# e4s2022/e4s

Measured on AMD Instinct MI355X. Metric: 1024^2 face-swap images/sec, higher is better.
Workload: dtype f32 operands as hi+lo bf16, 3 bf16 MFMAs per product, f32 accumulate (bf16x3) on the 3x3 convs whose launch fills the chip; exact f32 elsewhere; 1 GPU; E4S-core face swap at 1024^2 (2x Net3 encoder @256^2, style swap, 12 LocalMLPs, mask-guided StyleGAN2 generator K=13), BASELINE.json configs[3] shard: 8 swaps per GPU per step; per_gpu_batch=8, global_batch=8, out_size=1024, hip_graph=True, precision=as bf16x3 where the launch fills the chip (this batch), else exact fp32, parallelism=image-parallel x1

## Files before the change

### e4s_amd/csrc/encoder.hip

```cpp
#include "common.h"

namespace {

__global__ void resize_bilinear_kernel(const float* __restrict__ x, float* __restrict__ y, int B, int C, int Hi,
                                       int Wi, int Ho, int Wo) {
    const int64_t n = (int64_t)B * Ho * Wo * C;
    const int64_t i = (int64_t)blockIdx.x * blockDim.x + threadIdx.x;
    if (i >= n) return;
    const int c = (int)(i % C);
    int64_t r = i / C;
    const int ox = (int)(r % Wo); r /= Wo;
    const int oy = (int)(r % Ho);
    const int b = (int)(r / Ho);
    const float sy = (float)Hi / Ho, sx = (float)Wi / Wo;
    float fy = ((float)oy + 0.5f) * sy - 0.5f, fx = ((float)ox + 0.5f) * sx - 0.5f;
    fy = fy < 0.f ? 0.f : fy;
    fx = fx < 0.f ? 0.f : fx;
    const int y0 = (int)fy, x0 = (int)fx;
    const int y1 = y0 + (y0 < Hi - 1 ? 1 : 0), x1 = x0 + (x0 < Wi - 1 ? 1 : 0);
    const float ly = fy - y0, lx = fx - x0, hy = 1.f - ly, hx = 1.f - lx;
    const float* p = x + ((int64_t)b * C + c) * Hi * Wi;
    y[i] = hy * (hx * p[(int64_t)y0 * Wi + x0] + lx * p[(int64_t)y0 * Wi + x1]) +
           ly * (hx * p[(int64_t)y1 * Wi + x0] + lx * p[(int64_t)y1 * Wi + x1]);
}

__global__ void conv3x3_small_kernel(const float* __restrict__ x, const float* __restrict__ w, float* __restrict__ y,
                                     int B, int H, int W, int Cin, int Cout) {
    extern __shared__ float sw[];
    const int nw = Cout * Cin * 9;
    for (int t = threadIdx.x; t < nw; t += blockDim.x) {
        const int k = t % 9, ci = (t / 9) % Cin, co = t / (9 * Cin);
        sw[(k * Cin + ci) * Cout + co] = w[t];
    }
    __syncthreads();
    const int cg = Cout / 4;
    const int64_t n = (int64_t)B * H * W * cg;
    for (int64_t i = (int64_t)blockIdx.x * blockDim.x + threadIdx.x; i < n; i += (int64_t)gridDim.x * blockDim.x) {
        const int c4 = (int)(i % cg) * 4;
        int64_t r = i / cg;
        const int ox = (int)(r % W); r /= W;
        const int oy = (int)(r % H);
        const int b = (int)(r / H);
        f32x4 acc = {0.f, 0.f, 0.f, 0.f};
        for (int ky = 0; ky < 3; ++ky) {
            const int iy = oy + ky - 1;
            if (iy < 0 || iy >= H) continue;
            for (int kx = 0; kx < 3; ++kx) {
                const int ix = ox + kx - 1;
                if (ix < 0 || ix >= W) continue;
                const float* xp = x + (((int64_t)b * H + iy) * W + ix) * Cin;
                const float* wp = sw + ((ky * 3 + kx) * Cin) * Cout + c4;
                for (int ci = 0; ci < Cin; ++ci) acc += xp[ci] * *reinterpret_cast<const f32x4*>(wp + ci * Cout);
            }
        }
        *reinterpret_cast<f32x4*>(y + i * 4) = acc;
    }
}

__global__ __launch_bounds__(256) void conv3x3_stem_kernel(const float* __restrict__ x, const float* __restrict__ w, float* __restrict__ y,
                                                           double* __restrict__ stats_ws, int H, int W, int tx_n, int per_img) {
    __shared__ f32x4 sx[18 * 18];
    __shared__ double sred[2][16][64];
    const int tid = threadIdx.x;
    const int b = blockIdx.x / per_img, rem = blockIdx.x - b * per_img;
    const int tyb = rem / tx_n, txb = rem - tyb * tx_n;
    const int y0 = tyb * 16, x0 = txb * 16;
    for (int h = tid; h < 324; h += 256) {
        const int hy = h / 18, hx = h - hy * 18;
        const int iy = y0 + hy - 1, ix = x0 + hx - 1;
        f32x4 v = {0.f, 0.f, 0.f, 0.f};
        if ((unsigned)iy < (unsigned)H && (unsigned)ix < (unsigned)W) {
            const float* xp = x + (((int64_t)b * H + iy) * W + ix) * 3;
            v = f32x4{xp[0], xp[1], xp[2], 0.f};
        }
        sx[h] = v;
    }
    const int g = tid & 15, py = tid >> 4;
    f32x4 wr[27];
#pragma unroll
    for (int k = 0; k < 9; ++k)
#pragma unroll
        for (int ci = 0; ci < 3; ++ci)
#pragma unroll
            for (int j = 0; j < 4; ++j) wr[k * 3 + ci][j] = w[((4 * g + j) * 3 + ci) * 9 + k];
    __syncthreads();
    double s[4] = {0.0, 0.0, 0.0, 0.0}, q[4] = {0.0, 0.0, 0.0, 0.0};
    float* yrow = y + (((int64_t)b * H + y0 + py) * W + x0) * 64 + 4 * g;
#pragma unroll 4
    for (int px = 0; px < 16; ++px) {
        f32x4 acc = {0.f, 0.f, 0.f, 0.f};
#pragma unroll
        for (int ky = 0; ky < 3; ++ky)
#pragma unroll
            for (int kx = 0; kx < 3; ++kx) {
                const f32x4 v = sx[(py + ky) * 18 + px + kx];
                const int k = (ky * 3 + kx) * 3;
                acc += v[0] * wr[k] + v[1] * wr[k + 1] + v[2] * wr[k + 2];
            }
        *reinterpret_cast<f32x4*>(yrow + (int64_t)px * 64) = acc;
        if (stats_ws) {
#pragma unroll
            for (int j = 0; j < 4; ++j) {
                s[j] += (double)acc[j];
                q[j] += (double)acc[j] * (double)acc[j];
            }
        }
    }
    if (stats_ws) {
#pragma unroll
        for (int j = 0; j < 4; ++j) {
            sred[0][py][4 * g + j] = s[j];
            sred[1][py][4 * g + j] = q[j];
        }
        __syncthreads();
        if (tid < 64) {
            double a = 0.0, c = 0.0;
#pragma unroll
            for (int r = 0; r < 16; ++r) {
                a += sred[0][r][tid];
                c += sred[1][r][tid];
            }
            double* slot = stats_ws + (((int64_t)b * 64 + tid) * per_img + rem) * 2;
            slot[0] = a;
            slot[1] = c;
        }
    }
}

__global__ void instnorm_partial_kernel(const float* __restrict__ x, double* __restrict__ ws, int HW, int C, int nsplit) {
    const int slabs = C / 64;
    const int split = blockIdx.x % nsplit;
    const int slab = (blockIdx.x / nsplit) % slabs;
    const int b = blockIdx.x / (nsplit * slabs);
    const int cl = threadIdx.x & 63, pg = threadIdx.x >> 6;
    const int c = slab * 64 + cl;
    const int per = (HW + nsplit - 1) / nsplit;
    const int p0 = split * per, p1 = (p0 + per < HW) ? p0 + per : HW;
    const float* xb = x + (int64_t)b * HW * C + c;
    double s = 0.0, q = 0.0;
    for (int p = p0 + pg; p < p1; p += 4) {
        const double v = (double)xb[(int64_t)p * C];
        s += v;
        q += v * v;
    }
    __shared__ double red[2][4][64];
    red[0][pg][cl] = s;
    red[1][pg][cl] = q;
    __syncthreads();
    if (pg == 0) {
        s = red[0][0][cl] + red[0][1][cl] + red[0][2][cl] + red[0][3][cl];
        q = red[1][0][cl] + red[1][1][cl] + red[1][2][cl] + red[1][3][cl];
        double* slot = ws + (((int64_t)b * C + c) * nsplit + split) * 2;
        slot[0] = s;
        slot[1] = q;
    }
}

__global__ __launch_bounds__(1024) void instnorm_small_kernel(const float* __restrict__ x, float* __restrict__ stats,
                                                              float* __restrict__ pooled, int HW, int C, float eps) {
    const int slabs = C / 64;
    const int slab = blockIdx.x % slabs, b = blockIdx.x / slabs;
    const int cl = threadIdx.x & 63, pg = threadIdx.x >> 6;
    const int c = slab * 64 + cl;
    const float* xb = x + (int64_t)b * HW * C + c;
    double s = 0.0, q = 0.0;
    int p = pg;
    for (; p + 7 * 16 < HW; p += 8 * 16) {
        float v[8];
#pragma unroll
        for (int u = 0; u < 8; ++u) v[u] = xb[(int64_t)(p + 16 * u) * C];
#pragma unroll
        for (int u = 0; u < 8; ++u) {
            s += (double)v[u];
            q += (double)v[u] * (double)v[u];
        }
    }
    for (; p < HW; p += 16) {
        const double v = (double)xb[(int64_t)p * C];
        s += v;
        q += v * v;
    }
    __shared__ double red[2][16][64];
    red[0][pg][cl] = s;
    red[1][pg][cl] = q;
    __syncthreads();
    if (pg == 0) {
        s = 0.0;
        q = 0.0;
#pragma unroll
        for (int k = 0; k < 16; ++k) { s += red[0][k][cl]; q += red[1][k][cl]; }
        const double mean = s / HW;
        double var = q / HW - mean * mean;
        if (var < 0.0) var = 0.0;
        const float mf = (float)mean;
        const float rstd = rsqrtf((float)var + eps);
        const int64_t i = (int64_t)b * C + c;
        stats[i * 2] = mf;
        stats[i * 2 + 1] = rstd;
        if (pooled) pooled[i] = (float)((mean - (double)mf) * (double)rstd);
    }
}

__global__ void instnorm_finalize_kernel(const double* __restrict__ ws, float* __restrict__ stats,
                                         float* __restrict__ pooled, int n, int HW, float eps, int nsplit) {
    const int i = blockIdx.x * blockDim.x + threadIdx.x;
    if (i >= n) return;
    double s = 0.0, q = 0.0;
#pragma unroll 8
    for (int k = 0; k < nsplit; ++k) {
        s += ws[((int64_t)i * nsplit + k) * 2];
        q += ws[((int64_t)i * nsplit + k) * 2 + 1];
    }
    const double mean = s / HW;
    double var = q / HW - mean * mean;
    if (var < 0.0) var = 0.0;
    const float mf = (float)mean;
    const float rstd = rsqrtf((float)var + eps);
    stats[i * 2] = mf;
    stats[i * 2 + 1] = rstd;
    if (pooled) pooled[i] = (float)((mean - (double)mf) * (double)rstd);
}

__global__ void instnorm_apply_kernel(const float* __restrict__ x, const float* __restrict__ stats,
                                      const float* __restrict__ gate, const float* __restrict__ res,
                                      const float* __restrict__ res_stats, const float* __restrict__ slope,
                                      float* __restrict__ y, int B, int H, int W, int C, int rs) {
    const int C4 = C / 4;
    const int64_t n = (int64_t)B * H * W * C4;
    const int64_t i = (int64_t)blockIdx.x * blockDim.x + threadIdx.x;
    if (i >= n) return;
    const int c = (int)(i % C4) * 4;
    int64_t r = i / C4;
    const int xx = (int)(r % W); r /= W;
    const int yy = (int)(r % H);
    const int b = (int)(r / H);
    f32x4 v = *reinterpret_cast<const f32x4*>(x + i * 4);
    f32x4 o;
#pragma unroll
    for (int e = 0; e < 4; ++e) {
        const float* st = stats + ((int64_t)b * C + c + e) * 2;
        o[e] = (v[e] - st[0]) * st[1];
        if (gate) o[e] *= gate[(int64_t)b * C + c + e];
    }
    if (res) {
        const int Hr = H * rs, Wr = W * rs;
        const f32x4 rv = *reinterpret_cast<const f32x4*>(res + (((int64_t)b * Hr + (int64_t)yy * rs) * Wr + (int64_t)xx * rs) * C + c);
#pragma unroll
        for (int e = 0; e < 4; ++e) {
            float t = rv[e];
            if (res_stats) {
                const float* st = res_stats + ((int64_t)b * C + c + e) * 2;
                t = (t - st[0]) * st[1];
            }
            o[e] += t;
        }
    }
    if (slope) {
#pragma unroll
        for (int e = 0; e < 4; ++e) o[e] = o[e] > 0.f ? o[e] : o[e] * slope[c + e];
    }
    *reinterpret_cast<f32x4*>(y + i * 4) = o;
}

__global__ void instnorm_apply_stats_kernel(const float* __restrict__ x, const float* __restrict__ stats,
                                            const float* __restrict__ gate, const float* __restrict__ res,
                                            const float* __restrict__ res_stats, const float* __restrict__ slope,
                                            float* __restrict__ y, double* __restrict__ ws, int H, int W, int C, int rs,
                                            int nsplit) {
    const int slabs = C / 64, HW = H * W;
    const int split = blockIdx.x % nsplit;
    const int slab = (blockIdx.x / nsplit) % slabs;
    const int b = blockIdx.x / (nsplit * slabs);
    const int cl = (threadIdx.x & 15) * 4, pg = threadIdx.x >> 4;
    const int c = slab * 64 + cl;
    const int per = (HW + nsplit - 1) / nsplit;
    const int p0 = split * per, p1 = (p0 + per < HW) ? p0 + per : HW;
    const int64_t bc = (int64_t)b * C + c;
    f32x4 mean, rstd, g, rmean, rrstd, sl;
#pragma unroll
    for (int e = 0; e < 4; ++e) {
        mean[e] = stats[(bc + e) * 2];
        rstd[e] = stats[(bc + e) * 2 + 1];
        g[e] = gate ? gate[bc + e] : 1.f;
        rmean[e] = res_stats ? res_stats[(bc + e) * 2] : 0.f;
        rrstd[e] = res_stats ? res_stats[(bc + e) * 2 + 1] : 1.f;
        sl[e] = slope ? slope[c + e] : 0.f;
    }
    const int Wr = W * rs;
    double s[4] = {0.0, 0.0, 0.0, 0.0}, q[4] = {0.0, 0.0, 0.0, 0.0};
    for (int p = p0 + pg; p < p1; p += 16) {
        const int64_t idx = ((int64_t)b * HW + p) * C + c;
        f32x4 o = (*reinterpret_cast<const f32x4*>(x + idx) - mean) * rstd;
        if (gate) o *= g;
        if (res) {
            const int yy = p / W, xx = p - yy * W;
            f32x4 t = *reinterpret_cast<const f32x4*>(res + (((int64_t)b * H * rs + (int64_t)yy * rs) * Wr + (int64_t)xx * rs) * C + c);
            if (res_stats) t = (t - rmean) * rrstd;
            o += t;
        }
        if (slope) {
#pragma unroll
            for (int e = 0; e < 4; ++e) o[e] = o[e] > 0.f ? o[e] : o[e] * sl[e];
        }
        *reinterpret_cast<f32x4*>(y + idx) = o;
#pragma unroll
        for (int e = 0; e < 4; ++e) {
            s[e] += (double)o[e];
            q[e] += (double)o[e] * (double)o[e];
        }
    }
    __shared__ double red[2][16][64];
#pragma unroll
    for (int e = 0; e < 4; ++e) {
        red[0][pg][cl + e] = s[e];
        red[1][pg][cl + e] = q[e];
    }
    __syncthreads();
    if (threadIdx.x < 64) {
        double a = 0.0, d = 0.0;
#pragma unroll
        for (int k = 0; k < 16; ++k) {
            a += red[0][k][threadIdx.x];
            d += red[1][k][threadIdx.x];
        }
        double* slot = ws + (((int64_t)b * C + slab * 64 + threadIdx.x) * nsplit + split) * 2;
        slot[0] = a;
        slot[1] = d;
    }
}

__device__ __forceinline__ void se_body(const float* pooled, float* hidden, const float* __restrict__ fc1,
                                        const float* __restrict__ fc2, float* __restrict__ gate, int C, int Cr) {
    int tpr = 64;
    while (tpr * Cr > (int)blockDim.x && tpr > 1) tpr >>= 1;
    for (int j0 = 0; j0 < Cr; j0 += blockDim.x / tpr) {
        const int j = j0 + threadIdx.x / tpr, l = threadIdx.x % tpr;
        float a = 0.f;
        if (j < Cr) {
            const float* row = fc1 + (int64_t)j * C;
            int c = l;
            for (; c + 7 * tpr < C; c += 8 * tpr) {
                float w[8];
#pragma unroll
                for (int u = 0; u < 8; ++u) w[u] = row[c + u * tpr];
#pragma unroll
                for (int u = 0; u < 8; ++u) a += w[u] * pooled[c + u * tpr];
            }
            for (; c < C; c += tpr) a += row[c] * pooled[c];
        }
        for (int o = tpr >> 1; o > 0; o >>= 1) a += __shfl_xor(a, o, 64);
        if (j < Cr && l == 0) hidden[j] = a > 0.f ? a : 0.f;
    }
    __syncthreads();
    for (int c = threadIdx.x; c < C; c += blockDim.x) {
        float a = 0.f;
        if ((Cr & 3) == 0) {
            const f32x4* w4 = reinterpret_cast<const f32x4*>(fc2 + (int64_t)c * Cr);
#pragma unroll 8
            for (int j = 0; j < Cr; j += 4) {
                const f32x4 w = w4[j >> 2];
                a += w[0] * hidden[j];
                a += w[1] * hidden[j + 1];
                a += w[2] * hidden[j + 2];
                a += w[3] * hidden[j + 3];
            }
        } else {
            for (int j = 0; j < Cr; ++j) a += fc2[(int64_t)c * Cr + j] * hidden[j];
        }
        gate[c] = 1.f / (1.f + __expf(-a));
    }
}

__global__ __launch_bounds__(512) void se_gate_kernel(const float* __restrict__ pooled_in, const float* __restrict__ fc1,
                                                      const float* __restrict__ fc2, float* __restrict__ gate, int C, int Cr) {
    extern __shared__ float sm[];
    float* pooled = sm;
    float* hidden = sm + C;
    const int b = blockIdx.x;
    for (int c = threadIdx.x; c < C; c += blockDim.x) pooled[c] = pooled_in[(int64_t)b * C + c];
    __syncthreads();
    se_body(pooled, hidden, fc1, fc2, gate + (int64_t)b * C, C, Cr);
}

__global__ __launch_bounds__(512) void finalize_se_kernel(const double* __restrict__ ws, float* __restrict__ stats,
                                                          const float* __restrict__ fc1, const float* __restrict__ fc2,
                                                          float* __restrict__ gate, int C, int Cr, int HW, float eps, int nsplit) {
    extern __shared__ float sm[];
    float* pooled = sm;
    float* hidden = sm + C;
    const int b = blockIdx.x;
    for (int c = threadIdx.x; c < C; c += blockDim.x) {
        const int64_t i = (int64_t)b * C + c;
        double s = 0.0, q = 0.0;
#pragma unroll 8
        for (int k = 0; k < nsplit; ++k) {
            s += ws[(i * nsplit + k) * 2];
            q += ws[(i * nsplit + k) * 2 + 1];
        }
        const double mean = s / HW;
        double var = q / HW - mean * mean;
        if (var < 0.0) var = 0.0;
        const float mf = (float)mean;
        const float rstd = rsqrtf((float)var + eps);
        stats[i * 2] = mf;
        stats[i * 2 + 1] = rstd;
        pooled[c] = (float)((mean - (double)mf) * (double)rstd);
    }
    __syncthreads();
    se_body(pooled, hidden, fc1, fc2, gate + (int64_t)b * C, C, Cr);
}

__device__ __forceinline__ int nearest_src(int dst, int in, int out) {
    const float scale = (float)in / (float)out;
    const int s = (int)floorf((float)dst * scale);
    return s < in - 1 ? s : in - 1;
}

constexpr int RM_PIX = 256;
constexpr int RM_NPG = 16;
__global__ __launch_bounds__(256) void region_mean_kernel(const float* __restrict__ feats, const uint8_t* __restrict__ labels, int Hm,
                                                          int Wm, float* __restrict__ out, float* __restrict__ ws, int H, int W, int C,
                                                          int R, int out_stride, int out_off, int nsplit) {
    extern __shared__ float sm[];
    const int slabs = C / 64;
    const int split = blockIdx.x % nsplit;
    const int slab = (blockIdx.x / nsplit) % slabs;
    const int b = blockIdx.x / (nsplit * slabs);
    const int cl = (threadIdx.x & 15) * 4, pg = threadIdx.x >> 4;
    float* sums = sm;
    int* cnt = reinterpret_cast<int*>(sm + RM_NPG * R * 64);
    for (int t = threadIdx.x; t < RM_NPG * R * 64; t += blockDim.x) sums[t] = 0.f;
    for (int t = threadIdx.x; t < R; t += blockDim.x) cnt[t] = 0;
    __syncthreads();
    const int HW = H * W;
    const int pbeg = split * RM_PIX, pend = pbeg + RM_PIX < HW ? pbeg + RM_PIX : HW;
    const float* fb = feats + (int64_t)b * HW * C + slab * 64 + cl;
    float* mine = sums + (pg * R) * 64 + cl;
    constexpr int U = 8;
    for (int p0 = pbeg + pg; p0 < pend; p0 += RM_NPG * U) {
        f32x4 v[U];
        int lab[U];
#pragma unroll
        for (int u = 0; u < U; ++u) {
            const int p = p0 + u * RM_NPG;
            const bool ok = p < pend;
            const int pp = ok ? p : pbeg;
            const int yy = pp / W, xx = pp - yy * W;
            lab[u] = ok ? labels[((int64_t)b * Hm + nearest_src(yy, Hm, H)) * Wm + nearest_src(xx, Wm, W)] : -1;
            v[u] = *reinterpret_cast<const f32x4*>(fb + (int64_t)pp * C);
        }
#pragma unroll
        for (int u = 0; u < U; ++u) {
            if (lab[u] >= 0 && lab[u] < R) {
                f32x4* acc = reinterpret_cast<f32x4*>(mine + lab[u] * 64);
                *acc += v[u];
                if (cl == 0) atomicAdd(&cnt[lab[u]], 1);
            }
        }
    }
    __syncthreads();
    for (int t = threadIdx.x; t < R * 64; t += blockDim.x) {
        const int r = t / 64, c = t % 64;
        float s = 0.f;
        for (int j = 0; j < RM_NPG; ++j) s += sums[(j * R + r) * 64 + c];
        if (ws) {
            ws[((int64_t)blockIdx.x * R + r) * 65 + c] = s;
            if (c == 0) ws[((int64_t)blockIdx.x * R + r) * 65 + 64] = __int_as_float(cnt[r]);
        } else {
            const int n = cnt[r];
            out[((int64_t)b * R + r) * out_stride + out_off + slab * 64 + c] = n > 0 ? s / (float)n : 0.f;
        }
    }
}

__global__ void region_mean_finish_kernel(const float* __restrict__ ws, float* __restrict__ out, int B, int C, int R, int out_stride,
                                          int out_off, int nsplit) {
    const int i = blockIdx.x * blockDim.x + threadIdx.x;
    if (i >= B * R * C) return;
    const int c = i % C, r = (i / C) % R, b = i / (C * R);
    const int slab = c >> 6, cc = c & 63;
// ... 36 lines not shown
                acc += w[j][0] * v[0] + w[j][1] * v[1] + w[j][2] * v[2] + w[j][3] * v[3];
            }
        }
        float a = wave_sum(acc);
        if (lane == 0) {
            a = a * scale + bs;
            if (act == 1) a = a > 0.f ? a : a * alpha;
            y[((int64_t)b * R + r) * O + o] = a + ad;
        }
    }
}

constexpr int GL_TB = 8;
template <int KV, int NR>
__global__ __launch_bounds__(256) __attribute__((amdgpu_waves_per_eu(2))) void grouped_linear_rows_kernel(const float* __restrict__ x, const float* __restrict__ Wt,
                                                                  const float* __restrict__ bias, const float* __restrict__ add,
                                                                  float* __restrict__ y, int B, int R, int K, int O, float scale,
                                                                  int act, float alpha) {
    constexpr int N = NR * GL_TB;
    const int lane = threadIdx.x & 63;
    const int opr = O / NR;
    const int64_t wid = (int64_t)blockIdx.x * (blockDim.x >> 6) + (threadIdx.x >> 6);
    if (wid >= (int64_t)R * opr) return;
    const int r = (int)(wid / opr), o0 = (int)(wid % opr) * NR;
    const float* wrow = Wt + ((int64_t)r * O + o0) * K;
    f32x4 w[NR][KV];
#pragma unroll
    for (int n = 0; n < NR; ++n)
#pragma unroll
        for (int j = 0; j < KV; ++j) {
            const int i = (j * 64 + lane) * 4;
            w[n][j] = i < K ? *reinterpret_cast<const f32x4*>(wrow + (int64_t)n * K + i) : f32x4{0.f, 0.f, 0.f, 0.f};
        }
    static_assert(N == 64 || N == 32, "lane -> value mapping below");
    constexpr int SH = N == 64 ? 0 : 1;
    const int mine = lane >> SH, tbm = mine / NR, nm = mine % NR;
    const float bs = bias ? bias[(int64_t)r * O + o0 + nm] : 0.f;
    const float ad = add ? add[o0 + nm] : 0.f;
    for (int b0 = 0; b0 < B; b0 += GL_TB) {
        float v[N];
#pragma unroll
        for (int tb = 0; tb < GL_TB; ++tb) {
            if (b0 + tb < B) {
                const float* xr = x + ((int64_t)(b0 + tb) * R + r) * K;
                f32x4 xv[KV];
#pragma unroll
                for (int j = 0; j < KV; ++j) {
                    const int i = (j * 64 + lane) * 4;
                    xv[j] = i < K ? *reinterpret_cast<const f32x4*>(xr + i) : f32x4{0.f, 0.f, 0.f, 0.f};
                }
#pragma unroll
                for (int n = 0; n < NR; ++n) {
                    float acc = 0.f;
#pragma unroll
                    for (int j = 0; j < KV; ++j)
#pragma unroll
                        for (int e = 0; e < 4; ++e) acc = fmaf(w[n][j][e], xv[j][e], acc);
                    v[tb * NR + n] = acc;
                }
            } else {
#pragma unroll
                for (int n = 0; n < NR; ++n) v[tb * NR + n] = 0.f;
            }
        }
        packed_wave_sum<N>(v, lane);
        if ((lane & ((1 << SH) - 1)) == 0 && b0 + tbm < B) {
            float a = v[0] * scale + bs;
            if (act == 1) a = a > 0.f ? a : a * alpha;
            y[((int64_t)(b0 + tbm) * R + r) * O + o0 + nm] = a + ad;
        }
    }
}

__global__ void grouped_linear_longk_kernel(const float* __restrict__ x, const float* __restrict__ Wt,
                                            const float* __restrict__ bias, const float* __restrict__ add,
                                            float* __restrict__ y, int B, int R, int K, int O, float scale, int act,
                                            float alpha) {
    const int lane = threadIdx.x & 63;
    const int64_t wid = (int64_t)blockIdx.x * (blockDim.x >> 6) + (threadIdx.x >> 6);
    if (wid >= (int64_t)R * O) return;
    const int r = (int)(wid / O), o = (int)(wid % O);
    const float* wrow = Wt + ((int64_t)r * O + o) * K;
    for (int b = 0; b < B; ++b) {
        const float* xr = x + ((int64_t)b * R + r) * K;
        float acc = 0.f;
        for (int i = lane * 4; i < K; i += 256) {
            const f32x4 w = *reinterpret_cast<const f32x4*>(wrow + i);
            const f32x4 v = *reinterpret_cast<const f32x4*>(xr + i);
            acc += w[0] * v[0] + w[1] * v[1] + w[2] * v[2] + w[3] * v[3];
        }
        float a = wave_sum(acc);
        if (lane == 0) {
            a = a * scale + (bias ? bias[(int64_t)r * O + o] : 0.f);
            if (act == 1) a = a > 0.f ? a : a * alpha;
            y[((int64_t)b * R + r) * O + o] = a + (add ? add[o] : 0.f);
        }
    }
}


__global__ __launch_bounds__(256) void swap_styles_kernel(const float* __restrict__ tgt, const float* __restrict__ src,
                                                          float* __restrict__ out, int R, int C, unsigned sel, int ear, int teeth,
                                                          int below) {
    __shared__ float part[256];
    const int b = blockIdx.x / R, r = blockIdx.x - b * R;
    const float* a = tgt + ((int64_t)b * R + r) * C;
    const float* c = src + ((int64_t)b * R + r) * C;
    float* o = out + ((int64_t)b * R + r) * C;
    int mode = (sel >> r) & 1u;
    if (r == ear || r == teeth) {
        float s = 0.f;
        for (int i = threadIdx.x; i < C; i += 256) s += c[i];
        part[threadIdx.x] = s;
        __syncthreads();
        for (int st = 128; st > 0; st >>= 1) {
            if ((int)threadIdx.x < st) part[threadIdx.x] += part[threadIdx.x + st];
            __syncthreads();
        }
        if (part[0] == 0.f) mode = (r == ear) ? 2 : 0;
    }
    if (r == below) mode = 2;
    for (int i = threadIdx.x; i < C; i += 256) o[i] = mode == 2 ? (a[i] + c[i]) / 2.f : (mode == 1 ? c[i] : a[i]);
}

}

extern "C" int e4s_resize_bilinear_f32(const float* x, float* y, int B, int C, int Hi, int Wi, int Ho, int Wo, void* stream) {
    const int64_t n = (int64_t)B * Ho * Wo * C;
    if (n <= 0) return 0;
    hipLaunchKernelGGL(resize_bilinear_kernel, dim3((unsigned)((n + 255) / 256)), dim3(256), 0, as_stream(stream), x, y, B, C, Hi, Wi, Ho, Wo);
    E4S_CHECK_LAUNCH();
    return 0;
}

extern "C" int e4s_conv3x3_small_f32(const float* x, const float* w, float* y, int B, int H, int W, int Cin, int Cout, void* stream) {
    if (Cout % 4) return (int)hipErrorInvalidValue;
    const int64_t n = (int64_t)B * H * W * (Cout / 4);
    if (n <= 0) return 0;
    const size_t smem = (size_t)Cout * Cin * 9 * sizeof(float);
    if (smem > 48 * 1024) return (int)hipErrorInvalidValue;
    int64_t nblk = (n + 255) / 256;
    if (nblk > 4096) nblk = 4096;
    hipLaunchKernelGGL(conv3x3_small_kernel, dim3((unsigned)nblk), dim3(256), smem, as_stream(stream), x, w, y, B, H, W, Cin, Cout);
    E4S_CHECK_LAUNCH();
    return 0;
}

extern "C" int e4s_conv3x3_stem_f32(const float* x, const float* w, float* y, double* stats_ws, int B, int H, int W, int Cin, int Cout,
                                    void* stream) {
    if (!x || !w || !y || Cin != 3 || Cout != 64 || H % 16 || W % 16 || B <= 0 || H <= 0 || W <= 0) return (int)hipErrorInvalidValue;
    const int tx_n = W / 16, per_img = (H / 16) * tx_n;
    const int64_t blocks = (int64_t)B * per_img;
    if (blocks >= (1ll << 31)) return (int)hipErrorInvalidValue;
    hipLaunchKernelGGL(conv3x3_stem_kernel, dim3((unsigned)blocks), dim3(256), 0, as_stream(stream), x, w, y, stats_ws, H, W, tx_n, per_img);
    E4S_CHECK_LAUNCH();
    return 0;
}

static int instnorm_nsplit(int B, int HW, int C) {
    int nsplit = 2048 / (B * (C / 64) > 0 ? B * (C / 64) : 1);
    if (nsplit < 1) nsplit = 1;
    if (nsplit > HW / 64) nsplit = HW / 64 > 0 ? HW / 64 : 1;
    if (nsplit > 64) nsplit = 64;
    return nsplit;
}

extern "C" int e4s_instnorm_stats_f32(const float* x, float* stats, float* pooled, double* ws, int B, int HW, int C,
                                      float eps, void* stream) {
    if (C % 64) return (int)hipErrorInvalidValue;
    hipStream_t st = as_stream(stream);
    if (HW <= 1024 && HW >= 16) {
        hipLaunchKernelGGL(instnorm_small_kernel, dim3(B * (C / 64)), dim3(1024), 0, st, x, stats, pooled, HW, C, eps);
        E4S_CHECK_LAUNCH();
        return 0;
    }
    const int nsplit = instnorm_nsplit(B, HW, C);
    hipLaunchKernelGGL(instnorm_partial_kernel, dim3(B * (C / 64) * nsplit), dim3(256), 0, st, x, ws, HW, C, nsplit);
    E4S_CHECK_LAUNCH();
    const int n = B * C;
    hipLaunchKernelGGL(instnorm_finalize_kernel, dim3((n + 255) / 256), dim3(256), 0, st, ws, stats, pooled, n, HW, eps, nsplit);
    E4S_CHECK_LAUNCH();
    return 0;
}

extern "C" int e4s_instnorm_finalize_f32(const double* ws, float* stats, float* pooled, int B, int HW, int C, int nslots,
                                         float eps, void* stream) {
    const int n = B * C;
    if (n <= 0 || nslots < 1) return (int)hipErrorInvalidValue;
    hipLaunchKernelGGL(instnorm_finalize_kernel, dim3((n + 255) / 256), dim3(256), 0, as_stream(stream), ws, stats, pooled, n,
                       HW, eps, nslots);
    E4S_CHECK_LAUNCH();
    return 0;
}

extern "C" int e4s_instnorm_apply_stats_f32(const float* x, const float* stats, const float* gate, const float* res,
                                            const float* res_stats, const float* slope, float* y, double* ws, int* nslots,
                                            int B, int H, int W, int C, int rs, void* stream) {
    if (C % 64 || rs < 1 || !nslots) return (int)hipErrorInvalidValue;
    const int ns = instnorm_nsplit(B, H * W, C);
    *nslots = ns;
    hipLaunchKernelGGL(instnorm_apply_stats_kernel, dim3(B * (C / 64) * ns), dim3(256), 0, as_stream(stream), x, stats, gate,
                       res, res_stats, slope, y, ws, H, W, C, rs, ns);
    E4S_CHECK_LAUNCH();
    return 0;
}

extern "C" int64_t e4s_instnorm_ws_doubles(int B, int HW, int C) {
    return (int64_t)2 * B * C * instnorm_nsplit(B, HW, C);
}

extern "C" int e4s_instnorm_apply_f32(const float* x, const float* stats, const float* gate, const float* res,
                                      const float* res_stats, const float* slope, float* y, int B, int H, int W, int C,
                                      int rs, void* stream) {
    if (C % 4 || rs < 1) return (int)hipErrorInvalidValue;
    const int64_t n = (int64_t)B * H * W * (C / 4);
    if (n <= 0) return 0;
    hipLaunchKernelGGL(instnorm_apply_kernel, dim3((unsigned)((n + 255) / 256)), dim3(256), 0, as_stream(stream), x, stats, gate, res, res_stats, slope, y, B, H, W, C, rs);
    E4S_CHECK_LAUNCH();
    return 0;
}

extern "C" int e4s_se_gate_f32(const float* pooled, const float* fc1, const float* fc2, float* gate, int B, int C,
                               int Cr, void* stream) {
    if (B <= 0 || C <= 0 || Cr <= 0 || (size_t)(C + Cr) * sizeof(float) > 48 * 1024) return (int)hipErrorInvalidValue;
    hipLaunchKernelGGL(se_gate_kernel, dim3(B), dim3(512), (size_t)(C + Cr) * sizeof(float), as_stream(stream), pooled, fc1, fc2, gate, C, Cr);
    E4S_CHECK_LAUNCH();
    return 0;
}

extern "C" int e4s_instnorm_finalize_se_f32(const double* ws, float* stats, const float* fc1, const float* fc2, float* gate, int B,
                                            int HW, int C, int Cr, int nslots, float eps, void* stream) {
    if (B <= 0 || C <= 0 || Cr <= 0 || nslots <= 0 || HW <= 0 || (size_t)(C + Cr) * sizeof(float) > 48 * 1024)
        return (int)hipErrorInvalidValue;
    hipLaunchKernelGGL(finalize_se_kernel, dim3(B), dim3(512), (size_t)(C + Cr) * sizeof(float), as_stream(stream), ws, stats, fc1, fc2,
                       gate, C, Cr, HW, eps, nslots);
    E4S_CHECK_LAUNCH();
    return 0;
}

static int region_mean_nsplit(int HW) { return (HW + RM_PIX - 1) / RM_PIX; }

extern "C" int64_t e4s_region_mean_ws_floats(int B, int HW, int C, int R) {
    const int ns = region_mean_nsplit(HW);
    return ns > 1 ? (int64_t)B * (C / 64) * ns * R * 65 : 0;
}

extern "C" int e4s_region_mean_f32(const float* feats, const uint8_t* labels, int Hm, int Wm, float* out, float* ws, int B, int H,
                                   int W, int C, int R, int out_stride, int out_off, void* stream) {
    if (C % 64 || R > 64 || R < 1 || B <= 0 || H <= 0 || W <= 0) return (int)hipErrorInvalidValue;
    if (reinterpret_cast<uintptr_t>(feats) & 15) return (int)hipErrorInvalidValue;
    const int ns = region_mean_nsplit(H * W);
    if (ns > 1 && !ws) return (int)hipErrorInvalidValue;
    const int64_t blocks = (int64_t)B * (C / 64) * ns;
    if (blocks >= (1ll << 31) || (int64_t)B * R * C >= (1ll << 31)) return (int)hipErrorInvalidValue;
    const size_t smem = (size_t)(RM_NPG * R * 64) * sizeof(float) + (size_t)R * sizeof(int);
    if (smem > 64 * 1024) return (int)hipErrorInvalidValue;
    hipStream_t st = as_stream(stream);
    hipLaunchKernelGGL(region_mean_kernel, dim3((unsigned)blocks), dim3(256), smem, st, feats, labels, Hm, Wm, out, ns > 1 ? ws : nullptr,
                       H, W, C, R, out_stride, out_off, ns);
    E4S_CHECK_LAUNCH();
    if (ns > 1) {
        const int n = B * R * C;
        hipLaunchKernelGGL(region_mean_finish_kernel, dim3((n + 255) / 256), dim3(256), 0, st, ws, out, B, C, R, out_stride, out_off, ns);
        E4S_CHECK_LAUNCH();
    }
    return 0;
}

extern "C" int e4s_grouped_linear_f32(const float* x, const float* W, const float* bias, const float* add, float* y,
                                      int B, int R, int K, int O, float scale, int act, float alpha, void* stream) {
    if (K % 4) return (int)hipErrorInvalidValue;
    const int64_t nw = (int64_t)R * O;
    if (nw <= 0 || B <= 0) return 0;
    hipStream_t st = as_stream(stream);
    if (K > 64 * 4 * MAXKV) {
        hipLaunchKernelGGL(grouped_linear_longk_kernel, dim3((unsigned)((nw + 3) / 4)), dim3(256), 0, st, x, W, bias, add, y, B, R, K, O, scale, act, alpha);
        E4S_CHECK_LAUNCH();
        return 0;
    }
    if (K <= 1536 && O % 8 == 0 && nw >= 4096) {
        if (K <= 512)
            hipLaunchKernelGGL((grouped_linear_rows_kernel<2, 8>), dim3((unsigned)((nw / 8 + 3) / 4)), dim3(256), 0, st, x, W, bias, add, y, B, R, K, O, scale, act, alpha);
        else if (K <= 1024)
            hipLaunchKernelGGL((grouped_linear_rows_kernel<4, 4>), dim3((unsigned)((nw / 4 + 3) / 4)), dim3(256), 0, st, x, W, bias, add, y, B, R, K, O, scale, act, alpha);
        else
            hipLaunchKernelGGL((grouped_linear_rows_kernel<6, 4>), dim3((unsigned)((nw / 4 + 3) / 4)), dim3(256), 0, st, x, W, bias, add, y, B, R, K, O, scale, act, alpha);
        E4S_CHECK_LAUNCH();
        return 0;
    }
    hipLaunchKernelGGL(grouped_linear_kernel, dim3((unsigned)((nw + 3) / 4)), dim3(256), 0, st, x, W, bias, add, y, B, R, K, O, scale, act, alpha);
    E4S_CHECK_LAUNCH();
    return 0;
}

extern "C" int e4s_swap_styles_f32(const float* tgt, const float* src, float* out, int B, int R, int C, unsigned sel, int ear, int teeth,
                                   int below, void* stream) {
    if (!tgt || !src || !out || B < 1 || R < 1 || R > 32 || C < 1) return (int)hipErrorInvalidValue;
    hipLaunchKernelGGL(swap_styles_kernel, dim3((unsigned)(B * R)), dim3(256), 0, as_stream(stream), tgt, src, out, R, C, sel, ear, teeth,
                       below);
    E4S_CHECK_LAUNCH();
    return 0;
}
```

### e4s_amd/csrc/ops.hip

```cpp
#include "common.h"

namespace {

__device__ __forceinline__ float bias_act_one(float x, float ref, int code, float alpha, float scale) {
    float y;
    switch (code) {
        case 12: case 32: y = 0.f; break;
        case 30: y = (x > 0.f) ? x : x * alpha; break;
        case 31: y = (ref > 0.f) ? x : x * alpha; break;
        default: y = x; break;
    }
    return y * scale;
}

__global__ void fused_bias_act_v4(const f32x4* __restrict__ x, const float* __restrict__ b,
                                  const f32x4* __restrict__ ref, f32x4* __restrict__ y, int64_t n4,
                                  int step_b, int size_b, int code, float alpha, float scale) {
    const int64_t stride = (int64_t)gridDim.x * blockDim.x;
    for (int64_t i = (int64_t)blockIdx.x * blockDim.x + threadIdx.x; i < n4; i += stride) {
        f32x4 v = x[i];
        if (b) {
            const float bv = b[((i * 4) / step_b) % size_b];
            v += bv;
        }
        f32x4 r = {0.f, 0.f, 0.f, 0.f};
        if (ref) r = ref[i];
        f32x4 o;
#pragma unroll
        for (int e = 0; e < 4; ++e) o[e] = bias_act_one(v[e], r[e], code, alpha, scale);
        y[i] = o;
    }
}

__global__ void fused_bias_act_scalar(const float* __restrict__ x, const float* __restrict__ b,
                                      const float* __restrict__ ref, float* __restrict__ y, int64_t n,
                                      int step_b, int size_b, int code, float alpha, float scale) {
    const int64_t stride = (int64_t)gridDim.x * blockDim.x;
    for (int64_t i = (int64_t)blockIdx.x * blockDim.x + threadIdx.x; i < n; i += stride) {
        float v = x[i];
        if (b) v += b[(i / step_b) % size_b];
        y[i] = bias_act_one(v, ref ? ref[i] : 0.f, code, alpha, scale);
    }
}

__global__ void channel_sum_kernel(const float* __restrict__ g, float* __restrict__ out, int64_t n,
                                   int step_b, int size_b) {
    const int c = blockIdx.x;
    const int64_t outer = n / ((int64_t)step_b * size_b);
    float acc = 0.f;
    for (int64_t o = 0; o < outer; ++o) {
        const float* base = g + (o * size_b + c) * (int64_t)step_b;
        for (int i = threadIdx.x; i < step_b; i += blockDim.x) acc += base[i];
    }
    __shared__ float red[4];
    acc = wave_sum(acc);
    if ((threadIdx.x & 63) == 0) red[threadIdx.x >> 6] = acc;
    __syncthreads();
    if (threadIdx.x == 0) out[c] = red[0] + red[1] + red[2] + red[3];
}

constexpr int TOH = 16, TOW = 64;

__device__ __forceinline__ int floordiv(int a, int b) {
    int c = a / b;
    if (c * b > a) --c;
    return c;
}

__global__ void upfirdn2d_kernel(const float* __restrict__ x, const float* __restrict__ k, float* __restrict__ y,
                                 int major, int in_h, int in_w, int minor, int kh, int kw, int up_x, int up_y,
                                 int down_x, int down_y, int pad_x0, int pad_y0, int out_h, int out_w,
                                 int tin_h, int tin_w, int tiles_x, int tiles_y) {
    extern __shared__ float sm[];
    float* sk = sm;
    float* sx = sm + kh * kw;
    int bid = blockIdx.x;
    const int tx = bid % tiles_x; bid /= tiles_x;
    const int ty = bid % tiles_y; bid /= tiles_y;
    const int mi = bid % minor;
    const int mj = bid / minor;
    const int oy0 = ty * TOH, ox0 = tx * TOW;
    for (int t = threadIdx.x; t < kh * kw; t += blockDim.x) {
        const int ky = t / kw, kx = t - ky * kw;
        sk[t] = k[(kh - 1 - ky) * kw + (kw - 1 - kx)];
    }
    const int mid_y0 = oy0 * down_y - pad_y0, mid_x0 = ox0 * down_x - pad_x0;
    const int in_y0 = floordiv(mid_y0 + up_y - 1, up_y), in_x0 = floordiv(mid_x0 + up_x - 1, up_x);
    for (int t = threadIdx.x; t < tin_h * tin_w; t += blockDim.x) {
        const int ry = t / tin_w, rx = t - ry * tin_w;
        const int iy = in_y0 + ry, ix = in_x0 + rx;
        float v = 0.f;
        if (iy >= 0 && ix >= 0 && iy < in_h && ix < in_w)
            v = x[(((int64_t)mj * in_h + iy) * in_w + ix) * minor + mi];
        sx[t] = v;
    }
    __syncthreads();
    for (int t = threadIdx.x; t < TOH * TOW; t += blockDim.x) {
        const int ry = t / TOW, rx = t - ry * TOW;
        const int oy = oy0 + ry, ox = ox0 + rx;
        if (oy >= out_h || ox >= out_w) continue;
        const int my = oy * down_y - pad_y0, mx = ox * down_x - pad_x0;
        const int iy_first = floordiv(my + up_y - 1, up_y), ix_first = floordiv(mx + up_x - 1, up_x);
        float acc = 0.f;
        for (int iy = iy_first, jy = iy_first * up_y - my; jy < kh; ++iy, jy += up_y) {
            const float* row = sx + (iy - in_y0) * tin_w;
            for (int ix = ix_first, jx = ix_first * up_x - mx; jx < kw; ++ix, jx += up_x)
                acc += row[ix - in_x0] * sk[jy * kw + jx];
        }
        y[(((int64_t)mj * out_h + oy) * out_w + ox) * minor + mi] = acc;
    }
}

}

extern "C" int e4s_abi_version(void) { return 18; }
extern "C" const char* e4s_build_arch(void) { return "gfx950"; }

extern "C" int e4s_fused_bias_act_f32(const float* x, const float* b, const float* ref, float* y, int64_t n,
                                      int step_b, int size_b, int act, int grad, float alpha, float scale,
                                      void* stream) {
    if (n <= 0) return 0;
    const int code = act * 10 + grad;
    if (code == 31 && !ref) return (int)hipErrorInvalidValue;
    if (b && (step_b <= 0 || size_b <= 0)) return (int)hipErrorInvalidValue;
    const bool vec = (n % 4 == 0) && (!b || step_b % 4 == 0) &&
                     ((reinterpret_cast<uintptr_t>(x) | reinterpret_cast<uintptr_t>(y) |
                       reinterpret_cast<uintptr_t>(ref)) % 16 == 0);
    const int block = 256;
    if (vec) {
        const int64_t n4 = n / 4;
        const int grid = (int)((n4 + block - 1) / block < 8192 ? (n4 + block - 1) / block : 8192);
        hipLaunchKernelGGL(fused_bias_act_v4, dim3(grid), dim3(block), 0, as_stream(stream),
                           reinterpret_cast<const f32x4*>(x), b, reinterpret_cast<const f32x4*>(ref),
                           reinterpret_cast<f32x4*>(y), n4, step_b, size_b, code, alpha, scale);
    } else {
        const int grid = (int)((n + block - 1) / block < 8192 ? (n + block - 1) / block : 8192);
        hipLaunchKernelGGL(fused_bias_act_scalar, dim3(grid), dim3(block), 0, as_stream(stream), x, b, ref, y, n,
                           step_b, size_b, code, alpha, scale);
    }
    E4S_CHECK_LAUNCH();
    return 0;
}

extern "C" int e4s_channel_sum_f32(const float* g, float* out, int64_t n, int step_b, int size_b, void* stream) {
    if (size_b <= 0 || step_b <= 0 || n % ((int64_t)step_b * size_b)) return (int)hipErrorInvalidValue;
    hipLaunchKernelGGL(channel_sum_kernel, dim3(size_b), dim3(256), 0, as_stream(stream), g, out, n, step_b, size_b);
    E4S_CHECK_LAUNCH();
    return 0;
}

__global__ __launch_bounds__(256) void fir_nhwc_kernel(const float* __restrict__ x, const float* __restrict__ k, float* __restrict__ y,
                                                       int in_h, int in_w, int C, int kh, int kw, int pad_x0, int pad_y0,
                                                       int out_h, int out_w) {
    __shared__ float sk[64];
    if (threadIdx.x < kh * kw) {
        const int ky = threadIdx.x / kw, kx = threadIdx.x - ky * kw;
        sk[threadIdx.x] = k[(kh - 1 - ky) * kw + (kw - 1 - kx)];
    }
    __syncthreads();
    const int c4n = C >> 2, ppb = 256 / c4n;
    const int c4 = threadIdx.x % c4n, pxl = threadIdx.x / c4n;
    const int ox = blockIdx.x * ppb + pxl, oy0 = blockIdx.y * 4;
    if (pxl >= ppb || ox >= out_w) return;
    const float* xb = x + (size_t)blockIdx.z * in_h * in_w * C + c4 * 4;
    f32x4 acc[4];
#pragma unroll
    for (int r = 0; r < 4; ++r) acc[r] = f32x4{0.f, 0.f, 0.f, 0.f};
    for (int ry = 0; ry < kh + 3; ++ry) {
        const int iy = oy0 + ry - pad_y0;
        if ((unsigned)iy >= (unsigned)in_h) continue;
        for (int jx = 0; jx < kw; ++jx) {
            const int ix = ox + jx - pad_x0;
            if ((unsigned)ix >= (unsigned)in_w) continue;
            const f32x4 v = *reinterpret_cast<const f32x4*>(xb + ((size_t)iy * in_w + ix) * C);
#pragma unroll
            for (int r = 0; r < 4; ++r) {
                const int jy = ry - r;
                if (jy >= 0 && jy < kh) acc[r] += v * sk[jy * kw + jx];
            }
        }
    }
#pragma unroll
    for (int r = 0; r < 4; ++r)
        if (oy0 + r < out_h)
            *reinterpret_cast<f32x4*>(y + (((size_t)blockIdx.z * out_h + oy0 + r) * out_w + ox) * C + c4 * 4) = acc[r];
}

template <int KH, int KW>
__global__ __launch_bounds__(256) void fir_nhwc_fixed_kernel(const float* __restrict__ x, const float* __restrict__ k, float* __restrict__ y,
                                                             int in_h, int in_w, int C, int pad_x0, int pad_y0, int out_h, int out_w) {
    __shared__ float sk[KH * KW];
    if (threadIdx.x < KH * KW) {
        const int ky = threadIdx.x / KW, kx = threadIdx.x - ky * KW;
        sk[threadIdx.x] = k[(KH - 1 - ky) * KW + (KW - 1 - kx)];
    }
    __syncthreads();
    const int c4n = C >> 2, ppb = 256 / c4n;
    const int c4 = threadIdx.x % c4n, pxl = threadIdx.x / c4n;
    const int ox = blockIdx.x * ppb + pxl, oy0 = blockIdx.y * 4;
    if (pxl >= ppb || ox >= out_w) return;
    const float* xb = x + (size_t)blockIdx.z * in_h * in_w * C + c4 * 4;
    f32x4 v[KH + 3][KW];
#pragma unroll
    for (int ry = 0; ry < KH + 3; ++ry) {
        const int iy = oy0 + ry - pad_y0;
#pragma unroll
        for (int jx = 0; jx < KW; ++jx) {
            const int ix = ox + jx - pad_x0;
            v[ry][jx] = ((unsigned)iy < (unsigned)in_h && (unsigned)ix < (unsigned)in_w)
                            ? *reinterpret_cast<const f32x4*>(xb + ((size_t)iy * in_w + ix) * C) : f32x4{0.f, 0.f, 0.f, 0.f};
        }
    }
#pragma unroll
    for (int r = 0; r < 4; ++r) {
        if (oy0 + r >= out_h) continue;
        f32x4 acc = {0.f, 0.f, 0.f, 0.f};
#pragma unroll
        for (int ry = r; ry < r + KH; ++ry) {
            const int iy = oy0 + ry - pad_y0;
            if ((unsigned)iy >= (unsigned)in_h) continue;
#pragma unroll
            for (int jx = 0; jx < KW; ++jx) {
                const int ix = ox + jx - pad_x0;
                if ((unsigned)ix < (unsigned)in_w) acc += v[ry][jx] * sk[(ry - r) * KW + jx];
            }
        }
        *reinterpret_cast<f32x4*>(y + (((size_t)blockIdx.z * out_h + oy0 + r) * out_w + ox) * C + c4 * 4) = acc;
    }
}

extern "C" int e4s_upfirdn2d_f32(const float* x, const float* k, float* y, int major, int in_h, int in_w, int minor,
                                 int kh, int kw, int up_x, int up_y, int down_x, int down_y, int pad_x0, int pad_x1,
                                 int pad_y0, int pad_y1, void* stream) {
    if (up_x < 1 || up_y < 1 || down_x < 1 || down_y < 1 || kh < 1 || kw < 1 || kh > 16 || kw > 16)
        return (int)hipErrorInvalidValue;
    const int out_h = (in_h * up_y + pad_y0 + pad_y1 - kh) / down_y + 1;
    const int out_w = (in_w * up_x + pad_x0 + pad_x1 - kw) / down_x + 1;
    if (out_h <= 0 || out_w <= 0 || major <= 0 || minor <= 0) return 0;
    if (up_x == 1 && up_y == 1 && down_x == 1 && down_y == 1 && minor % 4 == 0 && minor >= 8 && minor <= 1024 && kh * kw <= 64 &&
        major <= 65535) {
        const int ppb = 256 / (minor / 4);
        if (kh == 4 && kw == 4) {
            hipLaunchKernelGGL((fir_nhwc_fixed_kernel<4, 4>), dim3((unsigned)((out_w + ppb - 1) / ppb), (unsigned)((out_h + 3) / 4), (unsigned)major),
                               dim3(256), 0, as_stream(stream), x, k, y, in_h, in_w, minor, pad_x0, pad_y0, out_h, out_w);
            E4S_CHECK_LAUNCH();
            return 0;
        }
        hipLaunchKernelGGL(fir_nhwc_kernel, dim3((unsigned)((out_w + ppb - 1) / ppb), (unsigned)((out_h + 3) / 4), (unsigned)major),
                           dim3(256), 0, as_stream(stream), x, k, y, in_h, in_w, minor, kh, kw, pad_x0, pad_y0, out_h, out_w);
        E4S_CHECK_LAUNCH();
        return 0;
    }
    const int tin_h = ((TOH - 1) * down_y + kh - 1) / up_y + 2;
    const int tin_w = ((TOW - 1) * down_x + kw - 1) / up_x + 2;
    const int tiles_x = (out_w + TOW - 1) / TOW, tiles_y = (out_h + TOH - 1) / TOH;
    const int64_t blocks = (int64_t)tiles_x * tiles_y * major * minor;
    if (blocks > 0x7fffffff) return (int)hipErrorInvalidValue;
    const size_t smem = (size_t)(kh * kw + tin_h * tin_w) * sizeof(float);
    hipLaunchKernelGGL(upfirdn2d_kernel, dim3((unsigned)blocks), dim3(256), smem, as_stream(stream), x, k, y, major,
                       in_h, in_w, minor, kh, kw, up_x, up_y, down_x, down_y, pad_x0, pad_y0, out_h, out_w, tin_h,
                       tin_w, tiles_x, tiles_y);
    E4S_CHECK_LAUNCH();
    return 0;
}
```

### e4s_amd/csrc/style.hip

```cpp
#include "common.h"

namespace {

constexpr int GCHUNK = 8;
constexpr int RD_OW = 4;
template <int MODE>
__global__ void rowdot_kernel(const float* __restrict__ in, int64_t in_stride, const float* __restrict__ M,
                              const float* __restrict__ bias, float* __restrict__ out, int G, int O, int K,
                              float scale) {
    const int lane = threadIdx.x & 63;
    const int o = blockIdx.x * (blockDim.x >> 6) + (threadIdx.x >> 6);
    if (o >= O) return;
    const int g0 = blockIdx.y * GCHUNK;
    const float* mrow = M + (size_t)o * K;
    float acc[GCHUNK];
#pragma unroll
    for (int j = 0; j < GCHUNK; ++j) acc[j] = 0.f;
    for (int i = lane * 4; i < K; i += 256) {
        const f32x4 m = *reinterpret_cast<const f32x4*>(mrow + i);
#pragma unroll
        for (int j = 0; j < GCHUNK; ++j) {
            if (g0 + j < G) {
                f32x4 x = *reinterpret_cast<const f32x4*>(in + (size_t)(g0 + j) * in_stride + i);
                if (MODE == 1) x *= x;
                acc[j] += m[0] * x[0] + m[1] * x[1] + m[2] * x[2] + m[3] * x[3];
            }
        }
    }
#pragma unroll
    for (int j = 0; j < GCHUNK; ++j) {
        if (g0 + j < G) {
            const float a = wave_sum(acc[j]);
            if (lane == 0) {
                float r;
                if (MODE == 0) r = a * scale + (bias ? bias[o] : 0.f);
                else r = scale * rsqrtf(scale * scale * a + 1e-8f);
                out[(size_t)(g0 + j) * O + o] = r;
            }
        }
    }
}

template <int MODE>
__global__ void rowdot_multi_kernel(const e4s_rowdot_job* __restrict__ jobs, const float* __restrict__ in_base,
                                    float* __restrict__ out_base) {
    const e4s_rowdot_job jb = jobs[blockIdx.z];
    const int lane = threadIdx.x & 63;
    const int o0 = (blockIdx.x * (blockDim.x >> 6) + (threadIdx.x >> 6)) * RD_OW;
    const int g0 = blockIdx.y * GCHUNK;
    if (o0 >= jb.O || g0 >= jb.G) return;
    const float* in = in_base + jb.in_off;
    float* out = out_base + jb.out_off;
    const int G = jb.G, O = jb.O, K = jb.K;
    const float scale = jb.scale;
    float acc[RD_OW * GCHUNK];
#pragma unroll
    for (int t = 0; t < RD_OW * GCHUNK; ++t) acc[t] = 0.f;
    for (int i = lane * 4; i < K; i += 256) {
        f32x4 m[RD_OW];
#pragma unroll
        for (int w = 0; w < RD_OW; ++w)
            m[w] = o0 + w < O ? *reinterpret_cast<const f32x4*>(jb.M + (size_t)(o0 + w) * K + i) : f32x4{0.f, 0.f, 0.f, 0.f};
#pragma unroll
        for (int j = 0; j < GCHUNK; ++j) {
            if (g0 + j < G) {
                f32x4 x = *reinterpret_cast<const f32x4*>(in + (size_t)(g0 + j) * jb.in_stride + i);
                if (MODE == 1) x *= x;
#pragma unroll
                for (int w = 0; w < RD_OW; ++w) acc[w * GCHUNK + j] += m[w][0] * x[0] + m[w][1] * x[1] + m[w][2] * x[2] + m[w][3] * x[3];
            }
        }
    }
    static_assert(RD_OW * GCHUNK == 32, "lane -> (w, j) below");
    packed_wave_sum<RD_OW * GCHUNK>(acc, lane);
    const int o = o0 + (lane >> 1) / GCHUNK, g = g0 + (lane >> 1) % GCHUNK;
    if ((lane & 1) == 0 && o < O && g < G) {
        const float a = acc[0];
        float r;
        if (MODE == 0) r = a * scale + (jb.bias ? jb.bias[o] : 0.f);
        else r = scale * rsqrtf(scale * scale * a + 1e-8f);
        out[(size_t)g * O + o] = r;
    }
}

__global__ void weight_sqsum_kernel(const float* __restrict__ w, float* __restrict__ wsq, int64_t n, int taps) {
    const int64_t i = (int64_t)blockIdx.x * blockDim.x + threadIdx.x;
    if (i >= n) return;
    float acc = 0.f;
    for (int t = 0; t < taps; ++t) {
        const float v = w[i * taps + t];
        acc += v * v;
    }
    wsq[i] = acc;
}

__global__ void rgb_weights_kernel(const float* __restrict__ w, const float* __restrict__ s, float* __restrict__ ws,
                                   int G, int cin, float scale) {
    const int64_t i = (int64_t)blockIdx.x * blockDim.x + threadIdx.x;
    const int64_t n = (int64_t)G * 3 * cin;
    if (i >= n) return;
    const int ci = (int)(i % cin);
    const int c = (int)((i / cin) % 3);
    const int g = (int)(i / (3 * (int64_t)cin));
    ws[i] = scale * w[c * cin + ci] * s[(size_t)g * cin + ci];
}

__global__ void polyphase_weights_kernel(const float* __restrict__ w, const float* __restrict__ k4,
                                         float* __restrict__ out, int cout, int cin) {
    const int64_t n = (int64_t)cout * cin;
    const int64_t i = (int64_t)blockIdx.x * blockDim.x + threadIdx.x;
    if (i >= n) return;
    float wv[9], kf[16];
#pragma unroll
    for (int t = 0; t < 9; ++t) wv[t] = w[i * 9 + t];
#pragma unroll
    for (int t = 0; t < 16; ++t) kf[t] = k4[15 - t];
#pragma unroll
    for (int ph = 0; ph < 4; ++ph) {
        const int py = ph >> 1, px = ph & 1;
#pragma unroll
        for (int ey = 0; ey < 3; ++ey) {
#pragma unroll
            for (int ex = 0; ex < 3; ++ex) {
                const int ty = py - 2 * (ey - 1), tx = px - 2 * (ex - 1);
                float acc = 0.f;
#pragma unroll
                for (int jy = 0; jy < 4; ++jy) {
                    const int ky = ty + jy - 1;
                    if (ky < 0 || ky > 2) continue;
#pragma unroll
                    for (int jx = 0; jx < 4; ++jx) {
                        const int kx = tx + jx - 1;
                        if (kx < 0 || kx > 2) continue;
                        acc += kf[jy * 4 + jx] * wv[ky * 3 + kx];
                    }
                }
                out[((int64_t)(ph * 9 + ey * 3 + ex)) * n + i] = acc;
            }
        }
    }
}

__global__ void polyphase_fold_kernel(const float* __restrict__ deff, const float* __restrict__ k4, float* __restrict__ dw, int cout,
                                      int cin) {
    const int64_t n = (int64_t)cout * cin;
    const int64_t i = (int64_t)blockIdx.x * blockDim.x + threadIdx.x;
    if (i >= n) return;
    float kf[16], acc[9];
#pragma unroll
    for (int t = 0; t < 16; ++t) kf[t] = k4[15 - t];
#pragma unroll
    for (int t = 0; t < 9; ++t) acc[t] = 0.f;
#pragma unroll
    for (int ph = 0; ph < 4; ++ph) {
        const int py = ph >> 1, px = ph & 1;
#pragma unroll
        for (int ey = 0; ey < 3; ++ey) {
#pragma unroll
            for (int ex = 0; ex < 3; ++ex) {
                const int ty = py - 2 * (ey - 1), tx = px - 2 * (ex - 1);
                const float g = deff[((int64_t)(ph * 9 + ey * 3 + ex)) * n + i];
#pragma unroll
                for (int jy = 0; jy < 4; ++jy) {
                    const int ky = ty + jy - 1;
                    if (ky < 0 || ky > 2) continue;
#pragma unroll
                    for (int jx = 0; jx < 4; ++jx) {
                        const int kx = tx + jx - 1;
                        if (kx < 0 || kx > 2) continue;
                        acc[ky * 3 + kx] += kf[jy * 4 + jx] * g;
                    }
                }
            }
        }
    }
#pragma unroll
    for (int t = 0; t < 9; ++t) dw[i * 9 + t] = acc[t];
}

__global__ void pack_taps_kernel(const float* __restrict__ w, float* __restrict__ out, int64_t n, int taps) {
    const int64_t i = (int64_t)blockIdx.x * blockDim.x + threadIdx.x;
    if (i >= n) return;
    for (int t = 0; t < taps; ++t) out[(int64_t)t * n + i] = w[i * taps + t];
}

}

extern "C" int e4s_polyphase_weights_f32(const float* w, const float* k4, float* out, int cout, int cin, void* stream) {
    const int64_t n = (int64_t)cout * cin;
    hipLaunchKernelGGL(polyphase_weights_kernel, dim3((unsigned)((n + 255) / 256)), dim3(256), 0, as_stream(stream), w, k4, out, cout, cin);
    E4S_CHECK_LAUNCH();
    return 0;
}

extern "C" int e4s_polyphase_fold_f32(const float* deff, const float* k4, float* dw, int cout, int cin, void* stream) {
    if (!deff || !k4 || !dw || cout <= 0 || cin <= 0) return (int)hipErrorInvalidValue;
    const int64_t n = (int64_t)cout * cin;
    hipLaunchKernelGGL(polyphase_fold_kernel, dim3((unsigned)((n + 255) / 256)), dim3(256), 0, as_stream(stream), deff, k4, dw, cout, cin);
    E4S_CHECK_LAUNCH();
    return 0;
}

extern "C" int e4s_pack_taps_f32(const float* w, float* out, int cout, int cin, int taps, void* stream) {
    const int64_t n = (int64_t)cout * cin;
    hipLaunchKernelGGL(pack_taps_kernel, dim3((unsigned)((n + 255) / 256)), dim3(256), 0, as_stream(stream), w, out, n, taps);
    E4S_CHECK_LAUNCH();
    return 0;
}

extern "C" int e4s_rowdot_f32(const float* in, int64_t in_stride, const float* M, const float* bias, float* out,
                              int G, int O, int K, int mode, float scale, void* stream) {
    if (K % 4 || (mode != 0 && mode != 1)) return (int)hipErrorInvalidValue;
    if (G <= 0 || O <= 0) return 0;
    const int waves = 4;
    dim3 grid((O + waves - 1) / waves, (G + GCHUNK - 1) / GCHUNK), block(64 * waves);
    if (mode == 0)
        hipLaunchKernelGGL(rowdot_kernel<0>, grid, block, 0, as_stream(stream), in, in_stride, M, bias, out, G, O, K, scale);
    else
        hipLaunchKernelGGL(rowdot_kernel<1>, grid, block, 0, as_stream(stream), in, in_stride, M, bias, out, G, O, K, scale);
    E4S_CHECK_LAUNCH();
    return 0;
}

extern "C" int e4s_rowdot_multi_f32(const e4s_rowdot_job* jobs, int njobs, const float* in_base, float* out_base, int max_O,
                                    int max_G, int mode, void* stream) {
    if (!jobs || njobs <= 0 || (mode != 0 && mode != 1) || max_O <= 0 || max_G <= 0 || njobs > 65535) return (int)hipErrorInvalidValue;
    const int waves = 4;
    dim3 grid((max_O + waves * RD_OW - 1) / (waves * RD_OW), (max_G + GCHUNK - 1) / GCHUNK, njobs), block(64 * waves);
    if (mode == 0) hipLaunchKernelGGL(rowdot_multi_kernel<0>, grid, block, 0, as_stream(stream), jobs, in_base, out_base);
    else hipLaunchKernelGGL(rowdot_multi_kernel<1>, grid, block, 0, as_stream(stream), jobs, in_base, out_base);
    E4S_CHECK_LAUNCH();
    return 0;
}

extern "C" int e4s_weight_sqsum_f32(const float* w, float* wsq, int cout, int cin, int taps, void* stream) {
    const int64_t n = (int64_t)cout * cin;
    hipLaunchKernelGGL(weight_sqsum_kernel, dim3((unsigned)((n + 255) / 256)), dim3(256), 0, as_stream(stream), w, wsq, n, taps);
    E4S_CHECK_LAUNCH();
    return 0;
}

extern "C" int e4s_rgb_weights_f32(const float* w, const float* s, float* ws, int G, int cin, float scale, void* stream) {
    const int64_t n = (int64_t)G * 3 * cin;
    hipLaunchKernelGGL(rgb_weights_kernel, dim3((unsigned)((n + 255) / 256)), dim3(256), 0, as_stream(stream), w, s, ws, G, cin, scale);
    E4S_CHECK_LAUNCH();
    return 0;
}
```

### e4s_amd/kernels.py

```python
import contextlib
import ctypes
import math
import os
import threading

import torch

from . import lib
from .lib import ConvBwdParams, ConvParams, ConvWgradParams, c_p, call, fptr, ptr, stream

BM = 128
PRECISION = os.environ.get("E4S_PRECISION", "auto")
if PRECISION not in ("f32", "bf16x3", "auto"):
    raise RuntimeError(f"E4S_PRECISION must be f32, bf16x3 or auto, got {PRECISION!r}")
BF16X3_MIN_BLOCKS = int(os.environ.get("E4S_BF16X3_MIN_BLOCKS", "128"))
LRELU_GAIN = math.sqrt(2.0)


def _f32(t):
    if t.dtype != torch.float32:
        raise RuntimeError(f"expected float32 tensor, got {t.dtype}")
    return t.contiguous()


# ... 9 lines not shown
         fptr(_f32(ref)) if has_r else None, fptr(y), x.numel(), step_b, bias.numel() if has_b else 1,
         int(act), int(grad), float(alpha), float(scale), stream())
    return y


def channel_sum(g):
    g = _f32(g)
    c = g.shape[1]
    step_b = 1
    for d in g.shape[2:]:
        step_b *= d
    out = torch.empty(c, device=g.device, dtype=torch.float32)
    call("e4s_channel_sum_f32", fptr(g), fptr(out), g.numel(), step_b, c, stream())
    return out


def upfirdn2d_raw(x, kernel, up_x, up_y, down_x, down_y, pad_x0, pad_x1, pad_y0, pad_y1):
    x = _f32(x)
    kernel = _f32(kernel)
    major, in_h, in_w, minor = x.shape
    kh, kw = kernel.shape
    out_h = (in_h * up_y + pad_y0 + pad_y1 - kh) // down_y + 1
    out_w = (in_w * up_x + pad_x0 + pad_x1 - kw) // down_x + 1
    y = torch.empty(major, out_h, out_w, minor, device=x.device, dtype=torch.float32)
    call("e4s_upfirdn2d_f32", fptr(x), fptr(kernel), fptr(y), major, in_h, in_w, minor, kh, kw, up_x, up_y,
         down_x, down_y, pad_x0, pad_x1, pad_y0, pad_y1, stream())
    return y


def nchw_to_nhwc(x):
    x = _f32(x)
    b, c, h, w = x.shape
    y = torch.empty(b, h, w, c, device=x.device, dtype=torch.float32)
    call("e4s_nchw_to_nhwc_f32", fptr(x), fptr(y), b, c, h, w, stream())
    return y


def nhwc_to_nchw(x):
    x = _f32(x)
    b, h, w, c = x.shape
    y = torch.empty(b, c, h, w, device=x.device, dtype=torch.float32)
    call("e4s_nhwc_to_nchw_f32", fptr(x), fptr(y), b, c, h, w, stream())
    return y


def const_input(inp, batch):
    inp = _f32(inp)
    _, c, h, w = inp.shape
    y = torch.empty(batch, h, w, c, device=inp.device, dtype=torch.float32)
    call("e4s_const_input_f32", fptr(inp), fptr(y), batch, c, h, w, stream())
    return y


def modulate(latent, layer_idx, masked, mod_weight, mod_bias):
    b, r, nl, d = latent.shape
    cin = mod_weight.shape[0]
    g = b * r if masked else b
    stride = nl * d if masked else r * nl * d
    out = torch.empty(g, cin, device=latent.device, dtype=torch.float32)
    base = c_p(latent.data_ptr() + layer_idx * d * 4)
    call("e4s_rowdot_f32", base, stride, fptr(mod_weight), fptr(mod_bias), fptr(out), g, cin, d, 0,
         1.0 / math.sqrt(d), stream())
    return out


def modulate_vec(style, mod_weight, mod_bias):
    style = _f32(style)
    g, d = style.shape
    cin = mod_weight.shape[0]
    out = torch.empty(g, cin, device=style.device, dtype=torch.float32)
    call("e4s_rowdot_f32", fptr(style), d, fptr(mod_weight), fptr(mod_bias), fptr(out), g, cin, d, 0,
         1.0 / math.sqrt(d), stream())
    return out


_JOB_FMT = "qqqQQiiif"


def rowdot_jobs(jobs, device):
    import struct
    buf = b"".join(struct.pack(_JOB_FMT, int(j["in_off"]), int(j["in_stride"]), int(j["out_off"]), j["M"].data_ptr(),
                               j["bias"].data_ptr() if j["bias"] is not None else 0, int(j["G"]), int(j["O"]), int(j["K"]),
                               float(j["scale"])) for j in jobs)
    assert struct.calcsize(_JOB_FMT) == 56
    for j in jobs:
        if j["M"].dtype != torch.float32 or not j["M"].is_contiguous() or j["K"] % 4:
            raise RuntimeError("rowdot_jobs: contiguous fp32 matrices with K % 4 == 0")
    table = torch.frombuffer(bytearray(buf), dtype=torch.uint8).to(device)
    return table, len(jobs), max(j["O"] for j in jobs), max(j["G"] for j in jobs)


def rowdot_multi(table, njobs, max_o, max_g, in_base, out_base, mode):
    call("e4s_rowdot_multi_f32", ptr(table), njobs, fptr(in_base), fptr(out_base), max_o, max_g, mode, stream())


def demod_coefs(s, wsq, conv_scale):
    g, cin = s.shape
    cout = wsq.shape[0]
    out = torch.empty(g, cout, device=s.device, dtype=torch.float32)
    call("e4s_rowdot_f32", fptr(s), cin, fptr(wsq), None, fptr(out), g, cout, cin, 1, float(conv_scale), stream())
    return out


def weight_sqsum(w, out=None):
    w = _f32(w)
    cout, cin = w.shape[:2]
    taps = w.shape[2] * w.shape[3]
    if out is None:
        out = torch.empty(cout, cin, device=w.device, dtype=torch.float32)
    elif out.shape != (cout, cin) or out.dtype != torch.float32 or out.device != w.device or not out.is_contiguous():
        raise RuntimeError("weight_sqsum: out must be a contiguous fp32 [Cout,Cin] tensor on the weight's device")
    call("e4s_weight_sqsum_f32", fptr(w), fptr(out), cout, cin, taps, stream())
    return out


def _into(out, shape, device):
    if out is None:
        return torch.empty(shape, device=device, dtype=torch.float32)
    if tuple(out.shape) != tuple(shape) or out.dtype != torch.float32 or out.device != device or not out.is_contiguous():
        raise RuntimeError(f"pack buffer mismatch: need contiguous fp32 {tuple(shape)} on {device}, got {tuple(out.shape)} {out.dtype} {out.device}")
    return out


def pack_taps(w, out=None):
    w = _f32(w)
    cout, cin = w.shape[:2]
    taps = w.shape[2] * w.shape[3]
    out = _into(out, (1, taps, cout, cin), w.device)
    call("e4s_pack_taps_f32", fptr(w), fptr(out), cout, cin, taps, stream())
    return out


def polyphase_weights(w, blur_kernel, out=None):
    w = _f32(w)
    cout, cin = w.shape[:2]
    out = _into(out, (4, 9, cout, cin), w.device)
    call("e4s_polyphase_weights_f32", fptr(w), fptr(_f32(blur_kernel)), fptr(out), cout, cin, stream())
    return out


def polyphase_fold(deff, blur_kernel, cout, cin):
    deff = _f32(deff)
    if deff.numel() != 36 * cout * cin:
        raise RuntimeError("polyphase_fold: deff must hold 4 * 9 * Cout * Cin values")
    dw = torch.empty(cout, cin, 3, 3, device=deff.device, dtype=torch.float32)
    call("e4s_polyphase_fold_f32", fptr(deff), fptr(_f32(blur_kernel)), fptr(dw), cout, cin, stream())
    return dw


def rgb_weights(w, s, scale):
    g, cin = s.shape
    out = torch.empty(g, 3, cin, device=s.device, dtype=torch.float32)
    call("e4s_rgb_weights_f32", fptr(w), fptr(s), fptr(out), g, cin, float(scale), stream())
    return out


_tls = threading.local()


@contextlib.contextmanager
def flag_sink(flags):
    prev = getattr(_tls, "sink", None)
    _tls.sink = flags
    try:
        yield flags
    finally:
        _tls.sink = prev


def mask_labels(mask):
    mask = _f32(mask)
    b, r, hm, wm = mask.shape
    labels = torch.empty(b, hm, wm, device=mask.device, dtype=torch.uint8)
    sink = getattr(_tls, "sink", None)
    flags = sink if sink is not None else torch.zeros(1, device=mask.device, dtype=torch.int32)
    call("e4s_mask_labels", fptr(mask), ptr(labels), ptr(flags), b, r, hm, wm, stream())
    return labels, flags


def swap_styles(tgt, src, comp_indices, below_face=False):
    tgt, src = _f32(tgt), _f32(src)
    b, r, c = tgt.shape
    out = torch.empty_like(tgt)
    sel = 0
    for i in comp_indices:
        sel |= 1 << int(i)
    call("e4s_swap_styles_f32", fptr(tgt), fptr(src), fptr(out), b, r, c, sel, 7, 9, 8 if below_face else -1, stream())
    return out


class RowPlan:
    __slots__ = ("rows", "tiles", "meta", "tiles_cap", "Ha", "Wa", "nphase", "R")


def region_plan(labels, num_regions, ha, wa, nphase):
    b, hm, wm = labels.shape
    nkeys = b * num_regions * nphase
    rows_cap = b * ha * wa * nphase + nkeys * BM
    tiles_cap = (rows_cap + BM - 1) // BM
    dev = labels.device
    pl = RowPlan()
    pl.rows = torch.empty(rows_cap, device=dev, dtype=torch.int32)
    pl.tiles = torch.empty(tiles_cap * 4, device=dev, dtype=torch.int32)
    pl.meta = torch.empty(4, device=dev, dtype=torch.int32)
    work = torch.empty(3 * nkeys, device=dev, dtype=torch.int32)
    call("e4s_region_plan", ptr(labels), b, num_regions, hm, wm, ha, wa, nphase, BM, ptr(pl.rows), ptr(pl.tiles),
         ptr(pl.meta), ptr(work), rows_cap, tiles_cap, stream())
    pl.tiles_cap, pl.Ha, pl.Wa, pl.nphase, pl.R = tiles_cap, ha, wa, nphase, num_regions
    return pl


_split_tl = threading.local()


@contextlib.contextmanager
def f32_plain_split(on=True):
    prev = getattr(_split_tl, "on", False)
    _split_tl.on = bool(on)
    try:
        yield
    finally:
        _split_tl.on = prev


def conv_mfma(x, w, cout, *, plan=None, istride=1, ostride=1, ntaps=9, ncls=1, in_scale=None, out_scale=None,
              noise=None, noise_w=None, noise_per_channel=False, bias=None, slope=None, act=0, alpha=0.2,
              gain=LRELU_GAIN, spatial=None, anchors=None, labels=None, num_regions=1, w_split=None, in_stats=None,
              out=None, tap_shift=0, want_stats=False, w_split16=None, se=None):
    b, hi, wi, cin = x.shape
    if anchors is None:
        anchors = (hi // istride, wi // istride)
    ha, wa = anchors
    ho, wo = ha * ostride, wa * ostride
    if spatial is None:
        spatial = plan is None and istride == 1 and ntaps == 9
    if labels is not None and not spatial:
        raise RuntimeError("per-pixel region labels need the spatial (halo-tiled) mode")
    if plan is None and not spatial and (ha * wa) % BM != 0 and w_split is None and (in_scale is not None or out_scale is not None):
        plan = region_plan(torch.zeros(b, 1, 1, device=x.device, dtype=torch.uint8), 1, ha, wa, ncls)
    if out is None:
        y = torch.empty(b, ho, wo, cout, device=x.device, dtype=torch.float32)
    else:
        y = out
        if tuple(y.shape[:3]) != (b, ho, wo) or y.shape[3] < cout or labels is not None or plan is not None:
            raise RuntimeError("conv_mfma(out=...): need an unlabelled conv and an NHWC buffer [B,Ho,Wo,>=Cout]")
    p = ConvParams()
    p.x, p.w, p.y = fptr(x), fptr(w), fptr(y)
    p.y_cstride = y.shape[3] if out is not None else 0
    p.tap_shift = int(tap_shift)
    if plan is not None:
        p.rows, p.tiles, p.meta, p.tiles_cap = ptr(plan.rows), ptr(plan.tiles), ptr(plan.meta), plan.tiles_cap
        p.groups_per_batch = plan.R
    else:
        p.rows = p.tiles = p.meta = None
        p.tiles_cap = 0
        p.groups_per_batch = num_regions if labels is not None else 1
    if labels is not None:
        p.labels, p.Hm, p.Wm = ptr(labels), labels.shape[1], labels.shape[2]
    else:
        p.labels, p.Hm, p.Wm = None, 0, 0
    p.B, p.Ha, p.Wa = b, ha, wa
    p.Hi, p.Wi, p.Ho, p.Wo, p.Cin, p.Cout = hi, wi, ho, wo, cin, cout
    p.istride, p.ostride, p.ntaps, p.ncls = istride, ostride, ntaps, ncls
    p.in_scale, p.out_scale = fptr(in_scale), fptr(out_scale)
    if noise is not None:
        p.noise, p.noise_w = fptr(noise), fptr(noise_w)
        p.noise_bstride = ho * wo if noise.shape[0] > 1 else 0
        p.noise_per_channel = 1 if noise_per_channel else 0
    else:
        p.noise = p.noise_w = None
        p.noise_bstride = 0
        p.noise_per_channel = 0
    p.bias, p.slope = fptr(bias), fptr(slope)
    p.act, p.alpha, p.gain = act, alpha, gain
    p.in_stats = fptr(in_stats)
    p.split_hint = 1 if getattr(_split_tl, "on", False) else 0
    if w_split is not None:
        gather_ok = (istride == 2 or ntaps == 1) and cin % 32 == 0 and (cout % 128 == 0 or cout == 64) and ncls == 1 and ostride == 1 \
            and plan is None and labels is None and in_scale is None and out_scale is None and noise is None \
            and in_stats is None
        if not gather_ok and (
                not bf16x3_eligible(cin, cout, istride=istride, ostride=ostride, ntaps=ntaps, ncls=ncls,
                                    masked=labels is not None)
                or not spatial or noise_per_channel or (labels is not None and in_scale is None)
                or (in_stats is not None and (in_scale is not None or labels is not None))):
            raise RuntimeError("e4s_conv_bf16x3_f32 does not cover this contraction")
        p.w = fptr(w_split)
        if w_split16 is not None:
            if labels is None or out is not None:
                raise RuntimeError("e4s_conv_region_bf16x3_f32 is the masked-layer kernel")
            nws = lib.load().e4s_conv_region_ws_floats(ctypes.byref(p))
            if nws <= 0:
                raise RuntimeError("e4s_conv_region_bf16x3_f32 does not cover this contraction")
            skws = torch.empty(nws, device=x.device, dtype=torch.float32)
            p.splitk_ws = fptr(skws)
            global LAST_REGION_PATH
            LAST_REGION_PATH = lib.load().e4s_conv_region_path(ctypes.byref(p))
            call("e4s_conv_region_bf16x3_f32", ctypes.byref(p), ptr(w_split16), stream())
            return y
        nws = lib.load().e4s_conv_bf16x3_ws_floats(ctypes.byref(p))
        skws = torch.empty(nws, device=x.device, dtype=torch.float32) if nws else None
        p.splitk_ws = fptr(skws)
        fused = None
        if want_stats and nws == 0 and act == 0 and noise is None and out_scale is None and labels is None and ncls == 1 \
                and cout % 64 == 0 and out is None:
            if gather_ok:
# ... 151 lines not shown
    p.x, p.w, p.y = fptr(x), fptr(w3), fptr(y)
    p.y_cstride = y.shape[3] if out is not None else 0
    p.rows = p.tiles = p.meta = None
    p.tiles_cap = 0
    p.B, p.Ha, p.Wa = b, hi, wi
    p.Hi, p.Wi, p.Ho, p.Wo, p.Cin, p.Cout = hi, wi, ho, wo, cin, cout
    p.istride, p.ostride, p.ntaps, p.ncls = 1, 2, 9, 1
    p.in_scale, p.out_scale = fptr(in_scale), fptr(out_scale)
    p.groups_per_batch = num_regions if labels is not None else 1
    if labels is not None:
        p.labels, p.Hm, p.Wm = ptr(labels), labels.shape[1], labels.shape[2]
    else:
        p.labels, p.Hm, p.Wm = None, 0, 0
    if noise is not None:
        p.noise, p.noise_w = fptr(noise), fptr(noise_w)
        p.noise_bstride = ho * wo if noise.shape[0] > 1 else 0
        p.noise_per_channel = 1 if noise_per_channel else 0
    else:
        p.noise = p.noise_w = None
        p.noise_bstride = 0
        p.noise_per_channel = 0
    p.bias, p.slope = fptr(bias), None
    p.act, p.alpha, p.gain = act, alpha, gain
    call("e4s_upconv_mfma_f32", ctypes.byref(p), fptr(_f32(k4)), stream())
    return y


def subpixel_weights(w, out=None):
    w = _f32(w)
    cout, cin = w.shape[:2]
    out = _into(out, (cin // 32, cout // 32, 9, 32, 32), w.device)
    call("e4s_subpixel_weights_f32", fptr(w), ptr(out), cout, cin, stream())
    return out


def upconv_bf16x3_eligible(cin, cout):
    return cin % 64 == 0 and cin <= 512 and cout % 32 == 0


def upconv_bf16x3(x, w_sub, cout, k4, *, in_scale=None, out_scale=None, noise=None, noise_w=None, bias=None, act=0,
                  alpha=0.2, gain=LRELU_GAIN, out=None):
    b, hi, wi, cin = x.shape
    ho, wo = 2 * hi, 2 * wi
    y = torch.empty(b, ho, wo, cout, device=x.device, dtype=torch.float32) if out is None else out
    p = ConvParams()
    p.x, p.w, p.y = fptr(x), fptr(w_sub), fptr(y)
    p.y_cstride = y.shape[3] if out is not None else 0
    p.rows = p.tiles = p.meta = None
    p.tiles_cap = 0
    p.B, p.Ha, p.Wa = b, hi, wi
    p.Hi, p.Wi, p.Ho, p.Wo, p.Cin, p.Cout = hi, wi, ho, wo, cin, cout
    p.istride, p.ostride, p.ntaps, p.ncls = 1, 2, 9, 1
    p.in_scale, p.out_scale = fptr(in_scale), fptr(out_scale)
    p.groups_per_batch = 1
    p.labels, p.Hm, p.Wm = None, 0, 0
    if noise is not None:
        p.noise, p.noise_w = fptr(noise), fptr(noise_w)
        p.noise_bstride = ho * wo if noise.shape[0] > 1 else 0
    else:
        p.noise = p.noise_w = None
        p.noise_bstride = 0
    p.noise_per_channel = 0
    p.bias, p.slope = fptr(bias), None
    p.act, p.alpha, p.gain = act, alpha, gain
    call("e4s_upconv_bf16x3_f32", ctypes.byref(p), fptr(_f32(k4)), stream())
    return y


def conv_c32(x, w_split, cout, *, in_scale=None, out_scale=None, noise=None, noise_w=None, bias=None, act=0, alpha=0.2,
             gain=LRELU_GAIN, rgb_ws=None):
    b, h, w, cin = x.shape
    if cin != 32 or cout % 32:
        raise RuntimeError("conv_c32: Cin == 32 and Cout % 32 == 0")
    y = torch.empty(b, h, w, cout, device=x.device, dtype=torch.float32)
    p = ConvParams()
    p.x, p.w, p.y = fptr(x), fptr(w_split), fptr(y)
    p.y_cstride = 0
    p.rows = p.tiles = p.meta = None
    p.tiles_cap = 0
    p.B, p.Ha, p.Wa = b, h, w
    p.Hi, p.Wi, p.Ho, p.Wo, p.Cin, p.Cout = h, w, h, w, cin, cout
    p.istride, p.ostride, p.ntaps, p.ncls = 1, 1, 9, 1
    p.in_scale, p.out_scale = fptr(in_scale), fptr(out_scale)
    p.groups_per_batch = 1
    p.labels, p.Hm, p.Wm = None, 0, 0
    if noise is not None:
        p.noise, p.noise_w = fptr(noise), fptr(noise_w)
        p.noise_bstride = h * w if noise.shape[0] > 1 else 0
    else:
        p.noise = p.noise_w = None
        p.noise_bstride = 0
    p.noise_per_channel = 0
    p.bias, p.slope = fptr(bias), None
    p.act, p.alpha, p.gain = act, alpha, gain
    partial = None
    if rgb_ws is not None:
        if cout != 32 or tuple(rgb_ws.shape) != (b, 3, 32):
            raise RuntimeError("conv_c32: the fused ToRGB partial needs Cout == 32 and rgb_ws [B,3,32]")
        partial = torch.empty(b, 3, h, w, device=x.device, dtype=torch.float32)
    call("e4s_conv_c32_bf16x3_f32", ctypes.byref(p), fptr(rgb_ws), fptr(partial), stream())
    return y if partial is None else (y, partial)


def torgb_finish(partial, bias, skip, k4):
    b, _, h, w = partial.shape
    out = torch.empty_like(partial)
    call("e4s_torgb_finish_f32", fptr(partial), fptr(_f32(bias)), fptr(skip), fptr(_f32(k4)) if skip is not None else None,
         fptr(out), b, h, w, stream())
    return out


def torgb(x, ws, bias, skip, k4, labels, num_regions):
    b, h, w, cin = x.shape
    out = torch.empty(b, 3, h, w, device=x.device, dtype=torch.float32)
    hm = wm = 0
    if labels is not None:
        hm, wm = labels.shape[1:]
    call("e4s_torgb_f32", fptr(x), fptr(ws), fptr(bias), fptr(skip), fptr(k4), ptr(labels), hm, wm, num_regions,
         fptr(out), b, h, w, cin, stream())
    return out


def mask_mul_add(y, mask, r, out, channels_last):
    if channels_last:
        b, h, w, c = y.shape
    else:
        b, c, h, w = y.shape
    acc = 1 if out is not None else 0
    if out is None:
        out = torch.empty_like(y)
    mask = _f32(mask)
    call("e4s_mask_mul_add_f32", fptr(y), fptr(mask), fptr(out), r, b, h, w, c, mask.shape[1], mask.shape[2],
         mask.shape[3], 1 if channels_last else 0, acc, stream())
    return out


def noise_bias_act_nhwc(x, noise, noise_w, bias, alpha, gain):
    b, h, w, c = x.shape
    y = torch.empty_like(x)
    nb = 0 if noise is None or noise.shape[0] == 1 else h * w
    call("e4s_noise_bias_act_nhwc_f32", fptr(x), fptr(noise), fptr(noise_w) if noise is not None else None, nb,
         fptr(bias), fptr(y), b, h * w, c, float(alpha), float(gain), stream())
    return y


def resize_bilinear_to_nhwc(x, ho, wo):
    x = _f32(x)
    b, c, hi, wi = x.shape
    y = torch.empty(b, ho, wo, c, device=x.device, dtype=torch.float32)
    call("e4s_resize_bilinear_f32", fptr(x), fptr(y), b, c, hi, wi, ho, wo, stream())
    return y


def conv3x3_small(x, w, want_stats=False):
    b, h, wd, cin = x.shape
    cout = w.shape[0]
    y = torch.empty(b, h, wd, cout, device=x.device, dtype=torch.float32)
    if cin == 3 and cout == 64 and h % 16 == 0 and wd % 16 == 0:
        slots = (h // 16) * (wd // 16)
        fused = torch.empty(b * cout * slots * 2, device=x.device, dtype=torch.float64) if want_stats else None
        call("e4s_conv3x3_stem_f32", fptr(x), fptr(_f32(w)), fptr(y), ptr(fused), b, h, wd, cin, cout, stream())
        if not want_stats:
            return y
        stats = torch.empty(b, cout, 2, device=x.device, dtype=torch.float32)
        call("e4s_instnorm_finalize_f32", ptr(fused), fptr(stats), None, b, h * wd, cout, slots, 1e-5, stream())
        return y, stats
    call("e4s_conv3x3_small_f32", fptr(x), fptr(w), fptr(y), b, h, wd, cin, cout, stream())
    if want_stats:
        return y, instnorm_stats(y)[0]
    return y


def instnorm_stats(x, want_pooled=False, eps=1e-5):
    b, h, w, c = x.shape
    stats = torch.empty(b, c, 2, device=x.device, dtype=torch.float32)
    pooled = torch.empty(b, c, device=x.device, dtype=torch.float32) if want_pooled else None
    ws = torch.empty(lib.load().e4s_instnorm_ws_doubles(b, h * w, c), device=x.device, dtype=torch.float64)
    call("e4s_instnorm_stats_f32", fptr(x), fptr(stats), fptr(pooled), ptr(ws), b, h * w, c, float(eps), stream())
    return stats, pooled


def instnorm_apply(x, stats, gate=None, res=None, res_stats=None, slope=None, rs=1, want_stats=False):
    b, h, w, c = x.shape
    y = torch.empty_like(x)
    if want_stats and c % 64 == 0:
        ws = torch.empty(lib.load().e4s_instnorm_ws_doubles(b, h * w, c), device=x.device, dtype=torch.float64)
        nslots = ctypes.c_int(0)
        call("e4s_instnorm_apply_stats_f32", fptr(x), fptr(stats), fptr(gate), fptr(res), fptr(res_stats), fptr(slope),
             fptr(y), ptr(ws), ctypes.byref(nslots), b, h, w, c, rs, stream())
        out_stats = torch.empty(b, c, 2, device=x.device, dtype=torch.float32)
        call("e4s_instnorm_finalize_f32", ptr(ws), fptr(out_stats), None, b, h * w, c, nslots.value, 1e-5, stream())
        return y, out_stats
    call("e4s_instnorm_apply_f32", fptr(x), fptr(stats), fptr(gate), fptr(res), fptr(res_stats), fptr(slope), fptr(y),
         b, h, w, c, rs, stream())
    if want_stats:
        return y, instnorm_stats(y)[0]
    return y


def se_gate(pooled, fc1, fc2):
    b, c = pooled.shape
    cr = fc1.shape[0]
    gate = torch.empty(b, c, device=pooled.device, dtype=torch.float32)
    call("e4s_se_gate_f32", fptr(pooled), fptr(fc1), fptr(fc2), fptr(gate), b, c, cr, stream())
    return gate


def region_mean_into(feats, labels, out, num_regions, out_off):
    b, h, w, c = feats.shape
    hm, wm = labels.shape[1:]
    nws = lib.load().e4s_region_mean_ws_floats(b, h * w, c, num_regions)
    ws = torch.empty(nws, device=feats.device, dtype=torch.float32) if nws else None
    call("e4s_region_mean_f32", fptr(feats), ptr(labels), hm, wm, fptr(out), fptr(ws), b, h, w, c, num_regions,
         out.shape[2], out_off, stream())


def grouped_linear(x, w, bias, add, scale, act=0, alpha=0.01):
    b, r, k = x.shape
    o = w.shape[1]
    y = torch.empty(b, r, o, device=x.device, dtype=torch.float32)
    call("e4s_grouped_linear_f32", fptr(x), fptr(w), fptr(bias), fptr(add), fptr(y), b, r, k, o, float(scale), act,
         float(alpha), stream())
    return y


def grouped_linear_t(g, w, scale, base=None, mul=None, ref=None, alpha=1.0):
    b, r, o = g.shape
    k = w.shape[2]
    out = torch.empty(b, r, k, device=g.device, dtype=torch.float32)
    for lo in range(0, b, 16):
        n = min(16, b - lo)
        ws = torch.empty(lib.load().e4s_grouped_linear_t_ws_floats(n, r, o, k), device=g.device, dtype=torch.float32)
        sl = slice(lo, lo + n)
        call("e4s_grouped_linear_t_f32", fptr(g[sl]), fptr(w), fptr(out[sl]), fptr(ws), n, r, o, k, float(scale),
             fptr(base[sl]) if base is not None else None, fptr(mul[sl]) if mul is not None else None,
             fptr(ref[sl]) if ref is not None else None, float(alpha), stream())
    return out


STYLE_GRAD_MULTI = os.environ.get("E4S_STYLE_GRAD_MULTI", "1") != "0"


def style_grad_multi(jobs, b, r, nl, sdim, device):
    if len(jobs) > lib.STYLE_GRAD_MAX_JOBS:
        raise RuntimeError(f"{len(jobs)} style-gradient jobs: the ABI carries at most {lib.STYLE_GRAD_MAX_JOBS}")
    arr = (lib.StyleGradJob * max(len(jobs), 1))()
    ws = torch.empty(sum(j["G"] * j["Cin"] for j in jobs), device=device, dtype=torch.float32)
    outs, keep, off = [], [], 0
    for q, j in zip(arr, jobs):
        n = j["G"] * j["Cin"]
        out = ws[off:off + n].view(j["G"], j["Cin"])
        off += n
        outs.append(out)
        rgb = "dws" in j
        for name in (("dws", "w3") if rgb else ("ds_raw", "dd_d", "d", "s", "wsq")) + ("wmod",):
            t = _f32(j[name])
            keep.append(t)
            setattr(q, name, fptr(t).value)
        q.ds_total = fptr(out).value
        q.conv_scale = float(j.get("conv_scale", 0.0))
        q.mod_scale = float(j["mod_scale"])
        q.G, q.Cin, q.Cout, q.slot, q.masked = j["G"], j["Cin"], j.get("Cout", 0), j["slot"], int(j["masked"])
    dlat = torch.empty(b, r, nl, sdim, device=device, dtype=torch.float32)
    call("e4s_style_grad_multi_f32", ctypes.cast(arr, ctypes.c_void_p), len(jobs), fptr(dlat), b, r, nl, sdim, stream())
    return dlat, outs


def grouped_outer(g, h, scale):
    b, r, o = g.shape
    k = h.shape[2]
    dw = torch.empty(r, o, k, device=g.device, dtype=torch.float32)
    call("e4s_grouped_outer_f32", fptr(g), fptr(h), fptr(dw), b, r, o, k, float(scale), stream())
    return dw


def batch_sum(x):
    x = _f32(x)
    out = torch.empty(x.shape[1:], device=x.device, dtype=torch.float32)
    call("e4s_batch_sum_f32", fptr(x), fptr(out), x.shape[0], out.numel(), stream())
    return out


def colsum(x):
    x = _f32(x)
    c = x.shape[-1]
    rows = x.numel() // c
    if rows <= 64 or c % 4 or c > 1024:
        return batch_sum(x.view(rows, c))
    out = torch.empty(c, device=x.device, dtype=torch.float32)
    ws = torch.empty(lib.load().e4s_colsum_ws_floats(rows, c), device=x.device, dtype=torch.float32)
    call("e4s_colsum_f32", fptr(x), fptr(out), fptr(ws), rows, c, stream())
    return out


def sum_all(x):
    x = _f32(x)
    n = x.numel()
    if n % 4 == 0 and n // 4 > 64:
        return colsum(x.view(-1, 4)).sum()
    return x.sum()


def adam_step(p, grad, m, v, lr, beta1, beta2, eps, weight_decay, step):
    call("e4s_adam_step_f32", fptr(p), fptr(_f32(grad)), fptr(m), fptr(v), p.numel(), float(lr), float(beta1), float(beta2),
         float(eps), float(weight_decay), int(step), stream())


def _ptr_array(tensors, dtype=torch.float32):
    arr = (ctypes.c_void_p * len(tensors))()
    for i, t in enumerate(tensors):
        if t.dtype != dtype or not t.is_cuda or not t.is_contiguous():
            raise RuntimeError(f"multi-tensor call: contiguous {dtype} ROCm tensors expected")
        arr[i] = t.data_ptr()
    return arr


def advance_steps(steps):
    if steps.dtype != torch.int64 or not steps.is_cuda:
        raise RuntimeError("advance_steps: device int64 tensor")
    call("e4s_advance_i64", ptr(steps), steps.numel(), stream())


def adam_step_dev(p, grad, m, v, lr, beta1, beta2, eps, weight_decay, step, lr_dev=None):
    if step.dtype != torch.int64 or not step.is_cuda:
        raise RuntimeError("adam_step_dev: step must be a device int64 tensor")
    if lr_dev is not None and (lr_dev.dtype != torch.float64 or not lr_dev.is_cuda):
        raise RuntimeError("adam_step_dev: lr_dev must be a device float64 tensor")
    call("e4s_adam_step_dev_f32", fptr(p), fptr(_f32(grad)), fptr(m), fptr(v), p.numel(), float(lr), ptr(lr_dev), float(beta1),
         float(beta2), float(eps), float(weight_decay), ptr(step), stream())


def adam_multi_dev(ps, grads, ms, vs, steps, lr, beta1, beta2, eps, weight_decay, lr_dev=None):
    n = len(ps)
    if not (n == len(grads) == len(ms) == len(vs) == len(steps)):
        raise RuntimeError("adam_multi_dev: list lengths differ")
    if lr_dev is not None and (lr_dev.dtype != torch.float64 or not lr_dev.is_cuda):
        raise RuntimeError("adam_multi_dev: lr_dev must be a device float64 tensor")
    for p, g in zip(ps, grads):
        if g.shape != p.shape:
# ... 633 lines not shown
```

### e4s_amd/lib.py

```python
import ctypes
import os

import torch

_HERE = os.path.dirname(os.path.abspath(__file__))
LIB_PATH = os.environ.get("E4S_LIB_PATH") or os.path.join(_HERE, "libe4s_hip.so")
ABI_VERSION = 18

c_p = ctypes.c_void_p
c_i = ctypes.c_int
c_l = ctypes.c_int64
c_f = ctypes.c_float
c_d = ctypes.c_double


STYLE_GRAD_MAX_JOBS = 32


class StyleGradJob(ctypes.Structure):
    _fields_ = [
        ("ds_raw", c_p), ("dd_d", c_p), ("d", c_p), ("s", c_p), ("wsq", c_p), ("dws", c_p), ("w3", c_p), ("wmod", c_p), ("ds_total", c_p),
        ("conv_scale", c_f), ("mod_scale", c_f), ("G", c_i), ("Cin", c_i), ("Cout", c_i), ("slot", c_i), ("masked", c_i),
    ]


class ConvParams(ctypes.Structure):
    _fields_ = [
        ("x", c_p), ("w", c_p), ("y", c_p), ("rows", c_p), ("tiles", c_p), ("meta", c_p), ("tiles_cap", c_i),
        ("B", c_i), ("Ha", c_i), ("Wa", c_i),
        ("Hi", c_i), ("Wi", c_i), ("Ho", c_i), ("Wo", c_i), ("Cin", c_i), ("Cout", c_i),
        ("istride", c_i), ("ostride", c_i), ("ntaps", c_i), ("ncls", c_i),
        ("in_scale", c_p), ("out_scale", c_p), ("groups_per_batch", c_i),
        ("labels", c_p), ("Hm", c_i), ("Wm", c_i),
        ("noise", c_p), ("noise_w", c_p), ("noise_bstride", c_l), ("noise_per_channel", c_i),
        ("bias", c_p), ("slope", c_p), ("act", c_i), ("alpha", c_f), ("gain", c_f),
        ("in_stats", c_p), ("y_cstride", c_i), ("splitk_ws", c_p), ("stats_ws", c_p), ("stats_slots", c_i), ("tap_shift", c_i),
        ("split_hint", c_i),
    ]


class ConvBwdParams(ctypes.Structure):
    _fields_ = [
        ("gz", c_p), ("wt", c_p), ("dx", c_p), ("x", c_p), ("ds", c_p), ("s", c_p), ("d", c_p), ("labels", c_p),
        ("Hm", c_i), ("Wm", c_i), ("R", c_i),
        ("B", c_i), ("Hx", c_i), ("Wx", c_i), ("Cx", c_i), ("Hy", c_i), ("Wy", c_i), ("Cy", c_i),
        ("ncls", c_i), ("ds_ws", c_p),
    ]


class ConvWgradParams(ctypes.Structure):
    _fields_ = [
        ("gz", c_p), ("x", c_p), ("dw", c_p), ("ws", c_p), ("s", c_p), ("d", c_p), ("labels", c_p),
        ("Hm", c_i), ("Wm", c_i), ("R", c_i),
        ("B", c_i), ("Hi", c_i), ("Wi", c_i), ("Cin", c_i), ("Ha", c_i), ("Wa", c_i), ("Ho", c_i), ("Wo", c_i), ("Cout", c_i),
        ("istride", c_i), ("ostride", c_i), ("py", c_i), ("px", c_i), ("ntaps", c_i), ("tap_shift", c_i),
    ]


class RrdbParams(ctypes.Structure):
    _fields_ = [
        ("x", c_p), ("w", c_p), ("bias", c_p), ("y", c_p), ("r0", c_p), ("r1", c_p),
        ("B", c_i), ("Hi", c_i), ("Wi", c_i), ("Cin", c_i),
        ("x_cstride", c_i), ("y_cstride", c_i), ("y_coff", c_i),
        ("r0_cstride", c_i), ("r0_coff", c_i), ("r1_cstride", c_i), ("r1_coff", c_i),
        ("epilogue", c_i), ("up2", c_i), ("precision", c_i),
        ("s0", c_f), ("s1", c_f), ("slope", c_f),
    ]


SIGNATURES = {
    "e4s_fused_bias_act_f32": [c_p, c_p, c_p, c_p, c_l, c_i, c_i, c_i, c_i, c_f, c_f, c_p],
    "e4s_upfirdn2d_f32": [c_p, c_p, c_p] + [c_i] * 14 + [c_p],
    "e4s_channel_sum_f32": [c_p, c_p, c_l, c_i, c_i, c_p],
    "e4s_rowdot_f32": [c_p, c_l, c_p, c_p, c_p, c_i, c_i, c_i, c_i, c_f, c_p],
    "e4s_weight_sqsum_f32": [c_p, c_p, c_i, c_i, c_i, c_p],
    "e4s_pack_taps_f32": [c_p, c_p, c_i, c_i, c_i, c_p],
    "e4s_polyphase_weights_f32": [c_p, c_p, c_p, c_i, c_i, c_p],
    "e4s_polyphase_fold_f32": [c_p, c_p, c_p, c_i, c_i, c_p],
    "e4s_rgb_weights_f32": [c_p, c_p, c_p, c_i, c_i, c_f, c_p],
    "e4s_mask_labels": [c_p, c_p, c_p, c_i, c_i, c_i, c_i, c_p],
    "e4s_region_plan": [c_p] + [c_i] * 8 + [c_p, c_p, c_p, c_p, c_i, c_i, c_p],
    "e4s_conv_mfma_f32": [ctypes.POINTER(ConvParams), c_i, c_p],
    "e4s_upconv_mfma_f32": [ctypes.POINTER(ConvParams), c_p, c_p],
    "e4s_conv_bf16x3_f32": [ctypes.POINTER(ConvParams), c_p],
    "e4s_conv_bf16x3_ws_floats": [ctypes.POINTER(ConvParams)],
    "e4s_conv_mfma_ws_floats": [ctypes.POINTER(ConvParams), c_i],
    "e4s_split_bf16x2_f32": [c_p, c_p, c_l, c_i, c_p],
    "e4s_conv_region_bf16x3_f32": [ctypes.POINTER(ConvParams), c_p, c_p],
    "e4s_conv_region_ws_floats": [ctypes.POINTER(ConvParams)],
    "e4s_conv_region_path": [ctypes.POINTER(ConvParams)],
    "e4s_split16_bytes": [ctypes.c_int64, c_i, c_i],
    "e4s_split16_bf16x2_f32": [c_p, c_p, c_l, c_i, c_i, c_p],
    "e4s_upconv_blocks_per_cu": [],
    "e4s_instnorm_ws_doubles": [c_i, c_i, c_i],
    "e4s_conv_bwd_mfma_f32": [ctypes.POINTER(ConvBwdParams), c_p],
    "e4s_pack_taps_bwd_f32": [c_p, c_p, c_i, c_i, c_i, c_p],
    "e4s_demod_grad_f32": [c_p, c_p, c_p, c_p, c_l, c_p, c_f, c_f, c_p, c_i, c_i, c_i, c_p, c_p, c_i, c_i, c_i, c_i, c_p],
    "e4s_torgb_bwd_w_f32": [c_p, c_p, c_p, c_i, c_i, c_i, c_p, c_p, c_i, c_i, c_i, c_i, c_p],
    "e4s_conv_bwd_ws_floats": [ctypes.POINTER(ConvBwdParams)],
    "e4s_seg_reduce_nsplit": [c_i, c_i, c_i, c_i],
    "e4s_grouped_linear_t_f32": [c_p, c_p, c_p, c_p, c_i, c_i, c_i, c_i, c_f, c_p, c_p, c_p, c_f, c_p],
    "e4s_grouped_linear_t_ws_floats": [c_i, c_i, c_i, c_i],
    "e4s_reduce_parts_f32": [c_p, c_p, c_i, c_l, c_f, c_p],
    "e4s_reduce_parts_ws_floats": [c_i, c_l],
    "e4s_grouped_outer_f32": [c_p, c_p, c_p, c_i, c_i, c_i, c_i, c_f, c_p],
    "e4s_style_grad_multi_f32": [c_p, c_i, c_p, c_i, c_i, c_i, c_i, c_p],
    "e4s_swap_styles_f32": [c_p, c_p, c_p, c_i, c_i, c_i, ctypes.c_uint, c_i, c_i, c_i, c_p],
    "e4s_batch_sum_f32": [c_p, c_p, c_i, c_l, c_p],
    "e4s_adam_step_f32": [c_p, c_p, c_p, c_p, c_l, c_d, c_d, c_d, c_d, c_d, c_i, c_p],
    "e4s_subpixel_weights_f32": [c_p, c_p, c_i, c_i, c_p],
    "e4s_upconv_bf16x3_f32": [c_p, c_p, c_p],
    "e4s_colsum_f32": [c_p, c_p, c_p, c_l, c_i, c_p],
    "e4s_colsum_ws_floats": [c_l, c_i],
    "e4s_scale_dot_f32": [c_p, c_p, c_p, c_p, c_p, c_i, c_l, c_i, c_p],
    "e4s_scale_dot_ws_floats": [c_i, c_l, c_i],
    "e4s_mask_to_u8": [c_p, c_p, c_i, c_i, c_i, c_i, c_i, c_p],
    "e4s_erode_u8": [c_p, c_p, c_i, c_i, c_i, c_i, c_i, c_p],
    "e4s_gaussian_blur_u8": [c_p, c_p, c_i, c_i, c_i, c_i, ctypes.POINTER(c_i), c_p],
    "e4s_alpha_composite_u8": [c_p, c_p, c_p, c_p, c_i, c_i, c_i, c_p],
    "e4s_pyrdown_u8": [c_p, c_p, c_i, c_i, c_i, c_i, c_p],
    "e4s_pyrdown_f32": [c_p, c_p, c_i, c_i, c_i, c_i, c_p],
    "e4s_pyrup_f32": [c_p, c_p, c_i, c_i, c_i, c_i, c_p],
    "e4s_u8_to_f32": [c_p, c_p, c_l, c_p],
    "e4s_lap_level_f32": [c_p, c_p, c_p, c_p, c_p, c_p, c_p, c_l, c_i, c_p],
    "e4s_clip_u8": [c_p, c_p, c_l, c_p],
    "e4s_conv_c32_bf16x3_f32": [c_p, c_p, c_p, c_p],
    "e4s_torgb_finish_f32": [c_p, c_p, c_p, c_p, c_p, c_i, c_i, c_i, c_p],
    "e4s_rowdot_multi_f32": [c_p, c_i, c_p, c_p, c_i, c_i, c_i, c_p],
    "e4s_ema_f32": [c_p, c_p, c_l, c_d, c_p],
    "e4s_adam_step_dev_f32": [c_p, c_p, c_p, c_p, c_l, c_d, c_p, c_d, c_d, c_d, c_d, c_p, c_p],
    "e4s_advance_i64": [c_p, c_l, c_p],
    "e4s_conv_smallcin_col2im_f32": [c_p, c_p] + [c_i] * 10 + [c_p],
    "e4s_region_scale_f32": [c_p, c_p, c_p, c_i, c_i, c_i, c_p, c_i, c_i, c_i, c_i, c_i, c_p],
    "e4s_col2im_region_nsplit": [c_i, c_i, c_i, c_i],
    "e4s_col2im_region_f32": [c_p, c_p, c_p, c_p, c_i, c_i, c_i, c_p, c_p, c_p, c_i, c_i, c_i, c_i, c_i, c_p],
    "e4s_act_bwd_demod_nsplit": [c_i, c_i, c_i, c_i],
    "e4s_act_bwd_demod_f32": [c_p, c_p, c_p, c_p, c_p, c_l, c_p, c_f, c_f, c_p, c_i, c_i, c_i, c_p, c_p, c_i, c_i, c_i, c_i, c_p],
    "e4s_pixel_unshuffle2_f32": [c_p, c_p, c_i, c_i, c_i, c_i, c_p],
    "e4s_wino_weights_bytes": [c_i, c_i],
    "e4s_wino_weights_f32": [c_p, c_p, c_i, c_i, c_p],
    "e4s_conv_wino_covers": [c_p],
    "e4s_conv_wino_ws_floats": [c_p],
    "e4s_conv_wino_bf16x3_f32": [c_p, c_p],
    "e4s_adam_multi_dev_f32": [c_i, c_p, c_p, c_p, c_p, c_p, c_p, c_d, c_p, c_d, c_d, c_d, c_d, c_p],
    "e4s_ema_multi_f32": [c_i, c_p, c_p, c_p, c_d, c_p],
    "e4s_torgb_bwd_x_f32": [c_p, c_p, c_p, c_i, c_i, c_i, c_p, c_i, c_i, c_i, c_i, c_i, c_p],
    "e4s_shift_scale_f32": [c_p, c_p, c_p, c_i, c_i, c_i, c_p] + [c_i] * 12 + [c_p],
    "e4s_torgb_f32": [c_p, c_p, c_p, c_p, c_p, c_p, c_i, c_i, c_i, c_p, c_i, c_i, c_i, c_i, c_p],
    "e4s_mask_mul_add_f32": [c_p, c_p, c_p] + [c_i] * 10 + [c_p],
    "e4s_noise_bias_act_nhwc_f32": [c_p, c_p, c_p, c_l, c_p, c_p, c_i, c_i, c_i, c_f, c_f, c_p],
    "e4s_nchw_to_nhwc_f32": [c_p, c_p, c_i, c_i, c_i, c_i, c_p],
    "e4s_nhwc_to_nchw_f32": [c_p, c_p, c_i, c_i, c_i, c_i, c_p],
    "e4s_const_input_f32": [c_p, c_p, c_i, c_i, c_i, c_i, c_p],
    "e4s_resize_bilinear_f32": [c_p, c_p] + [c_i] * 6 + [c_p],
    "e4s_conv3x3_small_f32": [c_p, c_p, c_p] + [c_i] * 5 + [c_p],
    "e4s_conv3x3_stem_f32": [c_p, c_p, c_p, c_p] + [c_i] * 5 + [c_p],
    "e4s_instnorm_stats_f32": [c_p, c_p, c_p, c_p, c_i, c_i, c_i, c_f, c_p],
    "e4s_instnorm_finalize_f32": [c_p, c_p, c_p, c_i, c_i, c_i, c_i, c_f, c_p],
    "e4s_instnorm_apply_stats_f32": [c_p] * 9 + [c_i] * 5 + [c_p],
    "e4s_instnorm_apply_f32": [c_p] * 7 + [c_i] * 5 + [c_p],
    "e4s_se_gate_f32": [c_p, c_p, c_p, c_p, c_i, c_i, c_i, c_p],
    "e4s_instnorm_finalize_se_f32": [c_p, c_p, c_p, c_p, c_p, c_i, c_i, c_i, c_i, c_i, c_f, c_p],
    "e4s_region_mean_f32": [c_p, c_p, c_i, c_i, c_p, c_p] + [c_i] * 7 + [c_p],
    "e4s_region_mean_ws_floats": [c_i, c_i, c_i, c_i],
    "e4s_conv_wgrad_f32": [ctypes.POINTER(ConvWgradParams), c_p],
    "e4s_conv_wgrad_ws_floats": [ctypes.POINTER(ConvWgradParams)],
    "e4s_conv_wgrad_path": [ctypes.POINTER(ConvWgradParams)],
    "e4s_instnorm_bwd_f32": [c_p, c_p, c_p, c_p, c_p, c_p, c_p, c_i, c_i, c_i, c_i, c_p],
    "e4s_instnorm_bwd_ws_doubles": [c_i, c_i, c_i],
    "e4s_prelu_f32": [c_p, c_p, c_p, c_l, c_i, c_p],
    "e4s_prelu_bwd_f32": [c_p, c_p, c_p, c_p, c_p, c_p, c_l, c_i, c_p],
    "e4s_prelu_bwd_ws_floats": [c_l, c_i],
    "e4s_strided_scatter_f32": [c_p, c_p, c_i, c_i, c_i, c_i, c_i, c_i, c_p],
    "e4s_strided_place_f32": [c_p, c_p] + [c_i] * 9 + [c_p],
    "e4s_region_mean_bwd_f32": [c_p, c_p, c_i, c_i, c_p, c_p, c_i, c_i, c_i, c_i, c_i, c_i, c_i, c_i, c_p],
    "e4s_conv1x1_small_f32": [c_p, c_p, c_p, c_p, c_i, c_i, c_i, c_i, c_i, c_f, c_i, c_f, c_f, c_p],
    "e4s_noise_half_f32": [c_p, c_p, c_p, c_p, c_l, c_i, c_i, c_i, c_f, c_f, c_p],
    "e4s_pixelnorm_f32": [c_p, c_p, c_i, c_i, c_p],
    "e4s_add_scale_f32": [c_p, c_p, c_p, c_f, c_l, c_p],
    "e4s_minibatch_stddev_f32": [c_p, c_p, c_i, c_i, c_i, c_i, c_i, c_p],
    "e4s_onehot_u8_f32": [c_p, c_p, c_i, c_i, c_i, c_i, c_p],
    "e4s_swap_head_mask_u8": [c_p, c_p, c_p, c_p, c_l, c_p],
    "e4s_foreground_mask_f32": [c_p, c_p, c_p, c_l, c_p],
    "e4s_morph_f32": [c_p, c_p, c_p, c_i, c_i, c_i, c_i, c_p],
    "e4s_create_masks_f32": [c_p, c_p, c_p, c_p, c_i, c_i, c_i, c_i, c_i, c_p],
    "e4s_tensor2im_u8": [c_p, c_p, c_i, c_i, c_i, c_p],
    "e4s_stream_copy_u8": [c_p, c_p, ctypes.c_int64, c_i, c_p],
    "e4s_paste_u8": [c_p, c_p, c_p, c_p, c_i, c_i, c_i, c_i, c_i, c_p],
    "e4s_grouped_linear_f32": [c_p, c_p, c_p, c_p, c_p, c_i, c_i, c_i, c_i, c_f, c_i, c_f, c_p],
    "e4s_adaptive_pool_f32": [c_p, c_p] + [c_i] * 11 + [c_p, c_p, c_p],
    "e4s_adaptive_pool_bwd_f32": [c_p, c_p] + [c_i] * 11 + [c_p, c_i, c_p],
    "e4s_conv_smallcin_f32": [c_p, c_p, c_p, c_p] + [c_i] * 11 + [c_p],
    "e4s_conv_smallcin_bwd_f32": [c_p, c_p, c_p] + [c_i] * 10 + [c_p],
    "e4s_maxpool3s2_f32": [c_p, c_p, c_p, c_i, c_i, c_i, c_i, c_p],
    "e4s_maxpool3s2_bwd_f32": [c_p, c_p, c_p, c_i, c_i, c_i, c_i, c_p],
    "e4s_maxpool2_f32": [c_p, c_p, c_p, c_i, c_i, c_i, c_i, c_p],
    "e4s_maxpool2_bwd_f32": [c_p, c_p, c_p, c_i, c_i, c_i, c_i, c_p],
    "e4s_relu_bwd_f32": [c_p, c_p, c_p, c_l, c_i, c_p],
    "e4s_lpips_layer_f32": [c_p, c_p, c_p, c_p, c_p, c_i, c_i, c_i, c_p],
    "e4s_lpips_layer_ws_doubles": [c_i, c_i],
    "e4s_lpips_layer_bwd_f32": [c_p, c_p, c_p, c_p, c_f, c_p, c_i, c_i, c_i, c_i, c_p],
    "e4s_instnorm_bwd_sums_f32": [c_p, c_p, c_p, c_p, c_p, c_i, c_i, c_i, c_p],
    "e4s_norm_bwd_frozen_f32": [c_p, c_p, c_p, c_p, c_p, c_i, c_i, c_i, c_i, c_p],
    "e4s_cosine_f32": [c_p, c_p, c_p, c_p, c_i, c_l, c_p],
    "e4s_cosine_ws_doubles": [c_i, c_l],
    "e4s_cosine_bwd_f32": [c_p, c_p, c_p, c_p, c_f, c_p, c_i, c_l, c_i, c_p],
    "e4s_parser_preprocess_f32": [c_p, c_i, c_p, c_i, c_i, c_i, ctypes.POINTER(c_f), c_p],
    "e4s_maxpool3s2p1_f32": [c_p, c_p, c_i, c_i, c_i, c_i, c_p],
    "e4s_add_relu_f32": [c_p, c_p, c_p, c_l, c_i, c_i, c_i, c_p],
    "e4s_mean_hw_f32": [c_p, c_p, c_i, c_i, c_i, c_p],
    "e4s_parser_fc_f32": [c_p, c_p, c_p, c_p, c_i, c_i, c_i, c_i, c_f, c_p],
    "e4s_gate_add_up2_f32": [c_p, c_p, c_p, c_i, c_p, c_i, c_i, c_i, c_i, c_p],
    "e4s_parser_head_f32": [c_p] + [c_i] * 8 + [c_p, c_p, c_p, c_p],
    "e4s_quad_crop_u8": [c_p, c_p, c_p, c_p, c_p, c_i, c_i, c_i, c_i, c_p],
    "e4s_perspective_paste_u8": [c_p, c_p, c_p, c_p, c_i, c_i, c_i, c_i, c_p],
    "e4s_rrdb_conv_f32": [ctypes.POINTER(RrdbParams), c_p],
    "e4s_rrdb_pack_f32": [c_p, c_p, c_i, c_i, c_p],
    "e4s_rrdb_pack_bytes": [c_i],
    "e4s_rrdb_head_f32": [c_p, c_i, c_i, c_p, c_p, c_p, c_i, c_p, c_i, c_i, c_i, c_i, c_p],
    "e4s_rrdb_tail_f32": [c_p, c_i, c_p, c_p, c_p, c_i, c_p, c_i, c_i, c_i, c_i, c_p],
}

INT64_RETURN = {"e4s_split16_bytes", "e4s_instnorm_ws_doubles", "e4s_conv_bwd_ws_floats", "e4s_grouped_linear_t_ws_floats", "e4s_reduce_parts_ws_floats", "e4s_instnorm_bwd_ws_doubles", "e4s_prelu_bwd_ws_floats", "e4s_conv_wgrad_ws_floats", "e4s_conv_bf16x3_ws_floats", "e4s_conv_region_ws_floats", "e4s_lpips_layer_ws_doubles", "e4s_conv_mfma_ws_floats",
                "e4s_cosine_ws_doubles", "e4s_region_mean_ws_floats", "e4s_colsum_ws_floats", "e4s_scale_dot_ws_floats", "e4s_wino_weights_bytes", "e4s_conv_wino_ws_floats", "e4s_rrdb_pack_bytes"}

_lib = None


def load():
    global _lib
    if _lib is not None:
        return _lib
    if not os.path.isfile(LIB_PATH):
        raise RuntimeError(f"{LIB_PATH} not found: run `python -m e4s_amd.build` (hipcc, gfx950). "
                           "e4s_amd has no CPU / eager fallback.")
    lib = ctypes.CDLL(LIB_PATH)
    lib.e4s_abi_version.restype = c_i
    lib.e4s_build_arch.restype = ctypes.c_char_p
    if lib.e4s_abi_version() != ABI_VERSION:
        raise RuntimeError("libe4s_hip.so ABI version mismatch: rebuild with `python -m e4s_amd.build --force`")
    for name, argtypes in SIGNATURES.items():
        fn = getattr(lib, name)
        fn.argtypes = argtypes
        fn.restype = c_l if name in INT64_RETURN else c_i
    _lib = lib
    return lib


def stream():
    return c_p(torch.cuda.current_stream().cuda_stream)


def ptr(t):
    if t is None:
        return None
    if not t.is_cuda:
        raise RuntimeError("e4s_amd kernels need tensors on a ROCm device (no CPU fallback)")
    if not t.is_contiguous():
        raise RuntimeError("e4s_amd kernels need contiguous tensors")
    return c_p(t.data_ptr())


def fptr(t):
    if t is not None and t.dtype != torch.float32:
        raise RuntimeError(f"expected float32, got {t.dtype}")
    return ptr(t)


def check(code, what):
    if code != 0:
        raise RuntimeError(f"{what} failed: hipError {code}")


def call(name, *args):
    check(getattr(load(), name)(*args), name)
```

### e4s_amd/networks.py

```python
import math

import torch
from torch import nn

from . import kernels as K
from .encoders import FSEncoder_PSP
from .packs import param_key
from .stylegan2 import EqualLinear, Generator


class LocalMLP(nn.Module):

    def __init__(self, dim_component=512, dim_style=512, num_w_layers=18, latent_squeeze_ratio=1):
        super().__init__()
        self.dim_component, self.dim_style, self.num_w_layers = dim_component, dim_style, num_w_layers
        self.mlp = nn.Sequential(EqualLinear(dim_component, dim_style // latent_squeeze_ratio, lr_mul=1),
                                 nn.LeakyReLU(),
                                 EqualLinear(dim_style // latent_squeeze_ratio, dim_style * num_w_layers, lr_mul=1))

    def forward(self, x):
        l0, l2 = self.mlp[0], self.mlp[2]
        h = K.grouped_linear(x.unsqueeze(1).contiguous(), l0.weight.unsqueeze(0), l0.bias.unsqueeze(0), None,
                             l0.scale, act=1, alpha=self.mlp[1].negative_slope)
        y = K.grouped_linear(h, l2.weight.unsqueeze(0), l2.bias.unsqueeze(0), None, l2.scale)
# ... 43 lines not shown
    def _encoder_needs_grad(self, img):
        if not torch.is_grad_enabled():
            return False
        if img.requires_grad:
            raise NotImplementedError("gradients w.r.t. the input image of the regional encoder are not implemented "
                                      "(parameter gradients are: e4s_amd/encoder_autograd.py)")
        return any(p.requires_grad for p in self.encoder.parameters())

    def get_style_vectors(self, img, mask):
        train = self._encoder_needs_grad(img)
        with torch.no_grad():
            labels, flags = K.mask_labels(mask)
            if self.G.strict_mask and not torch.cuda.is_current_stream_capturing() and bool(flags.item()):
                raise NotImplementedError("get_style_vectors needs a one-hot parsing mask (labelMap2OneHot); the "
                                          "regional pooling of soft masks is not implemented")
            x256 = K.resize_bilinear_to_nhwc(img, 256, 256)
            if not train:
                codes, last = self.encoder.encode_nhwc(x256, labels, mask.shape[1])
                b, h, w, c = last.shape
                return codes, torch.zeros(b, c, h, w, device=img.device, dtype=torch.float32)
        from .encoder_autograd import EncoderFn
        params = [p for p in self.encoder.parameters() if p.requires_grad]
        codes = EncoderFn.apply(self.encoder, x256, labels, mask.shape[1], *params)
        return codes, torch.zeros(img.shape[0], 512, 16, 16, device=img.device, dtype=torch.float32)

    def cal_style_codes(self, style_vectors):
        if not self.opts.start_from_latent_avg or self.opts.learn_in_w:
            raise NotImplementedError("only start_from_latent_avg=True, learn_in_w=False (the shipped configs)")
        K_ = self.remaining_layer_idx
        nw = K_ if K_ != 17 else 18
        if torch.is_grad_enabled() and any(p.requires_grad for m in self.MLPs for p in m.parameters()):
            w0 = torch.stack([m.mlp[0].weight for m in self.MLPs])
            b0 = torch.stack([m.mlp[0].bias for m in self.MLPs])
            w2 = torch.stack([m.mlp[2].weight for m in self.MLPs])
            b2 = torch.stack([m.mlp[2].bias for m in self.MLPs])
        else:
            w0, b0, w2, b2 = self._mlp_weights()
        b, r, _ = style_vectors.shape
        lat = self.latent_avg.to(device=style_vectors.device, dtype=torch.float32)
        add = lat[:nw].reshape(-1).contiguous()
        from .autograd import StyleCodesFn
        codes = StyleCodesFn.apply(style_vectors, w0, b0, w2, b2, add).view(b, r, nw, 512)
        if K_ != 17:
            rest = lat[K_:].view(1, 1, -1, 512).expand(b, r, -1, -1)
            codes = torch.cat([codes, rest], dim=2)
        return codes

    def gen_img(self, struc_codes, style_codes, mask, randomize_noise=True, noise=None, return_latents=False):
        images, result_latent, feats = self.G([style_codes], struc_codes, mask, input_is_latent=True,
                                              randomize_noise=randomize_noise, noise=noise,
                                              return_latents=return_latents, use_structure_code=False)
        if return_latents:
            return images, result_latent, feats
        return images, -1, feats

    def forward(self, img, mask, resize=False, randomize_noise=True, return_latents=False):
        sv, struct = self.get_style_vectors(img, mask)
        codes = self.cal_style_codes(sv)
        images, latent, feats = self.G([codes], struct, mask, input_is_latent=True, randomize_noise=randomize_noise,
                                       return_latents=return_latents, use_structure_code=False)
        if return_latents:
            return images, feats, latent
        return images, feats


_SWAP_SEL = {}


def swap_comp_style_vector(style_vectors1, style_vectors2, comp_indices, belowFace_interpolation=False):
    r = style_vectors1.shape[1]
    if (style_vectors1.is_cuda and style_vectors1.dtype == torch.float32 and style_vectors2.dtype == torch.float32
            and style_vectors2.device == style_vectors1.device and style_vectors2.shape == style_vectors1.shape and 9 < r <= 32):
        return K.swap_styles(style_vectors1, style_vectors2, comp_indices, belowFace_interpolation)
    key = (style_vectors1.device, r, tuple(sorted(comp_indices)))
    sel = _SWAP_SEL.get(key)
    if sel is None:
        sel = torch.zeros(1, r, 1, dtype=torch.bool)
        sel[0, list(key[2]), 0] = True
        sel = _SWAP_SEL[key] = sel.to(style_vectors1.device)
    out = torch.where(sel, style_vectors2, style_vectors1)
    no_ear = (style_vectors2[:, 7].sum(1, keepdim=True) == 0)
    out[:, 7] = torch.where(no_ear, (style_vectors1[:, 7] + style_vectors2[:, 7]) / 2, out[:, 7])
    no_teeth = (style_vectors2[:, 9].sum(1, keepdim=True) == 0)
    out[:, 9] = torch.where(no_teeth, style_vectors1[:, 9], out[:, 9])
    if belowFace_interpolation:
        out[:, 8] = (style_vectors1[:, 8] + style_vectors2[:, 8]) / 2
    return out


@torch.no_grad()
def face_swap_core(net, driven, driven_mask, target, target_mask, swapped_mask, noise=None, randomize_noise=False):
    b = driven.shape[0]

    def stacked(a, c):
        if (a.is_contiguous() and c.is_contiguous() and a.shape == c.shape and a.dtype == c.dtype
                and a.untyped_storage().data_ptr() == c.untyped_storage().data_ptr()
                and c.storage_offset() == a.storage_offset() + a.numel()):
            return a.as_strided((2 * a.shape[0],) + tuple(a.shape[1:]), a.stride(), a.storage_offset())
        return torch.cat([a, c], 0)
    sv, _ = net.get_style_vectors(stacked(driven, target), stacked(driven_mask, target_mask))
    d_sv, t_sv = sv[:b], sv[b:]
    comp = set(range(net.opts.num_seg_cls)) - {0, 4, 11, 10}
    swapped = swap_comp_style_vector(t_sv, d_sv, comp)
    codes = net.cal_style_codes(swapped)
    img, _, _ = net.gen_img(None, codes, swapped_mask, randomize_noise=randomize_noise, noise=noise)
    return img


class GraphedFaceSwap:

    def __init__(self, net, batch, img_size=1024, mask_size=512, noise_batch=None):
        dev = next(net.parameters()).device
        self.net, self.batch = net, batch
        r = net.opts.num_seg_cls
        imgs = torch.zeros(2 * batch, 3, img_size, img_size, device=dev)
        masks = torch.zeros(2 * batch, r, mask_size, mask_size, device=dev)
        self.static = [imgs[:batch], masks[:batch], imgs[batch:], masks[batch:],
                       torch.zeros(batch, r, mask_size, mask_size, device=dev)]
        for m in self.static[1::2] + [self.static[4]]:
            m[:, 0] = 1.0
        nb = batch if noise_batch is None else noise_batch
        self.noise = [torch.zeros(nb, 1, n.shape[2], n.shape[3], device=dev) for n in net.G.make_noise()]
        self.flags = torch.zeros(1, device=dev, dtype=torch.int32)
        self.graph = None
        self.out = None

    def _load(self, driven, dm, target, tm, sm, noise):
        for dst, src in zip(self.static, (driven, dm, target, tm, sm)):
            dst.copy_(src)
        for dst, src in zip(self.noise, noise):
            dst.copy_(src)

    def __call__(self, driven, dm, target, tm, sm, noise):
        self._load(driven, dm, target, tm, sm, noise)
        return self.replay()

    def load(self, driven, dm, target, tm, sm, noise):
        self._load(driven, dm, target, tm, sm, noise)

    def replay(self):
        if self.graph is None:
            side = torch.cuda.Stream()
            side.wait_stream(torch.cuda.current_stream())
            with torch.cuda.stream(side):
                for _ in range(2):
                    face_swap_core(self.net, *self.static, noise=self.noise)
            torch.cuda.current_stream().wait_stream(side)
            torch.cuda.synchronize()
            self.graph = torch.cuda.CUDAGraph()
            mode = "thread_local" if (torch.distributed.is_available() and torch.distributed.is_initialized()) else "global"
            from .shard import quiesce_before_capture
            quiesce_before_capture()
            with K.flag_sink(self.flags):
                with torch.cuda.graph(self.graph, capture_error_mode=mode):
                    self.out = face_swap_core(self.net, *self.static, noise=self.noise)
        self.graph.replay()
        return self.out

    def validate(self):
        bad = bool(self.flags.item())
        self.flags.zero_()
        if bad:
            raise RuntimeError("GraphedFaceSwap was replayed with a parsing mask that is not one-hot: its outputs used "
                               "hard argmax regions; run face_swap_core eagerly for soft masks")
```

### e4s_amd/stylegan2.py

```python
import math
import os
import random

import torch
from torch import nn
from torch.nn import functional as F

from . import kernels as K
from .op import FusedLeakyReLU, fused_leaky_relu, upfirdn2d, conv2d_gradfix


UPCONV_EXACT = os.environ.get("E4S_UPCONV", "exact") != "polyphase"
UPCONV_EXACT_MIN_RES = int(os.environ.get("E4S_UPCONV_MIN_RES", "256"))
UPCONV_BF16X3_EXACT = os.environ.get("E4S_UPCONV_BF16X3", "exact") != "polyphase"
CONV_C32 = os.environ.get("E4S_CONV_C32", "1") != "0"
REGION_ROWS = os.environ.get("E4S_REGION_ROWS", "1") != "0"


def make_kernel(k):
    k = torch.tensor(k, dtype=torch.float32)
    if k.ndim == 1:
        k = k[None, :] * k[:, None]
    return k / k.sum()


class PixelNorm(nn.Module):
    def forward(self, input):
        return input * torch.rsqrt(torch.mean(input ** 2, dim=1, keepdim=True) + 1e-8)


class Upsample(nn.Module):

    def __init__(self, kernel, factor=2):
        super().__init__()
        self.factor = factor
        self.register_buffer("kernel", make_kernel(kernel) * (factor ** 2))
        p = self.kernel.shape[0] - factor
        self.pad = ((p + 1) // 2 + factor - 1, p // 2)

    def forward(self, input):
        return upfirdn2d(input, self.kernel, up=self.factor, down=1, pad=self.pad)


class Downsample(nn.Module):

    def __init__(self, kernel, factor=2):
        super().__init__()
        self.factor = factor
        self.register_buffer("kernel", make_kernel(kernel))
        p = self.kernel.shape[0] - factor
        self.pad = ((p + 1) // 2, p // 2)

    def forward(self, input):
        return upfirdn2d(input, self.kernel, up=1, down=self.factor, pad=self.pad)


class Blur(nn.Module):

    def __init__(self, kernel, pad, upsample_factor=1):
        super().__init__()
        kernel = make_kernel(kernel)
        if upsample_factor > 1:
            kernel = kernel * (upsample_factor ** 2)
        self.register_buffer("kernel", kernel)
        self.pad = pad

    def forward(self, input):
        return upfirdn2d(input, self.kernel, pad=self.pad)


class EqualConv2d(nn.Module):

    def __init__(self, in_channel, out_channel, kernel_size, stride=1, padding=0, bias=True):
        super().__init__()
        self.weight = nn.Parameter(torch.randn(out_channel, in_channel, kernel_size, kernel_size))
        self.scale = 1 / math.sqrt(in_channel * kernel_size ** 2)
        self.stride, self.padding = stride, padding
        self.bias = nn.Parameter(torch.zeros(out_channel)) if bias else None

    def forward(self, input):
        return conv2d_gradfix.conv2d(input, self.weight * self.scale, bias=self.bias, stride=self.stride,
                                     padding=self.padding)


class EqualLinear(nn.Module):

    def __init__(self, in_dim, out_dim, bias=True, bias_init=0, lr_mul=1, activation=None):
        super().__init__()
        self.weight = nn.Parameter(torch.randn(out_dim, in_dim).div_(lr_mul))
        self.bias = nn.Parameter(torch.zeros(out_dim).fill_(bias_init)) if bias else None
        self.activation = activation
        self.scale = (1 / math.sqrt(in_dim)) * lr_mul
        self.lr_mul = lr_mul

    def forward(self, input):
        if self.activation:
            out = F.linear(input, self.weight * self.scale)
            return fused_leaky_relu(out, self.bias * self.lr_mul)
        return F.linear(input, self.weight * self.scale, bias=self.bias * self.lr_mul)


class ScaledLeakyReLU(nn.Module):
    def __init__(self, negative_slope=0.2):
        super().__init__()
        self.negative_slope = negative_slope

    def forward(self, input):
        return F.leaky_relu(input, negative_slope=self.negative_slope) * math.sqrt(2)


def polyphase_upconv_weights(w, blur_kernel):
    cout, cin = w.shape[:2]
    kf = torch.flip(blur_kernel, [0, 1])
    e = F.conv2d(F.pad(w.reshape(cout * cin, 1, 3, 3), (3, 3, 3, 3)), kf[None, None]).reshape(cout, cin, 6, 6)
    phases = []
    for py in range(2):
        for px in range(2):
            iy = [py + 4 - 2 * ey for ey in range(3)]
            ix = [px + 4 - 2 * ex for ex in range(3)]
            sub = e[:, :, iy][:, :, :, ix]
            phases.append(sub.permute(2, 3, 0, 1).reshape(9, cout, cin))
    return torch.stack(phases, 0).contiguous()


from .packs import param_key as _param_key


class ModulatedConv2d(nn.Module):

    def __init__(self, in_channel, out_channel, kernel_size, style_dim, demodulate=True, upsample=False,
                 downsample=False, blur_kernel=[1, 3, 3, 1], fused=True):
        super().__init__()
        self.eps = 1e-8
        self.kernel_size = kernel_size
        self.in_channel, self.out_channel = in_channel, out_channel
        self.upsample, self.downsample = upsample, downsample
        if downsample:
            raise NotImplementedError("downsampling ModulatedConv2d is never instantiated by E4S")
        if upsample:
            factor = 2
            p = (len(blur_kernel) - factor) - (kernel_size - 1)
            self.blur = Blur(blur_kernel, pad=((p + 1) // 2 + factor - 1, p // 2 + 1), upsample_factor=factor)
        self.scale = 1 / math.sqrt(in_channel * kernel_size ** 2)
        self.padding = kernel_size // 2
        self.weight = nn.Parameter(torch.randn(1, out_channel, in_channel, kernel_size, kernel_size))
        self.modulation = EqualLinear(style_dim, in_channel, bias_init=1)
        self.demodulate = demodulate
        self.fused = fused
        self._pack = None

    def _buf(self, name, shape, device):
        bufs = self.__dict__.setdefault("_e4s_bufs", {})
        t = bufs.get(name)
        if t is None or tuple(t.shape) != tuple(shape) or t.device != device:
            t = torch.empty(shape, device=device, dtype=torch.float32)
            bufs[name] = t
        return t

    def packed(self):
        key = _param_key(self.weight) + ((_param_key(self.blur.kernel)) if self.upsample else ())
        if self._pack is not None and self._pack["key"] == key:
            return self._pack
        with torch.no_grad():
            w = self.weight.detach()[0].float()
            cout, cin, k, _ = w.shape
            dev = w.device
            pack = {"key": key}
            if k == 1:
                pack["w"] = w.reshape(1, 1, cout, cin).contiguous()
# ... 45 lines not shown
        s = K.modulate_vec(style, self.modulation.weight, self.modulation.bias)
        if self.kernel_size == 1:
            if self.out_channel != 3 or self.demodulate:
                raise NotImplementedError("1x1 ModulatedConv2d exists only as the ToRGB conv (model.py:417)")
            ws = K.rgb_weights(pk["w"].view(3, -1), s, self.scale)
            zero = torch.zeros(3, device=x.device)
            return K.torgb(x, ws, zero, None, None, None, 1)
        else:
            d = K.demod_coefs(s, pk["wsq"], self.scale) if self.demodulate else \
                torch.full((b, self.out_channel), self.scale, device=x.device)
            if self.upsample:
                y = K.conv_mfma(x, pk["w"], self.out_channel, ncls=4, ostride=2, in_scale=s, out_scale=d)
            else:
                y = K.conv_mfma(x, pk["w"], self.out_channel, in_scale=s, out_scale=d)
        return K.nhwc_to_nchw(y)


class NoiseInjection(nn.Module):
    def __init__(self):
        super().__init__()
        self.weight = nn.Parameter(torch.zeros(1))

    def forward(self, image, noise=None):
        if noise is None:
            b, _, h, w = image.shape
            noise = image.new_empty(b, 1, h, w).normal_()
        return image + self.weight * noise


class ConstantInput(nn.Module):
    def __init__(self, channel, size=4):
        super().__init__()
        self.input = nn.Parameter(torch.randn(1, channel, size, size))

    def forward(self, input):
        return self.input.repeat(input.shape[0], 1, 1, 1)


def _prep_noise(noise, b, h, w, device):
    if noise is None:
        return torch.randn(b, 1, h, w, device=device), False
    noise = noise.to(device=device, dtype=torch.float32)
    if noise.ndim != 4 or noise.shape[2] != h or noise.shape[3] != w or noise.shape[0] not in (1, b):
        raise RuntimeError(f"noise of shape {tuple(noise.shape)} is not broadcastable to [{b},C,{h},{w}]")
    if noise.shape[1] == 1:
        return noise.contiguous(), False
    return K.nchw_to_nhwc(noise), True


class StyledConv(nn.Module):

    def __init__(self, in_channel, out_channel, kernel_size, style_dim, upsample=False, blur_kernel=[1, 3, 3, 1],
                 demodulate=True, mask_op=False):
        super().__init__()
        self.conv = ModulatedConv2d(in_channel, out_channel, kernel_size, style_dim, upsample=upsample,
                                    blur_kernel=blur_kernel, demodulate=demodulate)
        self.noise = NoiseInjection()
        self.activate = FusedLeakyReLU(out_channel)
        self.mask_op = mask_op

    def c32_eligible(self, b, h, w, labels=None, plan=None):
        conv = self.conv
        return (CONV_C32 and not conv.upsample and labels is None and plan is None and conv.in_channel == 32
                and conv.out_channel % 32 == 0 and K.want_bf16x3(b, h, w, 32, conv.out_channel))

    def run_nhwc(self, x, s, noise, labels=None, num_regions=1, plan=None, rec=None, rgb_ws=None, d=None):
        conv = self.conv
        pk = conv.packed()
        b, h, w, _ = x.shape
        ho, wo = (2 * h, 2 * w) if conv.upsample else (h, w)
        if d is None:
            d = K.demod_coefs(s, pk["wsq"], conv.scale)
        nz, per_ch = _prep_noise(noise, b, ho, wo, x.device)
        if rec is not None:
            if per_ch:
                raise NotImplementedError("backward with per-channel noise maps")
            rec.update(d=d, noise=nz)
        ncls = 4 if conv.upsample else 1
        if not per_ch and self.c32_eligible(b, h, w, labels, plan):
            return K.conv_c32(x, conv.split_weights(), conv.out_channel, in_scale=s, out_scale=d, noise=nz,
                              noise_w=self.noise.weight, bias=self.activate.bias, act=1, alpha=self.activate.negative_slope,
                              gain=self.activate.scale, rgb_ws=rgb_ws)
        if rgb_ws is not None:
            raise RuntimeError("the fused ToRGB partial exists only on the Cin == 32 kernel")
        if (conv.upsample and labels is None and plan is None and not per_ch and UPCONV_BF16X3_EXACT
                and K.upconv_bf16x3_eligible(conv.in_channel, conv.out_channel)
                and K.want_bf16x3(b, h, w, conv.in_channel, conv.out_channel, ncls, masked=False)):
            return K.upconv_bf16x3(x, conv.subpixel_split_weights(), conv.out_channel, conv.blur.kernel, in_scale=s,
                                   out_scale=d, noise=nz, noise_w=self.noise.weight, bias=self.activate.bias, act=1,
                                   alpha=self.activate.negative_slope, gain=self.activate.scale)
        if plan is None and not per_ch and K.want_bf16x3(b, h, w, conv.in_channel, conv.out_channel, ncls,
                                                         masked=labels is not None):
            return K.conv_mfma(x, pk["w"], conv.out_channel, labels=labels, num_regions=num_regions, ncls=ncls,
                               ostride=2 if conv.upsample else 1, in_scale=s, out_scale=d, noise=nz,
                               noise_w=self.noise.weight, bias=self.activate.bias, act=1,
                               alpha=self.activate.negative_slope, gain=self.activate.scale,
                               w_split=conv.split_weights(),
                               w_split16=conv.split_weights16() if (labels is not None and REGION_ROWS) else None)
        if conv.upsample and plan is None and UPCONV_EXACT and (labels is None or ho >= UPCONV_EXACT_MIN_RES):
            return K.upconv_mfma(x, pk["w3"], conv.out_channel, conv.blur.kernel, in_scale=s, out_scale=d,
                                 labels=labels, num_regions=num_regions, noise=nz, noise_w=self.noise.weight,
                                 noise_per_channel=per_ch, bias=self.activate.bias, act=1,
                                 alpha=self.activate.negative_slope, gain=self.activate.scale)
        return K.conv_mfma(x, pk["w"], conv.out_channel, plan=plan, labels=None if plan is not None else labels,
                           num_regions=num_regions, ncls=4 if conv.upsample else 1,
                           ostride=2 if conv.upsample else 1, in_scale=s, out_scale=d, noise=nz,
                           noise_w=self.noise.weight, noise_per_channel=per_ch, bias=self.activate.bias, act=1,
                           alpha=self.activate.negative_slope, gain=self.activate.scale)

    def run_nhwc_soft(self, x, s, noise, mask):
        conv = self.conv
        pk = conv.packed()
        b, h, w, _ = x.shape
        r = mask.shape[1]
        ho, wo = (2 * h, 2 * w) if conv.upsample else (h, w)
        d = K.demod_coefs(s, pk["wsq"], conv.scale)
        s3, d3 = s.view(b, r, -1), d.view(b, r, -1)
        acc = None
        for i in range(r):
            y = K.conv_mfma(x, pk["w"], conv.out_channel, ncls=4 if conv.upsample else 1,
                            ostride=2 if conv.upsample else 1, in_scale=s3[:, i].contiguous(),
                            out_scale=d3[:, i].contiguous())
            acc = K.mask_mul_add(y, mask, i, acc, True)
        nz, per_ch = _prep_noise(noise, b, ho, wo, x.device)
        if per_ch:
            raise NotImplementedError("per-channel noise with soft masks")
        return K.noise_bias_act_nhwc(acc, nz, self.noise.weight, self.activate.bias, self.activate.negative_slope,
                                     self.activate.scale)

    def forward(self, input, style, mask, noise=None, use_plan=False):
        x = K.nchw_to_nhwc(input)
        b, h, w, _ = x.shape
        mod = self.conv.modulation
        if self.mask_op:
            r = style.shape[1]
            s = K.modulate_vec(style.reshape(b * r, -1), mod.weight, mod.bias)
            labels, _ = K.mask_labels(mask)
            plan = K.region_plan(labels, r, h, w, 4 if self.conv.upsample else 1) if use_plan else None
            return K.nhwc_to_nchw(self.run_nhwc(x, s, noise, labels, r, plan))
        s = K.modulate_vec(style, mod.weight, mod.bias)
        return K.nhwc_to_nchw(self.run_nhwc(x, s, noise))


class ToRGB(nn.Module):

    def __init__(self, in_channel, style_dim, upsample=True, blur_kernel=[1, 3, 3, 1], mask_op=False):
        super().__init__()
        if upsample:
            self.upsample = Upsample(blur_kernel)
        self.conv = ModulatedConv2d(in_channel, 3, 1, style_dim, demodulate=False)
        self.bias = nn.Parameter(torch.zeros(1, 3, 1, 1))
        self.mask_op = mask_op

    def run_nhwc(self, x, s, labels, num_regions, skip, rec=None):
        pk = self.conv.packed()
        ws = K.rgb_weights(pk["w"].view(3, -1), s, self.conv.scale)
        if rec is not None:
            rec.update(ws=ws)
        k4 = self.upsample.kernel if skip is not None else None
        return K.torgb(x, ws, self.bias, skip, k4, labels, num_regions)

    def run_nhwc_soft(self, x, s, mask, skip):
        pk = self.conv.packed()
        b = x.shape[0]
        r = mask.shape[1]
        ws = K.rgb_weights(pk["w"].view(3, -1), s, self.conv.scale).view(b, r, 3, -1)
        zero3 = torch.zeros(3, device=x.device)
        acc = None
        for i in range(r):
            y = K.torgb(x, ws[:, i].contiguous(), zero3, None, None, None, 1)
            acc = K.mask_mul_add(y, mask, i, acc, False)
        zw = torch.zeros(b, 3, x.shape[3], device=x.device)
        k4 = self.upsample.kernel if skip is not None else None
        tail = K.torgb(x, zw, self.bias, skip, k4, None, 1)
        return acc + tail

    def forward(self, input, style, mask, skip=None):
        x = K.nchw_to_nhwc(input)
        b = x.shape[0]
        mod = self.conv.modulation
        if self.mask_op:
            r = style.shape[1]
            s = K.modulate_vec(style.reshape(b * r, -1), mod.weight, mod.bias)
            labels, _ = K.mask_labels(mask)
            return self.run_nhwc(x, s, labels, r, skip)
        s = K.modulate_vec(style, mod.weight, mod.bias)
        return self.run_nhwc(x, s, None, 1, skip)


class Generator(nn.Module):

    def __init__(self, size, style_dim, n_mlp, channel_multiplier=2, blur_kernel=[1, 3, 3, 1], lr_mlp=0.01,
                 split_layer_idx=7, remaining_layer_idx=18):
        super().__init__()
        self.split_layer_idx = split_layer_idx
        self.remaining_layer_idx = remaining_layer_idx
        self.size = size
        self.style_dim = style_dim
        layers = [PixelNorm()]
        for _ in range(n_mlp):
            layers.append(EqualLinear(style_dim, style_dim, lr_mul=lr_mlp, activation="fused_lrelu"))
        self.style = nn.Sequential(*layers)
        self.channels = {4: 512, 8: 512, 16: 512, 32: 512, 64: 256 * channel_multiplier,
                         128: 128 * channel_multiplier, 256: 64 * channel_multiplier,
                         512: 32 * channel_multiplier, 1024: 16 * channel_multiplier}
        self.input = ConstantInput(self.channels[4])
        self.conv1 = StyledConv(self.channels[4], self.channels[4], 3, style_dim, blur_kernel=blur_kernel,
                                mask_op=True)
        self.to_rgb1 = ToRGB(self.channels[4], style_dim, upsample=False, mask_op=True)
        self.log_size = int(math.log(size, 2))
        self.num_layers = (self.log_size - 2) * 2 + 1
        self.convs = nn.ModuleList()
        self.upsamples = nn.ModuleList()
        self.to_rgbs = nn.ModuleList()
        self.noises = nn.Module()
        in_channel = self.channels[4]
        for layer_idx in range(self.num_layers):
            res = (layer_idx + 5) // 2
            self.noises.register_buffer(f"noise_{layer_idx}", torch.randn(1, 1, 2 ** res, 2 ** res))
        K_ = self.remaining_layer_idx
        for i in range(3, self.log_size + 1):
            out_channel = self.channels[2 ** i]
            conv_masked = not (i > 2 + K_ // 2)
            rgb_masked = not (K_ != 17 and i >= 2 + K_ // 2)
            self.convs.append(StyledConv(in_channel, out_channel, 3, style_dim, upsample=True,
                                         blur_kernel=blur_kernel, mask_op=conv_masked))
            self.convs.append(StyledConv(out_channel, out_channel, 3, style_dim, blur_kernel=blur_kernel,
                                         mask_op=conv_masked))
            self.to_rgbs.append(ToRGB(out_channel, style_dim, mask_op=rgb_masked))
            in_channel = out_channel
        self.n_latent = self.log_size * 2 - 2
        self.strict_mask = True

    def make_noise(self):
        device = self.input.input.device
        noises = [torch.randn(1, 1, 4, 4, device=device)]
        for i in range(3, self.log_size + 1):
            for _ in range(2):
                noises.append(torch.randn(1, 1, 2 ** i, 2 ** i, device=device))
        return noises

    def mean_latent(self, n_latent):
        latent_in = torch.randn(n_latent, self.style_dim, device=self.input.input.device)
        return self.get_latent(latent_in).mean(0, keepdim=True)

    def _style_is_canonical(self):
        ok = getattr(self, "_e4s_style_ok", None)
        if ok is None:
            mods = list(self.style)
            ok = (len(mods) >= 2 and isinstance(mods[0], PixelNorm)
                  and all(isinstance(m, EqualLinear) and m.activation == "fused_lrelu" and m.bias is not None for m in mods[1:]))
            self._e4s_style_ok = ok
        return ok

    def get_latent(self, input):
        if input.is_cuda and input.ndim == 2 and not (torch.is_grad_enabled() and (
                input.requires_grad or any(p.requires_grad for p in self.style.parameters()))):
            if not self._style_is_canonical():
                return self.style(input)
            with torch.no_grad():
                w = K.pixelnorm(input.to(torch.float32).contiguous())
                for lin in list(self.style)[1:]:
                    w = equal_linear_lrelu(lin, w)
            return w
        return self.style(input)

    def _assemble_latent(self, styles, input_is_latent, inject_index, truncation, truncation_latent):
        if not input_is_latent:
            styles = [self.get_latent(s) for s in styles]
        if truncation < 1:
            styles = [truncation_latent + truncation * (s - truncation_latent) for s in styles]
        if len(styles) < 2:
            if styles[0].ndim < 4:
                return styles[0].unsqueeze(1).repeat(1, self.n_latent, 1)
            return styles[0]
        if inject_index is None:
            inject_index = random.randint(1, self.n_latent - 1)
        l1 = styles[0].unsqueeze(1).repeat(1, inject_index, 1)
        l2 = styles[1].unsqueeze(1).repeat(1, self.n_latent - inject_index, 1)
        return torch.cat([l1, l2], 1)

    def forward(self, styles, structure_feats, mask, return_latents=False, inject_index=None, truncation=1,
                truncation_latent=None, input_is_latent=False, noise=None, randomize_noise=True,
                use_structure_code=False):
        if use_structure_code:
            raise NotImplementedError("use_structure_code=True is never used by E4S (networks.py:112,177)")
        latent = self._assemble_latent(styles, input_is_latent, inject_index, truncation, truncation_latent)
        if latent.ndim != 4:
            raise RuntimeError("E4S generator expects a regional latent [B, R, n_latent, 512]")
        if noise is None:
            noise = [None] * self.num_layers if randomize_noise else \
                [getattr(self.noises, f"noise_{i}") for i in range(self.num_layers)]
        if torch.is_grad_enabled() and any(n is not None and n.requires_grad for n in noise):
            raise NotImplementedError("gradients w.r.t. the injected noise maps are not implemented")
        params = [p for p in self.parameters() if p.requires_grad] if torch.is_grad_enabled() else []
        if any(p is q for q in self.style.parameters() for p in params) and not input_is_latent:
            raise NotImplementedError("gradients of the mapping network G.style (always frozen by Net3, networks.py:68-70)")
        if torch.is_grad_enabled() and (latent.requires_grad or params):
            from .autograd import GeneratorFn
            image, feats = GeneratorFn.apply(self, latent, mask, noise, *params)
        else:
            image, feats = self._fused_forward(latent, mask, noise)
        return (image, latent, feats) if return_latents else (image, None, feats)

    def _style_plan(self, b, r, nlat, dev):
        layers = [(self.conv1, 0, "conv"), (self.to_rgb1, 1, "rgb")]
        i = 1
        for c1, c2, tr in zip(self.convs[::2], self.convs[1::2], self.to_rgbs):
            layers += [(c1, i, "conv"), (c2, i + 1, "conv"), (tr, i + 2, "rgb")]
            i += 2
        packs = [l.conv.packed() for l, _, _ in layers]
        key = (b, r, nlat, str(dev)) + tuple(
            (l.conv.modulation.weight.data_ptr(), l.conv.modulation.bias.data_ptr(), pk["wsq"].data_ptr() if pk["wsq"] is not None else 0)
            for (l, _, _), pk in zip(layers, packs))
        plan = getattr(self, "_e4s_style_plan", None)
        if plan is not None and plan["key"] == key:
            return plan
        if torch.cuda.is_current_stream_capturing():
            raise RuntimeError("Generator._style_plan: the job tables of the style prologue must exist before a stream capture "
                               "(run the same shapes once eagerly first -- GraphedStep / GraphedFaceSwap warm up for that)")
        sjobs, djobs, meta, keep = [], [], {}, []
        s_off = d_off = 0
        for layer, idx, kind in layers:
            mod = layer.conv.modulation
            cin = mod.weight.shape[0]
            g = b * r if layer.mask_op else b
            stride = nlat * 512 if layer.mask_op else r * nlat * 512
            w, bs = mod.weight.detach(), mod.bias.detach()
            keep += [w, bs]
            sjobs.append(dict(in_off=idx * 512, in_stride=stride, out_off=s_off, M=w, bias=bs, G=g, O=cin, K=512,
                              scale=1.0 / math.sqrt(512)))
            m = {"s": (s_off, g, cin)}
            if kind == "conv":
                pk = layer.conv.packed()
                cout = layer.conv.out_channel
                keep.append(pk["wsq"])
                djobs.append(dict(in_off=s_off, in_stride=cin, out_off=d_off, M=pk["wsq"], bias=None, G=g, O=cout, K=cin,
                                  scale=layer.conv.scale))
                m["d"] = (d_off, g, cout)
                d_off += g * cout
            s_off += g * cin
            meta[id(layer)] = m
        plan = {"key": key, "s": K.rowdot_jobs(sjobs, dev), "d": K.rowdot_jobs(djobs, dev), "meta": meta, "s_floats": s_off,
                "d_floats": d_off, "keep": keep}
        self._e4s_style_plan = plan
        return plan

    @torch.no_grad()
    def _fused_forward(self, latent, mask, noise, tape=None):
        lat = latent.detach().to(torch.float32).contiguous()
        b, r = lat.shape[:2]
        labels, flags = K.mask_labels(mask)
        soft = False
        if self.strict_mask and not torch.cuda.is_current_stream_capturing():
            soft = bool(flags.item())
        if soft and tape is not None:
            raise NotImplementedError("backward with soft (non one-hot) masks")

        sp = None
        if not soft and lat.shape[3] == 512:
            sp = self._style_plan(b, r, lat.shape[2], lat.device)
            sbuf = torch.empty(sp["s_floats"], device=lat.device, dtype=torch.float32)
            dbuf = torch.empty(sp["d_floats"], device=lat.device, dtype=torch.float32)
            K.rowdot_multi(*sp["s"], lat, sbuf, 0)
            K.rowdot_multi(*sp["d"], sbuf, dbuf, 1)

        def pre(layer, which):
            off, g, c = sp["meta"][id(layer)][which]
            return (sbuf if which == "s" else dbuf)[off:off + g * c].view(g, c)

        def styled(layer, x, idx, nz, rgb_ws=None):
            mod = layer.conv.modulation
            s = pre(layer, "s") if sp is not None else K.modulate(lat, idx, layer.mask_op, mod.weight, mod.bias)
            if soft and layer.mask_op:
                return layer.run_nhwc_soft(x, s, nz, mask)
            rec = {} if tape is not None else None
            y = layer.run_nhwc(x, s, nz, labels if layer.mask_op else None, r, rec=rec, rgb_ws=rgb_ws,
                               d=pre(layer, "d") if sp is not None else None)
            partial = None
            if rgb_ws is not None:
                y, partial = y
            if tape is not None:
                rec.update(kind="conv", layer=layer, idx=idx, masked=layer.mask_op, x=x, y=y, s=s,
                           labels=labels if layer.mask_op else None)
                tape.append(rec)
            return y if rgb_ws is None else (y, partial)

        def styled_then_rgb(conv2, to_rgb, x, idx, nz, skip):
            mod = to_rgb.conv.modulation
            s_rgb = pre(to_rgb, "s") if sp is not None else K.modulate(lat, idx + 1, False, mod.weight, mod.bias)
            ws = K.rgb_weights(to_rgb.conv.packed()["w"].view(3, -1), s_rgb, to_rgb.conv.scale)
            y, partial = styled(conv2, x, idx, nz, rgb_ws=ws)
            out = K.torgb_finish(partial, to_rgb.bias, skip, to_rgb.upsample.kernel if skip is not None else None)
            if tape is not None:
                tape.append(dict(kind="rgb", layer=to_rgb, idx=idx + 1, masked=False, x=y, s=s_rgb, ws=ws,
                                 has_skip=skip is not None, out=out, labels=None))
            return y, out

        def rgb(layer, x, idx, skip):
            mod = layer.conv.modulation
            s = pre(layer, "s") if sp is not None else K.modulate(lat, idx, layer.mask_op, mod.weight, mod.bias)
            if soft and layer.mask_op:
                return layer.run_nhwc_soft(x, s, mask, skip)
            rec = {} if tape is not None else None
            out = layer.run_nhwc(x, s, labels if layer.mask_op else None, r, skip, rec=rec)
            if tape is not None:
                rec.update(kind="rgb", layer=layer, idx=idx, masked=layer.mask_op, x=x, s=s, has_skip=skip is not None, out=out,
                           labels=labels if layer.mask_op else None)
                tape.append(rec)
            return out

        x = K.const_input(self.input.input, b)
        x = styled(self.conv1, x, 0, noise[0])
        skip = rgb(self.to_rgb1, x, 1, None)
        feats = None
        i = 1
        for conv1, conv2, to_rgb in zip(self.convs[::2], self.convs[1::2], self.to_rgbs):
            x = styled(conv1, x, i, noise[i])
            if i + 2 == self.split_layer_idx:
                feats = K.nhwc_to_nchw(x)
                if tape is not None:
                    tape[-1]["is_feats"] = True
            nz2 = noise[i + 1]
            if (not soft and not conv2.mask_op and not to_rgb.mask_op and conv2.conv.out_channel == 32
                    and (nz2 is None or nz2.shape[1] == 1) and conv2.c32_eligible(b, x.shape[1], x.shape[2])):
                x, skip = styled_then_rgb(conv2, to_rgb, x, i + 1, nz2, skip)
            else:
                x = styled(conv2, x, i + 1, nz2)
                skip = rgb(to_rgb, x, i + 2, skip)
            i += 2
        return skip, feats


def _packed_equal_conv(conv, cin_pad):
    key = _param_key(conv.weight) + (cin_pad,)
    pk = getattr(conv, "_e4s_pack", None)
    if pk is None or pk["key"] != key:
        with torch.no_grad():
            w = conv.weight.detach().float() * conv.scale
            cout, cin, k, _ = w.shape
            if cin_pad != cin:
                w = torch.cat([w, w.new_zeros(cout, cin_pad - cin, k, k)], 1)
            pk = {"key": key, "w": K.pack_taps(w.contiguous())}
        conv._e4s_pack = pk
    return pk


def conv_layer_nhwc(layer, x, x_is_nchw=False):
    mods = list(layer)
    i = 0
    blur = None
    if isinstance(mods[0], Blur):
        blur, i = mods[0], 1
    conv = mods[i]
    tail = mods[i + 1] if len(mods) > i + 1 else None
    cout, cin, k, _ = conv.weight.shape
    if isinstance(tail, FusedLeakyReLU):
        bias, act, alpha, gain = tail.bias, 1, tail.negative_slope, tail.scale
    elif isinstance(tail, ScaledLeakyReLU):
        bias, act, alpha, gain = None, 1, tail.negative_slope, math.sqrt(2)
    else:
        bias, act, alpha, gain = conv.bias, 0, 0.2, 1.0
    if x_is_nchw:
        if k != 1 or conv.stride != 1 or cin > 4:
            raise NotImplementedError("NCHW input is only accepted by the 1x1 stem ConvLayer")
        return K.conv1x1_small(x, conv.weight.detach().reshape(cout, cin), bias, conv.scale, act, alpha, gain)
    cx = x.shape[3]
    pk = _packed_equal_conv(conv, cx)
    if cx < cin or cx % 32:
        raise RuntimeError(f"ConvLayer on {cx} channels: need a multiple of 32 >= {cin}")
    kw = dict(bias=bias, act=act, alpha=alpha, gain=gain)
    b, h, w, _ = x.shape

    def split():
        if "w_split" not in pk:
            pk["w_split"] = K.split_bf16x2(pk["w"])
        return pk["w_split"]
    if conv.stride == 1:
        if k != 3 or conv.padding != 1:
            raise NotImplementedError("stride-1 ConvLayers are 3x3 / padding 1 (model.py:701-703)")
        if K.want_bf16x3(b, h, w, cx, cout):
            return K.conv_mfma(x, pk["w"], cout, w_split=split(), **kw)
        return K.conv_mfma(x, pk["w"], cout, **kw)
    if blur is None or conv.stride != 2 or conv.padding != 0 or k not in (1, 3):
        raise NotImplementedError("down-sampling ConvLayers are Blur + stride-2 padding-0 convs (model.py:683-700)")
    xb = K.upfirdn2d_nhwc(x, blur.kernel, pad=blur.pad)
    hb, wb = xb.shape[1:3]
    anchors = ((hb - k) // 2 + 1, (wb - k) // 2 + 1)
    gk = dict(istride=2, ntaps=k * k, anchors=anchors, tap_shift=1 if k == 3 else 0, **kw)
    tiles = (b * anchors[0] * anchors[1] + 255) // 256 * (cout // 128 if cout % 128 == 0 else 0)
    if K.PRECISION != "f32" and cout % 128 == 0 and (K.PRECISION == "bf16x3" or tiles >= K.BF16X3_MIN_BLOCKS):
        return K.conv_mfma(xb, pk["w"], cout, w_split=split(), **gk)
    return K.conv_mfma(xb, pk["w"], cout, **gk)


def equal_linear_lrelu(lin, x):
    w = lin.weight.detach()
    g = math.sqrt(2) if lin.activation else 1.0
    bias = (lin.bias.detach() * (lin.lr_mul * g)).unsqueeze(0) if lin.bias is not None else None
    y = K.grouped_linear(x.unsqueeze(1).contiguous(), w.unsqueeze(0), bias, None, lin.scale * g,
                         act=1 if lin.activation else 0, alpha=0.2)
    return y.squeeze(1)


class ConvLayer(nn.Sequential):

    def __init__(self, in_channel, out_channel, kernel_size, downsample=False, blur_kernel=[1, 3, 3, 1], bias=True,
                 activate=True):
        layers = []
        if downsample:
            factor = 2
            p = (len(blur_kernel) - factor) + (kernel_size - 1)
            layers.append(Blur(blur_kernel, pad=((p + 1) // 2, p // 2)))
            stride, self.padding = 2, 0
        else:
            stride, self.padding = 1, kernel_size // 2
        layers.append(EqualConv2d(in_channel, out_channel, kernel_size, padding=self.padding, stride=stride,
                                  bias=bias and not activate))
        if activate:
            layers.append(FusedLeakyReLU(out_channel) if bias else ScaledLeakyReLU(0.2))
        super().__init__(*layers)


class ResBlock(nn.Module):

    def __init__(self, in_channel, out_channel, blur_kernel=[1, 3, 3, 1]):
        super().__init__()
        self.conv1 = ConvLayer(in_channel, in_channel, 3)
        self.conv2 = ConvLayer(in_channel, out_channel, 3, downsample=True)
        self.skip = ConvLayer(in_channel, out_channel, 1, downsample=True, activate=False, bias=False)

    def forward(self, input):
        out = self.conv2(self.conv1(input))
        return (out + self.skip(input)) / math.sqrt(2)


class Discriminator(nn.Module):

    def __init__(self, size, channel_multiplier=2, blur_kernel=[1, 3, 3, 1]):
        super().__init__()
        channels = {4: 512, 8: 512, 16: 512, 32: 512, 64: 256 * channel_multiplier, 128: 128 * channel_multiplier,
                    256: 64 * channel_multiplier, 512: 32 * channel_multiplier, 1024: 16 * channel_multiplier}
        convs = [ConvLayer(3, channels[size], 1)]
        log_size = int(math.log(size, 2))
        in_channel = channels[size]
        for i in range(log_size, 2, -1):
            out_channel = channels[2 ** (i - 1)]
            convs.append(ResBlock(in_channel, out_channel, blur_kernel))
            in_channel = out_channel
        self.convs = nn.Sequential(*convs)
        self.stddev_group = 4
        self.stddev_feat = 1
        self.final_conv = ConvLayer(in_channel + 1, channels[4], 3)
        self.final_linear = nn.Sequential(EqualLinear(channels[4] * 4 * 4, channels[4], activation="fused_lrelu"),
                                          EqualLinear(channels[4], 1))

    def _needs_autograd(self, input):
        return torch.is_grad_enabled() and (input.requires_grad or any(p.requires_grad for p in self.parameters()))
# ... 26 lines not shown
```

### include/e4s_hip.h

```cpp
#ifndef E4S_HIP_H
#define E4S_HIP_H
#include <stdint.h>

#ifdef __cplusplus
extern "C" {
#endif

int e4s_abi_version(void);
const char* e4s_build_arch(void);


int e4s_fused_bias_act_f32(const float* x, const float* b, const float* ref, float* y, int64_t n,
                           int step_b, int size_b, int act, int grad, float alpha, float scale,
                           void* stream);

int e4s_upfirdn2d_f32(const float* x, const float* k, float* y, int major, int in_h, int in_w, int minor,
                      int kh, int kw, int up_x, int up_y, int down_x, int down_y,
                      int pad_x0, int pad_x1, int pad_y0, int pad_y1, void* stream);

int e4s_channel_sum_f32(const float* g, float* out, int64_t n, int step_b, int size_b, void* stream);


int e4s_rowdot_f32(const float* in, int64_t in_stride, const float* M, const float* bias, float* out,
                   int G, int O, int K, int mode, float scale, void* stream);
typedef struct e4s_rowdot_job {
    int64_t in_off, in_stride, out_off;
    const float* M;
    const float* bias;
    int G, O, K;
    float scale;
} e4s_rowdot_job;
int e4s_rowdot_multi_f32(const e4s_rowdot_job* jobs, int njobs, const float* in_base, float* out_base, int max_O, int max_G,
                         int mode, void* stream);

int e4s_weight_sqsum_f32(const float* w, float* wsq, int cout, int cin, int taps, void* stream);

int e4s_pack_taps_f32(const float* w, float* out, int cout, int cin, int taps, void* stream);
int e4s_polyphase_weights_f32(const float* w, const float* k4, float* out, int cout, int cin, void* stream);
int e4s_polyphase_fold_f32(const float* deff, const float* k4, float* dw, int cout, int cin, void* stream);

int e4s_rgb_weights_f32(const float* w, const float* s, float* ws, int G, int cin, float scale, void* stream);


int e4s_mask_labels(const float* mask, uint8_t* labels, int* flags, int B, int R, int Hm, int Wm, void* stream);

int e4s_region_plan(const uint8_t* labels, int B, int R, int Hm, int Wm, int Ha, int Wa, int nphase,
                    int BM, int* rows, int* tiles, int* meta, int* work, int rows_cap, int tiles_cap,
                    void* stream);


typedef struct {
    const float* x;
    const float* w;
    float* y;
    const int* rows;
    const int* tiles;
    const int* meta;
    int tiles_cap;
    int B, Ha, Wa;
    int Hi, Wi, Ho, Wo, Cin, Cout;
    int istride;
    int ostride;
    int ntaps;
    int ncls;
    const float* in_scale;
    const float* out_scale;
    int groups_per_batch;
    const uint8_t* labels;
    int Hm, Wm;
    const float* noise;
    const float* noise_w;
    int64_t noise_bstride;
    int noise_per_channel;
    const float* bias;
    const float* slope;
    int act;
    float alpha, gain;
    const float* in_stats;
    int y_cstride;
    float* splitk_ws;
    double* stats_ws;
    int stats_slots;
    int tap_shift;
    int split_hint;
} e4s_conv_params;

int e4s_conv_mfma_f32(const e4s_conv_params* p, int spatial, void* stream);
int64_t e4s_conv_mfma_ws_floats(const e4s_conv_params* p, int spatial);

int e4s_upconv_mfma_f32(const e4s_conv_params* p, const float* k4, void* stream);
int e4s_upconv_blocks_per_cu(void);

int e4s_conv_bf16x3_f32(const e4s_conv_params* p, void* stream);
int64_t e4s_conv_bf16x3_ws_floats(const e4s_conv_params* p);
int e4s_split_bf16x2_f32(const float* w, void* out, int64_t rows, int cin, void* stream);

int e4s_conv_region_bf16x3_f32(const e4s_conv_params* p, const void* w16, void* stream);
int64_t e4s_conv_region_ws_floats(const e4s_conv_params* p);
int e4s_conv_region_path(const e4s_conv_params* p);
int e4s_split16_bf16x2_f32(const float* w, void* out, int64_t rows, int cout, int cin, void* stream);
int64_t e4s_split16_bytes(int64_t rows, int cout, int cin);

typedef struct {
    const float* gz;
    const float* wt;
    float* dx;
    const float* x;
    float* ds;
    const float* s;
    const float* d;
    const uint8_t* labels;
    int Hm, Wm, R;
    int B, Hx, Wx, Cx, Hy, Wy, Cy;
    int ncls;
    float* ds_ws;
} e4s_conv_bwd_params;

int e4s_conv_bwd_mfma_f32(const e4s_conv_bwd_params* p, void* stream);
int64_t e4s_conv_bwd_ws_floats(const e4s_conv_bwd_params* p);
typedef struct {
    const float* gz;
    const float* x;
    float* dw;
    float* ws;
    const float* s;
    const float* d;
    const uint8_t* labels;
    int Hm, Wm, R;
    int B, Hi, Wi, Cin, Ha, Wa, Ho, Wo, Cout;
    int istride;
    int ostride, py, px;
    int ntaps;
    int tap_shift;
} e4s_conv_wgrad_params;
int e4s_conv_wgrad_f32(const e4s_conv_wgrad_params* p, void* stream);
int64_t e4s_conv_wgrad_ws_floats(const e4s_conv_wgrad_params* p);
int e4s_conv_wgrad_path(const e4s_conv_wgrad_params* p);
int e4s_pack_taps_bwd_f32(const float* w, float* wt, int ncls, int cout, int cin, void* stream);
int e4s_act_bwd_demod_nsplit(int B, int H, int W, int C);
int e4s_act_bwd_demod_f32(const float* dy, const float* y, float* gz, const float* noise, const float* noise_w, int64_t noise_bstride,
                          const float* bias, float alpha, float gain, const uint8_t* labels, int Hm, int Wm, int R, float* dd, float* ws,
                          int B, int H, int W, int C, void* stream);
int e4s_demod_grad_f32(const float* gz, const float* y, const float* noise, const float* noise_w,
                       int64_t noise_bstride, const float* bias, float alpha, float gain,
                       const uint8_t* labels, int Hm, int Wm, int R, float* dd, float* ws, int B, int H, int W, int C,
                       void* stream);
int e4s_region_scale_f32(const float* gz, const float* d, const uint8_t* labels, int Hm, int Wm, int R, float* u, int B, int H, int W, int C,
                         int ncls, void* stream);
int e4s_col2im_region_nsplit(int B, int H, int W, int C);
int e4s_col2im_region_f32(const float* G, const float* x, const float* s, const uint8_t* labels, int Hm, int Wm, int R, float* dx, float* ds,
                          float* ws, int B, int H, int W, int C, int ncls, void* stream);

int e4s_seg_reduce_nsplit(int B, int H, int W, int C);
int e4s_torgb_bwd_w_f32(const float* drgb, const float* x, const uint8_t* labels, int Hm, int Wm, int R,
                        float* dws, float* ws, int B, int H, int W, int C, void* stream);
int e4s_torgb_bwd_x_f32(const float* drgb, const float* ws, const uint8_t* labels, int Hm, int Wm, int R,
                        float* dx, int B, int H, int W, int C, int accumulate, void* stream);

int e4s_shift_scale_f32(const float* in, const float* tab, const uint8_t* labels, int Hm, int Wm, int R,
                        float* out, int B, int Ha, int Wa, int Hi, int Wi, int C, int istride, int dy, int dx,
                        int os, int py, int px, void* stream);

int e4s_torgb_f32(const float* x, const float* ws, const float* bias, const float* skip, const float* k4,
                  const uint8_t* labels, int Hm, int Wm, int R, float* out,
                  int B, int H, int W, int Cin, void* stream);

int e4s_mask_mul_add_f32(const float* y, const float* mask, float* out, int r, int B, int H, int W, int C,
                         int R, int Hm, int Wm, int channels_last, int accumulate, void* stream);

int e4s_noise_bias_act_nhwc_f32(const float* x, const float* noise, const float* noise_w, int64_t noise_bstride,
                                const float* bias, float* y, int B, int HW, int C, float alpha, float gain,
                                void* stream);

int e4s_instnorm_bwd_f32(const float* dy, const float* x, const float* stats, const float* gate, float* sums, float* dx,
                         double* ws, int B, int HW, int C, int accumulate, void* stream);
int64_t e4s_instnorm_bwd_ws_doubles(int B, int HW, int C);
int e4s_prelu_f32(const float* u, const float* slope, float* y, int64_t npix, int C, void* stream);
int e4s_prelu_bwd_f32(const float* dy, const float* u, const float* slope, float* du, float* dslope, float* ws,
                      int64_t npix, int C, void* stream);
int64_t e4s_prelu_bwd_ws_floats(int64_t npix, int C);
int e4s_pixel_unshuffle2_f32(const float* in, float* out, int B, int H, int W, int C, void* stream);
int e4s_strided_scatter_f32(const float* in, float* out, int B, int H, int W, int C, int s, int accumulate, void* stream);
int e4s_strided_place_f32(const float* in, float* out, int B, int H, int W, int C, int s, int oy, int ox, int Ho, int Wo,
                          void* stream);
int e4s_region_mean_bwd_f32(const float* dcodes, const uint8_t* labels, int Hm, int Wm, int* counts, float* dfeat, int B,
                            int H, int W, int C, int R, int stride, int off, int accumulate, void* stream);

int e4s_conv1x1_small_f32(const float* x, const float* w, const float* bias, float* y, int B, int HW, int Cin, int Cout,
                          int y_cstride, float scale, int act, float alpha, float gain, void* stream);
int e4s_noise_half_f32(const float* feat, const float* noise_w, const float* bias, float* y, int64_t npix, int C,
                       int y_cstride, int coff, float alpha, float gain, void* stream);
int e4s_pixelnorm_f32(const float* x, float* y, int B, int D, void* stream);
int e4s_add_scale_f32(const float* a, const float* b, float* out, float scale, int64_t n, void* stream);
int e4s_minibatch_stddev_f32(const float* x, float* y, int B, int HW, int C, int Cy, int group, void* stream);

int e4s_grouped_linear_t_f32(const float* g, const float* w, float* out, float* ws, int B, int R, int O, int K,
                             float scale, const float* base, const float* mul, const float* ref, float alpha,
                             void* stream);
int64_t e4s_grouped_linear_t_ws_floats(int B, int R, int O, int K);
int e4s_reduce_parts_f32(float* parts, float* out, int nparts, int64_t n, float scale, void* stream);
int64_t e4s_reduce_parts_ws_floats(int nparts, int64_t n);
int e4s_grouped_outer_f32(const float* g, const float* h, float* dw, int B, int R, int O, int K, float scale, void* stream);
#define E4S_STYLE_GRAD_MAX_JOBS 32
typedef struct e4s_style_grad_job {
    const float* ds_raw; const float* dd_d; const float* d; const float* s; const float* wsq;
    const float* dws; const float* w3;
    const float* wmod; float* ds_total;
    float conv_scale, mod_scale;
    int G, Cin, Cout, slot, masked;
} e4s_style_grad_job;
int e4s_style_grad_multi_f32(const e4s_style_grad_job* jobs, int njobs, float* dlat, int B, int R, int NL, int S, void* stream);
int e4s_batch_sum_f32(const float* x, float* out, int B, int64_t n, void* stream);
int e4s_colsum_f32(const float* x, float* out, float* ws, int64_t rows, int C, void* stream);
int64_t e4s_colsum_ws_floats(int64_t rows, int C);
int e4s_scale_dot_f32(float* u, const float* x, const float* s, float* ds, float* ws, int B, int64_t hw, int C, void* stream);
int64_t e4s_scale_dot_ws_floats(int B, int64_t hw, int C);
int e4s_adam_step_f32(float* p, const float* grad, float* m, float* v, int64_t n, double lr, double beta1, double beta2,
                      double eps, double weight_decay, int step, void* stream);
int e4s_adam_step_dev_f32(float* p, const float* grad, float* m, float* v, int64_t n, double lr, const double* lr_dev, double beta1,
                          double beta2, double eps, double weight_decay, const int64_t* step, void* stream);
int e4s_advance_i64(int64_t* steps, int64_t n, void* stream);
int e4s_adam_multi_dev_f32(int count, float* const* p, const float* const* grad, float* const* m, float* const* v, const int64_t* n,
                           const int64_t* const* step, double lr, const double* lr_dev, double beta1, double beta2, double eps,
                           double weight_decay, void* stream);
int e4s_ema_multi_f32(int count, float* const* dst, const float* const* src, const int64_t* n, double decay, void* stream);
int64_t e4s_wino_weights_bytes(int Cout, int Cin);
int e4s_wino_weights_f32(const float* w9, void* out, int Cout, int Cin, void* stream);
int e4s_conv_wino_covers(const e4s_conv_params* p);
int64_t e4s_conv_wino_ws_floats(const e4s_conv_params* p);
int e4s_conv_wino_bf16x3_f32(const e4s_conv_params* p, void* stream);
int e4s_subpixel_weights_f32(const float* w, void* out, int Cout, int Cin, void* stream);
int e4s_upconv_bf16x3_f32(const e4s_conv_params* p, const float* k4, void* stream);

int e4s_conv_c32_bf16x3_f32(const e4s_conv_params* p, const float* rgb_ws, float* rgb_partial, void* stream);
int e4s_torgb_finish_f32(const float* partial, const float* bias, const float* skip, const float* k4, float* out, int B, int H,
                         int W, void* stream);

int e4s_mask_to_u8(const float* mask, uint8_t* out, int B, int H, int W, int Hm, int Wm, void* stream);
int e4s_erode_u8(const uint8_t* src, uint8_t* dst, int B, int H, int W, int radius, int border_value, void* stream);
int e4s_gaussian_blur_u8(const uint8_t* src, uint8_t* dst, int B, int H, int W, int ksize, const int* taps_fixed8, void* stream);
int e4s_alpha_composite_u8(const uint8_t* face, const uint8_t* target, const uint8_t* alpha, uint8_t* out, int B, int H, int W,
                           void* stream);
int e4s_pyrdown_u8(const uint8_t* src, uint8_t* dst, int B, int H, int W, int C, void* stream);
int e4s_pyrdown_f32(const float* src, float* dst, int B, int H, int W, int C, void* stream);
int e4s_pyrup_f32(const float* src, float* dst, int B, int h, int w, int C, void* stream);
int e4s_u8_to_f32(const uint8_t* src, float* dst, int64_t n, void* stream);
int e4s_lap_level_f32(const void* a, const float* ua, const void* b, const float* ub, const float* m, const float* acc,
                      float* out, int64_t n, int a_is_u8, void* stream);
int e4s_clip_u8(const float* src, uint8_t* dst, int64_t n, void* stream);

int e4s_ema_f32(float* dst, const float* src, int64_t n, double decay, void* stream);

int e4s_onehot_u8_f32(const uint8_t* labels, float* out, int B, int R, int H, int W, void* stream);
int e4s_swap_head_mask_u8(const uint8_t* src, const uint8_t* tgt, uint8_t* out, uint8_t* hole, int64_t n, void* stream);
int e4s_foreground_mask_f32(const uint8_t* labels, const uint8_t* hole, float* fg, int64_t n, void* stream);
int e4s_morph_f32(const float* x, float* dil, float* ero, int N, int H, int W, int radius, void* stream);
int e4s_create_masks_f32(const float* mask, float* border, float* full, float* ws, int N, int H, int W, int radius,
                         int operation, void* stream);
int e4s_tensor2im_u8(const float* img, uint8_t* out, int B, int H, int W, void* stream);
int e4s_stream_copy_u8(const void* src, void* dst, int64_t bytes, int blocks, void* stream);
int e4s_paste_u8(const uint8_t* face, const uint8_t* target, const float* mask, uint8_t* out, int B, int H, int W,
                 int Hm, int Wm, void* stream);

int e4s_quad_crop_u8(const uint8_t* frames, const double* coeffs, const int32_t* windows, uint8_t* out, float* normalized, int B,
                     int H, int W, int S, void* stream);
int e4s_perspective_paste_u8(const uint8_t* faces, const uint8_t* frames, const double* coeffs, uint8_t* out, int B, int H, int W,
                             int S, void* stream);

int e4s_nchw_to_nhwc_f32(const float* x, float* y, int B, int C, int H, int W, void* stream);
int e4s_nhwc_to_nchw_f32(const float* x, float* y, int B, int C, int H, int W, void* stream);
int e4s_const_input_f32(const float* x, float* y, int B, int C, int H, int W, void* stream);

int e4s_resize_bilinear_f32(const float* x, float* y, int B, int C, int Hi, int Wi, int Ho, int Wo, void* stream);
int e4s_conv3x3_small_f32(const float* x, const float* w, float* y, int B, int H, int W, int Cin, int Cout, void* stream);
int e4s_conv3x3_stem_f32(const float* x, const float* w, float* y, double* stats_ws, int B, int H, int W, int Cin, int Cout, void* stream);
int e4s_instnorm_stats_f32(const float* x, float* stats, float* pooled, double* ws, int B, int HW, int C,
                           float eps, void* stream);
int e4s_instnorm_finalize_f32(const double* ws, float* stats, float* pooled, int B, int HW, int C, int nslots, float eps,
                              void* stream);
int e4s_instnorm_apply_stats_f32(const float* x, const float* stats, const float* gate, const float* res,
                                 const float* res_stats, const float* slope, float* y, double* ws, int* nslots,
                                 int B, int H, int W, int C, int rs, void* stream);
int64_t e4s_instnorm_ws_doubles(int B, int HW, int C);
int e4s_instnorm_apply_f32(const float* x, const float* stats, const float* gate, const float* res,
                           const float* res_stats, const float* slope, float* y,
                           int B, int H, int W, int C, int rs, void* stream);
int e4s_se_gate_f32(const float* pooled, const float* fc1, const float* fc2, float* gate,
                    int B, int C, int Cr, void* stream);
int e4s_instnorm_finalize_se_f32(const double* ws, float* stats, const float* fc1, const float* fc2, float* gate, int B, int HW,
                                 int C, int Cr, int nslots, float eps, void* stream);
int e4s_region_mean_f32(const float* feats, const uint8_t* labels, int Hm, int Wm, float* out, float* ws,
                        int B, int H, int W, int C, int R, int out_stride, int out_off, void* stream);
int64_t e4s_region_mean_ws_floats(int B, int HW, int C, int R);
int e4s_swap_styles_f32(const float* tgt, const float* src, float* out, int B, int R, int C, unsigned sel, int ear, int teeth, int below,
                        void* stream);
int e4s_grouped_linear_f32(const float* x, const float* W, const float* bias, const float* add, float* y,
                           int B, int R, int K, int O, float scale, int act, float alpha, void* stream);

int e4s_adaptive_pool_f32(const float* x, float* y, int B, int C, int Hi, int Wi, int y0, int x0, int Hc, int Wc, int Ho,
                          int Wo, int in_nchw, const float* scale, const float* shift, void* stream);
int e4s_adaptive_pool_bwd_f32(const float* dy, float* dx, int B, int C, int Hi, int Wi, int y0, int x0, int Hc, int Wc,
                              int Ho, int Wo, int in_nchw, const float* scale, int accumulate, void* stream);
int e4s_conv_smallcin_f32(const float* x, const float* wp, const float* bias, float* y, int B, int Hi, int Wi, int Cin,
                          int Ho, int Wo, int Cout, int k, int stride, int pad, int relu, void* stream);
int e4s_conv_smallcin_bwd_f32(const float* dy, const float* wp, float* dx, int B, int Hi, int Wi, int Cin, int Ho, int Wo,
                              int Cout, int k, int stride, int pad, void* stream);
int e4s_conv_smallcin_col2im_f32(const float* z, float* dx, int B, int Hi, int Wi, int Cin, int Ho, int Wo, int ZC, int k, int stride,
                                 int pad, void* stream);
int e4s_maxpool3s2_f32(const float* x, float* y, uint8_t* idx, int B, int Hi, int Wi, int C, void* stream);
int e4s_maxpool3s2_bwd_f32(const float* dy, const uint8_t* idx, float* dx, int B, int Hi, int Wi, int C, void* stream);
int e4s_maxpool2_f32(const float* x, float* y, uint8_t* idx, int B, int Hi, int Wi, int C, void* stream);
int e4s_maxpool2_bwd_f32(const float* dy, const uint8_t* idx, float* dx, int B, int Hi, int Wi, int C, void* stream);
int e4s_relu_bwd_f32(const float* dy, const float* y, float* dx, int64_t n, int accumulate, void* stream);
int e4s_lpips_layer_f32(const float* fx, const float* fy, const float* w, float* out, double* ws, int B, int HW, int C,
                        void* stream);
int64_t e4s_lpips_layer_ws_doubles(int B, int HW);
int e4s_lpips_layer_bwd_f32(const float* fx, const float* fy, const float* w, const float* gout, float gmul, float* dfx,
                            int B, int HW, int C, int accumulate, void* stream);
int e4s_instnorm_bwd_sums_f32(const float* dy, const float* x, const float* stats, float* sums, double* ws, int B, int HW,
                              int C, void* stream);
int e4s_norm_bwd_frozen_f32(const float* dy, const float* stats, const float* gate, const float* extra, float* dx, int B,
                            int HW, int C, int accumulate, void* stream);
int e4s_cosine_f32(const float* a, const float* b, float* out, double* ws, int B, int64_t D, void* stream);
int64_t e4s_cosine_ws_doubles(int B, int64_t D);
int e4s_cosine_bwd_f32(const float* a, const float* b, const float* coef, const float* gout, float gmul, float* da, int B,
                       int64_t D, int accumulate, void* stream);

int e4s_parser_preprocess_f32(const void* src, int is_u8, float* dst, int B, int H, int W, const float* taps8, void* stream);
int e4s_maxpool3s2p1_f32(const float* x, float* y, int B, int Hi, int Wi, int C, void* stream);
int e4s_add_relu_f32(const float* a, const float* r, float* y, int64_t npix, int C, int y_cstride, int y_coff, void* stream);
int e4s_mean_hw_f32(const float* x, float* out, int B, int HW, int C, void* stream);
int e4s_parser_fc_f32(const float* v, const float* w, const float* bias, float* out, int B, int Ci, int Co, int act, float offset,
                      void* stream);
int e4s_gate_add_up2_f32(const float* x, const float* gate, const float* add, int add_map, float* y, int B, int h, int w, int C,
                         void* stream);
int e4s_parser_head_f32(const float* logits, int B, int h, int w, int ncls, int cstride, int H, int W, int seg12,
                        uint8_t* labels, float* onehot, float* nchw, void* stream);

typedef struct {
    const float* x;
    const float* w;
    const float* bias;
    float* y;
    const float* r0;
    const float* r1;
    int B, Hi, Wi, Cin;
    int x_cstride, y_cstride, y_coff;
    int r0_cstride, r0_coff, r1_cstride, r1_coff;
    int epilogue, up2, precision;
    float s0, s1, slope;
} e4s_rrdb_params;
int e4s_rrdb_conv_f32(const e4s_rrdb_params* p, void* stream);
int e4s_rrdb_pack_f32(const float* w, void* out, int Cin, int split, void* stream);
int64_t e4s_rrdb_pack_bytes(int Cin);
int e4s_rrdb_head_f32(const void* src, int is_u8, int flip, const float* wp, const float* bias, float* y, int y_cstride,
                      float* y2, int y2_cstride, int B, int H, int W, void* stream);
int e4s_rrdb_tail_f32(const float* x, int x_cstride, const float* wp, const float* bias, float* yf, int nchw, uint8_t* yu,
                      int flip, int B, int H, int W, void* stream);

#ifdef __cplusplus
}
#endif
#endif
```

Baseline: 486.3 images/s.

## Fuse instnorm finalize into stats kernels via last-block tickets; batch RGB weight jobs

The stem conv and the instnorm apply+stats kernel now finalize per-channel mean/rstd inside the kernel. Each block stores its partial sums atomically, takes a ticket, and the last arriving block reduces all slots, which removes a separate finalize launch per norm. Separately, the toRGB modulated weights for every layer are computed in one multi-job launch from a precomputed job table instead of one launch per layer. The ticket scheme adds atomics, fences and a serialized tail reduction in the last block. It also depends on ticket counters that reset themselves and are shared per stream, which is risky under graph capture.

```diff
diff --git a/e4s_amd/csrc/encoder.hip b/e4s_amd/csrc/encoder.hip
--- a/e4s_amd/csrc/encoder.hip
+++ b/e4s_amd/csrc/encoder.hip
@@ -57,8 +57,51 @@
     }
 }
 
+__device__ __forceinline__ void instnorm_finish(double s, double q, int HW, float eps, float& mf, float& rstd, float& pooled) {
+    const double mean = s / HW;
+    double var = q / HW - mean * mean;
+    if (var < 0.0) var = 0.0;
+    mf = (float)mean;
+    rstd = rsqrtf((float)var + eps);
+    pooled = (float)((mean - (double)mf) * (double)rstd);
+}
+
+__device__ __forceinline__ void slot_store(double* p, double v) {
+    __hip_atomic_store(reinterpret_cast<unsigned long long*>(p), (unsigned long long)__double_as_longlong(v), __ATOMIC_RELAXED,
+                       __HIP_MEMORY_SCOPE_AGENT);
+}
+__device__ __forceinline__ double slot_load(const double* p) {
+    return __longlong_as_double((long long)__hip_atomic_load(reinterpret_cast<const unsigned long long*>(p), __ATOMIC_RELAXED,
+                                                             __HIP_MEMORY_SCOPE_AGENT));
+}
+__device__ __forceinline__ bool last_ticket(unsigned* counter, unsigned n) {
+    asm volatile("s_waitcnt vmcnt(0)" ::: "memory");
+    unsigned t = 0;
+    if ((threadIdx.x & 63) == 0) t = __hip_atomic_fetch_add(counter, 1u, __ATOMIC_RELAXED, __HIP_MEMORY_SCOPE_AGENT);
+    t = __shfl(t, 0, 64);
+    if (t != n - 1) return false;
+    __builtin_amdgcn_fence(__ATOMIC_ACQUIRE, "agent");
+    asm volatile("s_waitcnt vmcnt(0)" ::: "memory");
+    if ((threadIdx.x & 63) == 0) __hip_atomic_store(counter, 0u, __ATOMIC_RELAXED, __HIP_MEMORY_SCOPE_AGENT);
+    return true;
+}
+__device__ __forceinline__ void finalize_slots(const double* ws, float* stats, float* pooled, int64_t i, int nslots, int HW, float eps) {
+    double s = 0.0, q = 0.0;
+#pragma unroll 8
+    for (int k = 0; k < nslots; ++k) {
+        s += slot_load(ws + (i * nslots + k) * 2);
+        q += slot_load(ws + (i * nslots + k) * 2 + 1);
+    }
+    float mf, rstd, pl;
+    instnorm_finish(s, q, HW, eps, mf, rstd, pl);
+    stats[i * 2] = mf;
+    stats[i * 2 + 1] = rstd;
+    if (pooled) pooled[i] = pl;
+}
+
 __global__ __launch_bounds__(256) void conv3x3_stem_kernel(const float* __restrict__ x, const float* __restrict__ w, float* __restrict__ y,
-                                                           double* __restrict__ stats_ws, int H, int W, int tx_n, int per_img) {
+                                                           double* stats_ws, int H, int W, int tx_n, int per_img,
+                                                           unsigned* tickets, float* __restrict__ fin_stats, float eps) {
     __shared__ f32x4 sx[18 * 18];
     __shared__ double sred[2][16][64];
     const int tid = threadIdx.x;
@@ -121,8 +164,15 @@
                 c += sred[1][r][tid];
             }
             double* slot = stats_ws + (((int64_t)b * 64 + tid) * per_img + rem) * 2;
-            slot[0] = a;
-            slot[1] = c;
+            if (!tickets) {
+                slot[0] = a;
+                slot[1] = c;
+            } else {
+                slot_store(slot, a);
+                slot_store(slot + 1, c);
+                if (last_ticket(tickets + b, (unsigned)per_img))
+                    finalize_slots(stats_ws, fin_stats, nullptr, (int64_t)b * 64 + tid, per_img, H * W, eps);
+            }
         }
     }
 }
@@ -211,14 +261,11 @@
         s += ws[((int64_t)i * nsplit + k) * 2];
         q += ws[((int64_t)i * nsplit + k) * 2 + 1];
     }
-    const double mean = s / HW;
-    double var = q / HW - mean * mean;
-    if (var < 0.0) var = 0.0;
-    const float mf = (float)mean;
-    const float rstd = rsqrtf((float)var + eps);
+    float mf, rstd, pl;
+    instnorm_finish(s, q, HW, eps, mf, rstd, pl);
     stats[i * 2] = mf;
     stats[i * 2 + 1] = rstd;
-    if (pooled) pooled[i] = (float)((mean - (double)mf) * (double)rstd);
+    if (pooled) pooled[i] = pl;
 }
 
 __global__ void instnorm_apply_kernel(const float* __restrict__ x, const float* __restrict__ stats,
@@ -265,8 +312,9 @@
 __global__ void instnorm_apply_stats_kernel(const float* __restrict__ x, const float* __restrict__ stats,
                                             const float* __restrict__ gate, const float* __restrict__ res,
                                             const float* __restrict__ res_stats, const float* __restrict__ slope,
-                                            float* __restrict__ y, double* __restrict__ ws, int H, int W, int C, int rs,
-                                            int nsplit) {
+                                            float* __restrict__ y, double* ws, int H, int W, int C, int rs,
+                                            int nsplit, unsigned* tickets, float* __restrict__ fin_stats,
+                                            float* __restrict__ fin_pooled, float eps) {
     const int slabs = C / 64, HW = H * W;
     const int split = blockIdx.x % nsplit;
     const int slab = (blockIdx.x / nsplit) % slabs;
@@ -323,9 +371,16 @@
             a += red[0][k][threadIdx.x];
             d += red[1][k][threadIdx.x];
         }
-        double* slot = ws + (((int64_t)b * C + slab * 64 + threadIdx.x) * nsplit + split) * 2;
-        slot[0] = a;
-        slot[1] = d;
+        const int64_t i = (int64_t)b * C + slab * 64 + threadIdx.x;
+        double* slot = ws + (i * nsplit + split) * 2;
+        if (!tickets) {
+            slot[0] = a;
+            slot[1] = d;
+        } else {
+            slot_store(slot, a);
+            slot_store(slot + 1, d);
+            if (last_ticket(tickets + b * slabs + slab, (unsigned)nsplit)) finalize_slots(ws, fin_stats, fin_pooled, i, nsplit, HW, eps);
+        }
     }
 }
 
@@ -668,7 +723,21 @@
     const int tx_n = W / 16, per_img = (H / 16) * tx_n;
     const int64_t blocks = (int64_t)B * per_img;
     if (blocks >= (1ll << 31)) return (int)hipErrorInvalidValue;
-    hipLaunchKernelGGL(conv3x3_stem_kernel, dim3((unsigned)blocks), dim3(256), 0, as_stream(stream), x, w, y, stats_ws, H, W, tx_n, per_img);
+    hipLaunchKernelGGL(conv3x3_stem_kernel, dim3((unsigned)blocks), dim3(256), 0, as_stream(stream), x, w, y, stats_ws, H, W, tx_n, per_img,
+                       (unsigned*)nullptr, (float*)nullptr, 0.f);
+    E4S_CHECK_LAUNCH();
+    return 0;
+}
+
+extern "C" int e4s_conv3x3_stem_fin_f32(const float* x, const float* w, float* y, double* stats_ws, unsigned* tickets, float* stats, int B,
+                                        int H, int W, int Cin, int Cout, float eps, void* stream) {
+    if (!x || !w || !y || !stats_ws || !tickets || !stats || Cin != 3 || Cout != 64 || H % 16 || W % 16 || B <= 0 || H <= 0 || W <= 0)
+        return (int)hipErrorInvalidValue;
+    const int tx_n = W / 16, per_img = (H / 16) * tx_n;
+    const int64_t blocks = (int64_t)B * per_img;
+    if (blocks >= (1ll << 31)) return (int)hipErrorInvalidValue;
+    hipLaunchKernelGGL(conv3x3_stem_kernel, dim3((unsigned)blocks), dim3(256), 0, as_stream(stream), x, w, y, stats_ws, H, W, tx_n, per_img,
+                       tickets, stats, eps);
     E4S_CHECK_LAUNCH();
     return 0;
 }
@@ -716,7 +785,19 @@
     const int ns = instnorm_nsplit(B, H * W, C);
     *nslots = ns;
     hipLaunchKernelGGL(instnorm_apply_stats_kernel, dim3(B * (C / 64) * ns), dim3(256), 0, as_stream(stream), x, stats, gate,
-                       res, res_stats, slope, y, ws, H, W, C, rs, ns);
+                       res, res_stats, slope, y, ws, H, W, C, rs, ns, (unsigned*)nullptr, (float*)nullptr, (float*)nullptr, 0.f);
+    E4S_CHECK_LAUNCH();
+    return 0;
+}
+
+extern "C" int e4s_instnorm_apply_stats_fin_f32(const float* x, const float* stats, const float* gate, const float* res,
+                                                const float* res_stats, const float* slope, float* y, double* ws, unsigned* tickets,
+                                                float* out_stats, float* out_pooled, int B, int H, int W, int C, int rs, float eps,
+                                                void* stream) {
+    if (C % 64 || rs < 1 || !ws || !tickets || !out_stats || B <= 0 || H <= 0 || W <= 0) return (int)hipErrorInvalidValue;
+    const int ns = instnorm_nsplit(B, H * W, C);
+    hipLaunchKernelGGL(instnorm_apply_stats_kernel, dim3(B * (C / 64) * ns), dim3(256), 0, as_stream(stream), x, stats, gate,
+                       res, res_stats, slope, y, ws, H, W, C, rs, ns, tickets, out_stats, out_pooled, eps);
     E4S_CHECK_LAUNCH();
     return 0;
 }
diff --git a/e4s_amd/csrc/ops.hip b/e4s_amd/csrc/ops.hip
--- a/e4s_amd/csrc/ops.hip
+++ b/e4s_amd/csrc/ops.hip
@@ -113,7 +113,7 @@
 
 }
 
-extern "C" int e4s_abi_version(void) { return 18; }
+extern "C" int e4s_abi_version(void) { return 19; }
 extern "C" const char* e4s_build_arch(void) { return "gfx950"; }
 
 extern "C" int e4s_fused_bias_act_f32(const float* x, const float* b, const float* ref, float* y, int64_t n,
diff --git a/e4s_amd/csrc/style.hip b/e4s_amd/csrc/style.hip
--- a/e4s_amd/csrc/style.hip
+++ b/e4s_amd/csrc/style.hip
@@ -105,6 +105,18 @@
     ws[i] = scale * w[c * cin + ci] * s[(size_t)g * cin + ci];
 }
 
+__global__ void rgb_weights_multi_kernel(const e4s_rgb_weights_job* __restrict__ jobs, const float* __restrict__ s_base,
+                                         float* __restrict__ ws_base) {
+    const e4s_rgb_weights_job jb = jobs[blockIdx.y];
+    const int64_t i = (int64_t)blockIdx.x * blockDim.x + threadIdx.x;
+    const int64_t n = (int64_t)jb.G * 3 * jb.cin;
+    if (i >= n) return;
+    const int ci = (int)(i % jb.cin);
+    const int c = (int)((i / jb.cin) % 3);
+    const int g = (int)(i / (3 * (int64_t)jb.cin));
+    ws_base[jb.out_off + i] = jb.scale * jb.w[c * jb.cin + ci] * s_base[jb.s_off + (size_t)g * jb.cin + ci];
+}
+
 __global__ void polyphase_weights_kernel(const float* __restrict__ w, const float* __restrict__ k4,
                                          float* __restrict__ out, int cout, int cin) {
     const int64_t n = (int64_t)cout * cin;
@@ -246,3 +258,13 @@
     E4S_CHECK_LAUNCH();
     return 0;
 }
+
+extern "C" int e4s_rgb_weights_multi_f32(const e4s_rgb_weights_job* jobs, int njobs, const float* s_base, float* ws_base, int64_t max_n,
+                                         void* stream) {
+    if (!jobs || !s_base || !ws_base || njobs <= 0 || njobs > 65535 || max_n <= 0 || (max_n + 255) / 256 >= (1ll << 31))
+        return (int)hipErrorInvalidValue;
+    hipLaunchKernelGGL(rgb_weights_multi_kernel, dim3((unsigned)((max_n + 255) / 256), njobs), dim3(256), 0, as_stream(stream), jobs, s_base,
+                       ws_base);
+    E4S_CHECK_LAUNCH();
+    return 0;
+}
diff --git a/e4s_amd/kernels.py b/e4s_amd/kernels.py
--- a/e4s_amd/kernels.py
+++ b/e4s_amd/kernels.py
@@ -185,6 +185,29 @@
     g, cin = s.shape
     out = torch.empty(g, 3, cin, device=s.device, dtype=torch.float32)
     call("e4s_rgb_weights_f32", fptr(w), fptr(s), fptr(out), g, cin, float(scale), stream())
+    return out
+
+
+_RGB_JOB_FMT = "Qqqiif4x"
+
+
+def rgb_weights_jobs(jobs, device):
+    import struct
+    assert struct.calcsize(_RGB_JOB_FMT) == 40
+    recs, offs, off = [], [], 0
+    for j in jobs:
+        if j["w"].dtype != torch.float32 or not j["w"].is_contiguous() or j["w"].numel() != 3 * j["cin"]:
+            raise RuntimeError("rgb_weights_jobs: contiguous fp32 [3,Cin] weights")
+        recs.append(struct.pack(_RGB_JOB_FMT, j["w"].data_ptr(), int(j["s_off"]), off, int(j["G"]), int(j["cin"]), float(j["scale"])))
+        offs.append(off)
+        off += j["G"] * 3 * j["cin"]
+    table = torch.frombuffer(bytearray(b"".join(recs)), dtype=torch.uint8).to(device)
+    return table, len(jobs), max(j["G"] * 3 * j["cin"] for j in jobs), offs, off
+
+
+def rgb_weights_multi(table, njobs, max_n, s_base, total):
+    out = torch.empty(total, device=s_base.device, dtype=torch.float32)
+    call("e4s_rgb_weights_multi_f32", ptr(table), njobs, fptr(s_base), fptr(out), max_n, stream())
     return out
 
 
@@ -642,6 +665,19 @@
     return y
 
 
+FUSED_FINALIZE = os.environ.get("E4S_FUSED_FINALIZE", "1") != "0"
+_ticket_bufs, _ticket_keep = {}, []
+
+
+def _tickets(n, device):
+    key = (device.index, torch.cuda.current_stream(device).cuda_stream)
+    t = _ticket_bufs.get(key)
+    if t is None or t.numel() < n:
+        _ticket_keep.append(t)
+        t = _ticket_bufs[key] = torch.zeros(max(n, 4096), device=device, dtype=torch.int32)
+    return t
+
+
 def conv3x3_small(x, w, want_stats=False):
     b, h, wd, cin = x.shape
     cout = w.shape[0]
@@ -649,6 +685,11 @@
     if cin == 3 and cout == 64 and h % 16 == 0 and wd % 16 == 0:
         slots = (h // 16) * (wd // 16)
         fused = torch.empty(b * cout * slots * 2, device=x.device, dtype=torch.float64) if want_stats else None
+        if want_stats and FUSED_FINALIZE:
+            stats = torch.empty(b, cout, 2, device=x.device, dtype=torch.float32)
+            call("e4s_conv3x3_stem_fin_f32", fptr(x), fptr(_f32(w)), fptr(y), ptr(fused), ptr(_tickets(b, x.device)), fptr(stats),
+                 b, h, wd, cin, cout, 1e-5, stream())
+            return y, stats
         call("e4s_conv3x3_stem_f32", fptr(x), fptr(_f32(w)), fptr(y), ptr(fused), b, h, wd, cin, cout, stream())
         if not want_stats:
             return y
@@ -675,6 +716,11 @@
     y = torch.empty_like(x)
     if want_stats and c % 64 == 0:
         ws = torch.empty(lib.load().e4s_instnorm_ws_doubles(b, h * w, c), device=x.device, dtype=torch.float64)
+        if FUSED_FINALIZE:
+            out_stats = torch.empty(b, c, 2, device=x.device, dtype=torch.float32)
+            call("e4s_instnorm_apply_stats_fin_f32", fptr(x), fptr(stats), fptr(gate), fptr(res), fptr(res_stats), fptr(slope),
+                 fptr(y), ptr(ws), ptr(_tickets(b * (c // 64), x.device)), fptr(out_stats), None, b, h, w, c, rs, 1e-5, stream())
+            return y, out_stats
         nslots = ctypes.c_int(0)
         call("e4s_instnorm_apply_stats_f32", fptr(x), fptr(stats), fptr(gate), fptr(res), fptr(res_stats), fptr(slope),
              fptr(y), ptr(ws), ctypes.byref(nslots), b, h, w, c, rs, stream())
diff --git a/e4s_amd/lib.py b/e4s_amd/lib.py
--- a/e4s_amd/lib.py
+++ b/e4s_amd/lib.py
@@ -5,7 +5,7 @@
 
 _HERE = os.path.dirname(os.path.abspath(__file__))
 LIB_PATH = os.environ.get("E4S_LIB_PATH") or os.path.join(_HERE, "libe4s_hip.so")
-ABI_VERSION = 18
+ABI_VERSION = 19
 
 c_p = ctypes.c_void_p
 c_i = ctypes.c_int
@@ -78,6 +78,7 @@
     "e4s_polyphase_weights_f32": [c_p, c_p, c_p, c_i, c_i, c_p],
     "e4s_polyphase_fold_f32": [c_p, c_p, c_p, c_i, c_i, c_p],
     "e4s_rgb_weights_f32": [c_p, c_p, c_p, c_i, c_i, c_f, c_p],
+    "e4s_rgb_weights_multi_f32": [c_p, c_i, c_p, c_p, c_l, c_p],
     "e4s_mask_labels": [c_p, c_p, c_p, c_i, c_i, c_i, c_i, c_p],
     "e4s_region_plan": [c_p] + [c_i] * 8 + [c_p, c_p, c_p, c_p, c_i, c_i, c_p],
     "e4s_conv_mfma_f32": [ctypes.POINTER(ConvParams), c_i, c_p],
@@ -155,9 +156,11 @@
     "e4s_resize_bilinear_f32": [c_p, c_p] + [c_i] * 6 + [c_p],
     "e4s_conv3x3_small_f32": [c_p, c_p, c_p] + [c_i] * 5 + [c_p],
     "e4s_conv3x3_stem_f32": [c_p, c_p, c_p, c_p] + [c_i] * 5 + [c_p],
+    "e4s_conv3x3_stem_fin_f32": [c_p] * 6 + [c_i] * 5 + [c_f, c_p],
     "e4s_instnorm_stats_f32": [c_p, c_p, c_p, c_p, c_i, c_i, c_i, c_f, c_p],
     "e4s_instnorm_finalize_f32": [c_p, c_p, c_p, c_i, c_i, c_i, c_i, c_f, c_p],
     "e4s_instnorm_apply_stats_f32": [c_p] * 9 + [c_i] * 5 + [c_p],
+    "e4s_instnorm_apply_stats_fin_f32": [c_p] * 11 + [c_i] * 5 + [c_f, c_p],
     "e4s_instnorm_apply_f32": [c_p] * 7 + [c_i] * 5 + [c_p],
     "e4s_se_gate_f32": [c_p, c_p, c_p, c_p, c_i, c_i, c_i, c_p],
     "e4s_instnorm_finalize_se_f32": [c_p, c_p, c_p, c_p, c_p, c_i, c_i, c_i, c_i, c_i, c_f, c_p],
diff --git a/e4s_amd/networks.py b/e4s_amd/networks.py
--- a/e4s_amd/networks.py
+++ b/e4s_amd/networks.py
@@ -219,7 +219,7 @@
             from .shard import quiesce_before_capture
             quiesce_before_capture()
             with K.flag_sink(self.flags):
-                with torch.cuda.graph(self.graph, capture_error_mode=mode):
+                with torch.cuda.graph(self.graph, stream=side, capture_error_mode=mode):
                     self.out = face_swap_core(self.net, *self.static, noise=self.noise)
         self.graph.replay()
         return self.out
diff --git a/e4s_amd/stylegan2.py b/e4s_amd/stylegan2.py
--- a/e4s_amd/stylegan2.py
+++ b/e4s_amd/stylegan2.py
@@ -15,6 +15,7 @@
 UPCONV_BF16X3_EXACT = os.environ.get("E4S_UPCONV_BF16X3", "exact") != "polyphase"
 CONV_C32 = os.environ.get("E4S_CONV_C32", "1") != "0"
 REGION_ROWS = os.environ.get("E4S_REGION_ROWS", "1") != "0"
+RGB_WEIGHTS_MULTI = os.environ.get("E4S_RGB_WEIGHTS_MULTI", "1") != "0"
 
 
 def make_kernel(k):
@@ -366,9 +367,9 @@
         self.bias = nn.Parameter(torch.zeros(1, 3, 1, 1))
         self.mask_op = mask_op
 
-    def run_nhwc(self, x, s, labels, num_regions, skip, rec=None):
-        pk = self.conv.packed()
-        ws = K.rgb_weights(pk["w"].view(3, -1), s, self.conv.scale)
+    def run_nhwc(self, x, s, labels, num_regions, skip, rec=None, ws=None):
+        if ws is None:
+            ws = K.rgb_weights(self.conv.packed()["w"].view(3, -1), s, self.conv.scale)
         if rec is not None:
             rec.update(ws=ws)
         k4 = self.upsample.kernel if skip is not None else None
@@ -525,15 +526,16 @@
             i += 2
         packs = [l.conv.packed() for l, _, _ in layers]
         key = (b, r, nlat, str(dev)) + tuple(
-            (l.conv.modulation.weight.data_ptr(), l.conv.modulation.bias.data_ptr(), pk["wsq"].data_ptr() if pk["wsq"] is not None else 0)
-            for (l, _, _), pk in zip(layers, packs))
+            (l.conv.modulation.weight.data_ptr(), l.conv.modulation.bias.data_ptr(), pk["wsq"].data_ptr() if pk["wsq"] is not None else 0,
+             pk["w"].data_ptr() if kind == "rgb" else 0)
+            for (l, _, kind), pk in zip(layers, packs))
         plan = getattr(self, "_e4s_style_plan", None)
         if plan is not None and plan["key"] == key:
             return plan
         if torch.cuda.is_current_stream_capturing():
             raise RuntimeError("Generator._style_plan: the job tables of the style prologue must exist before a stream capture "
                                "(run the same shapes once eagerly first -- GraphedStep / GraphedFaceSwap warm up for that)")
-        sjobs, djobs, meta, keep = [], [], {}, []
+        sjobs, djobs, rjobs, rlayers, meta, keep = [], [], [], [], {}, []
         s_off = d_off = 0
         for layer, idx, kind in layers:
             mod = layer.conv.modulation
@@ -553,10 +555,18 @@
                                   scale=layer.conv.scale))
                 m["d"] = (d_off, g, cout)
                 d_off += g * cout
+            else:
+                w_rgb = layer.conv.packed()["w"].view(3, -1)
+                keep.append(w_rgb)
+                rjobs.append(dict(w=w_rgb, s_off=s_off, G=g, cin=cin, scale=layer.conv.scale))
+                rlayers.append(m)
             s_off += g * cin
             meta[id(layer)] = m
+        rtab, nr, rmax, roffs, rtotal = K.rgb_weights_jobs(rjobs, dev)
+        for m, off in zip(rlayers, roffs):
+            m["ws"] = (off, m["s"][1], m["s"][2])
         plan = {"key": key, "s": K.rowdot_jobs(sjobs, dev), "d": K.rowdot_jobs(djobs, dev), "meta": meta, "s_floats": s_off,
-                "d_floats": d_off, "keep": keep}
+                "d_floats": d_off, "keep": keep, "rgb": (rtab, nr, rmax), "rgb_floats": rtotal}
         self._e4s_style_plan = plan
         return plan
 
@@ -578,6 +588,13 @@
             dbuf = torch.empty(sp["d_floats"], device=lat.device, dtype=torch.float32)
             K.rowdot_multi(*sp["s"], lat, sbuf, 0)
             K.rowdot_multi(*sp["d"], sbuf, dbuf, 1)
+        wsbuf = K.rgb_weights_multi(*sp["rgb"], sbuf, sp["rgb_floats"]) if sp is not None and tape is None and RGB_WEIGHTS_MULTI else None
+
+        def pre_ws(layer):
+            if wsbuf is None:
+                return None
+            off, g, c = sp["meta"][id(layer)]["ws"]
+            return wsbuf[off:off + g * 3 * c].view(g, 3, c)
 
         def pre(layer, which):
             off, g, c = sp["meta"][id(layer)][which]
@@ -603,7 +620,9 @@
         def styled_then_rgb(conv2, to_rgb, x, idx, nz, skip):
             mod = to_rgb.conv.modulation
             s_rgb = pre(to_rgb, "s") if sp is not None else K.modulate(lat, idx + 1, False, mod.weight, mod.bias)
-            ws = K.rgb_weights(to_rgb.conv.packed()["w"].view(3, -1), s_rgb, to_rgb.conv.scale)
+            ws = pre_ws(to_rgb)
+            if ws is None:
+                ws = K.rgb_weights(to_rgb.conv.packed()["w"].view(3, -1), s_rgb, to_rgb.conv.scale)
             y, partial = styled(conv2, x, idx, nz, rgb_ws=ws)
             out = K.torgb_finish(partial, to_rgb.bias, skip, to_rgb.upsample.kernel if skip is not None else None)
             if tape is not None:
@@ -617,7 +636,7 @@
             if soft and layer.mask_op:
                 return layer.run_nhwc_soft(x, s, mask, skip)
             rec = {} if tape is not None else None
-            out = layer.run_nhwc(x, s, labels if layer.mask_op else None, r, skip, rec=rec)
+            out = layer.run_nhwc(x, s, labels if layer.mask_op else None, r, skip, rec=rec, ws=pre_ws(layer))
             if tape is not None:
                 rec.update(kind="rgb", layer=layer, idx=idx, masked=layer.mask_op, x=x, s=s, has_skip=skip is not None, out=out,
                            labels=labels if layer.mask_op else None)
diff --git a/include/e4s_hip.h b/include/e4s_hip.h
--- a/include/e4s_hip.h
+++ b/include/e4s_hip.h
@@ -40,6 +40,14 @@
 int e4s_polyphase_fold_f32(const float* deff, const float* k4, float* dw, int cout, int cin, void* stream);
 
 int e4s_rgb_weights_f32(const float* w, const float* s, float* ws, int G, int cin, float scale, void* stream);
+typedef struct e4s_rgb_weights_job {
+    const float* w;
+    int64_t s_off, out_off;
+    int G, cin;
+    float scale;
+} e4s_rgb_weights_job;
+int e4s_rgb_weights_multi_f32(const e4s_rgb_weights_job* jobs, int njobs, const float* s_base, float* ws_base, int64_t max_n,
+                              void* stream);
 
 
 int e4s_mask_labels(const float* mask, uint8_t* labels, int* flags, int B, int R, int Hm, int Wm, void* stream);
@@ -274,6 +282,8 @@
 int e4s_resize_bilinear_f32(const float* x, float* y, int B, int C, int Hi, int Wi, int Ho, int Wo, void* stream);
 int e4s_conv3x3_small_f32(const float* x, const float* w, float* y, int B, int H, int W, int Cin, int Cout, void* stream);
 int e4s_conv3x3_stem_f32(const float* x, const float* w, float* y, double* stats_ws, int B, int H, int W, int Cin, int Cout, void* stream);
+int e4s_conv3x3_stem_fin_f32(const float* x, const float* w, float* y, double* stats_ws, unsigned* tickets, float* stats, int B, int H,
+                             int W, int Cin, int Cout, float eps, void* stream);
 int e4s_instnorm_stats_f32(const float* x, float* stats, float* pooled, double* ws, int B, int HW, int C,
                            float eps, void* stream);
 int e4s_instnorm_finalize_f32(const double* ws, float* stats, float* pooled, int B, int HW, int C, int nslots, float eps,
@@ -281,6 +291,10 @@
 int e4s_instnorm_apply_stats_f32(const float* x, const float* stats, const float* gate, const float* res,
                                  const float* res_stats, const float* slope, float* y, double* ws, int* nslots,
                                  int B, int H, int W, int C, int rs, void* stream);
+int e4s_instnorm_apply_stats_fin_f32(const float* x, const float* stats, const float* gate, const float* res,
+                                     const float* res_stats, const float* slope, float* y, double* ws, unsigned* tickets,
+                                     float* out_stats, float* out_pooled, int B, int H, int W, int C, int rs, float eps,
+                                     void* stream);
 int64_t e4s_instnorm_ws_doubles(int B, int HW, int C);
 int e4s_instnorm_apply_f32(const float* x, const float* stats, const float* gate, const float* res,
                            const float* res_stats, const float* slope, float* y,
```

Result: slower. 479.2 images/s (-1.4%).
